# irfanfadhullah/unet_zoo

Hardware: AMD Instinct MI355X
Metric: images/sec (fwd+bwd) at B=16 3x256x256, 1/2/4/8 MI355X (higher is better)
Workload: dtype bf16; 1 GPU; unet train step (zero_grad+fwd+BCE+bwd+clip+AdamW), B=16/GPU 3x256x256, random-init weights; global_batch=16, parallelism=dp1

## Files before the change

### include/unetzoo_hip.h

```cpp
#ifndef UNETZOO_HIP_H
#define UNETZOO_HIP_H

#include <stddef.h>
#include <stdint.h>

#ifdef __cplusplus
extern "C" {
#endif

#define UZ_ABI_VERSION 1

enum { UZ_F32 = 0, UZ_BF16 = 1 };

enum {
  UZ_OK = 0,
  UZ_EINVAL = -1,
  UZ_ENOTIMPL = -2
};

enum {
  UZ_TAPS_CONV = 0,
  UZ_TAPS_GATHER2X2 = 1,
  UZ_TAPS_CONV_UP2 = 2,
  UZ_TAPS_CONV_S2 = 3
// ... 34 lines not shown
                         const void* res, int ldres, void* y, void* workspace, void* stream);
long long uz_conv_igemm_workspace_bytes(const uz_conv_desc* d);
int uz_conv_igemm_ws_grid_m(const uz_conv_desc* d);
int uz_conv_igemm_ws(const uz_conv_desc* d, const void* x, const void* w_packed, const float* bias,
                     void* y, float* stats_partial, void* workspace, void* stream);
int uz_conv_igemm_bnred_supported(const uz_conv_desc* d);
int uz_conv_igemm_bnred(const uz_conv_desc* d, const void* x, const void* w_packed, void* y, const void* bn_y,
                        int ld_bny, const float* scale, const float* shift, const float* mean, const float* invstd,
                        float* partial, void* stream);

int uz_conv_igemm_xf_supported(const uz_conv_desc* d);
int uz_conv_igemm_xf(const uz_conv_desc* d, const void* x, const float* in_scale, const float* in_shift,
                     const void* w_packed, const float* bias, void* y, float* stats_partial, void* stream);

int uz_conv_igemm_bnact_supported(const uz_conv_desc* d);
int uz_conv_igemm_bnact(const uz_conv_desc* d, const void* x, const void* w_packed, const float* bias,
                        const float* out_scale, const float* out_shift, int relu, void* y, void* stream);

typedef struct uz_wgrad_desc {
  int dtype;
  int N, H, W;
  int Hr, Wr;
  int Ci, ldl;
  int Cj, ldr;
  int ntaps, taps_mode, dil;
} uz_wgrad_desc;

int uz_wgrad_split(const uz_wgrad_desc* d);
long long uz_wgrad_workspace_bytes(const uz_wgrad_desc* d);
int uz_wgrad(const uz_wgrad_desc* d, const void* L, const void* R, float* out, void* workspace,
             void* stream);
int uz_wgrad_kernel_name(const uz_wgrad_desc* d, char* buf, int cap);
int uz_wgrad_xf_supported(const uz_wgrad_desc* d);
int uz_wgrad_xf(const uz_wgrad_desc* d, const void* L, const void* R, const float* r_scale, const float* r_shift,
                float* out, void* workspace, void* stream, int phase);
int uz_wgrad_phase(const uz_wgrad_desc* d, const void* L, const void* R, float* out, void* workspace, void* stream,
                   int phase);
typedef struct {
  uz_wgrad_desc desc;
  const void* L;
  const void* R;
  float* out;
} uz_wgrad_item;
long long uz_wgrad_multi_workspace_bytes(const uz_wgrad_item* items, int n);
int uz_wgrad_multi(const uz_wgrad_item* items, int n, void* workspace, void* stream);
long long uz_wgrad_batched_workspace_bytes(const uz_wgrad_desc* d, int batch);
int uz_wgrad_batched(const uz_wgrad_desc* d, int batch, const void* L, long long lb, const void* R, long long rb,
                     float* out, long long ob, void* workspace, void* stream);
int uz_wgrad_batched2(const uz_wgrad_desc* d, int batch, int batch2, const void* L, long long lb, long long lb2, const void* R,
                      long long rb, long long rb2, float* out, long long ob, void* workspace, void* stream);

int uz_conv3x3_first_supported(int dtype, int C, int Cout);
int uz_conv3x3_first_rows(int N, int H, int W);
int uz_conv3x3_first_fwd(int dtype, const float* x, int N, int C, int H, int W, const float* w, const float* bias, int Cout,
                         void* y, int ldy, float* stats, void* stream);
int uz_conv3x3_first_fwd_bnact(int dtype, const float* x, int N, int C, int H, int W, const float* w, const float* bias,
                               int Cout, const float* out_scale, const float* out_shift, int relu, void* y, int ldy,
                               void* stream);
long long uz_conv3x3_first_wgrad_workspace_bytes(int N, int H, int W, int Cout);
int uz_conv3x3_first_wgrad(int dtype, const float* x, int N, int C, int H, int W, const void* dy, int lddy, int Cout, float* dw,
                           void* workspace, void* stream);
int uz_conv3x3_first_wgrad_bn(int dtype, const float* x, int N, int C, int H, int W, const void* g, int ldg, const void* y,
                              int ldy, const float* scale, const float* shift, const float* mean, const float* invstd,
                              const double* sums, double count, int Cout, float* dw, void* workspace, void* stream);

enum { UZ_PACK_CONV_FWD = 0, UZ_PACK_CONV_DGRAD = 1, UZ_PACK_CONVT_FWD = 2, UZ_PACK_CONVT_DGRAD = 3,
       UZ_PACK_IM2COL = 4, UZ_PACK_VEC_REPEAT = 5 };
int uz_pack_weights(int dtype, int mode, const float* w, int Co, int Ci, int T, int Kpad, void* dst,
                    void* stream);
typedef struct uz_pack_item {
  const float* src;
  void* dst;
  long long begin;
  int mode, Co, Ci, T, Kpad;
  int pad_;
} uz_pack_item;
int uz_pack_weights_batched(int dtype, const uz_pack_item* items_device, int n_items,
                            long long total_elements, void* stream);
typedef struct uz_pack3x3_item {
  const float* src;
  void* dst_fwd;
  void* dst_dgrad;
  int Co, Ci;
  int tile_begin;
  int pad_;
} uz_pack3x3_item;
int uz_pack_conv3x3_batched(int dtype, const uz_pack3x3_item* items_device, int n_items, int total_tiles,
                            void* stream);

int uz_im2col3x3_nchw(int dtype, const float* x_nchw, int N, int C, int H, int W, int Kpad, void* dst,
                      void* stream);

int uz_bn_finalize(const float* stats_partial, int grid_m, int C, double count, const float* gamma,
                   const float* beta, float eps, float momentum, float* running_mean,
                   float* running_var, float* scale, float* shift, float* mean, float* invstd,
                   void* stream);
int uz_bn_eval_scale(int C, const float* gamma, const float* beta, const float* running_mean,
                     const float* running_var, float eps, float* scale, float* shift, void* stream);

int uz_bn_relu_apply(int dtype, const void* y, int ldy, const float* scale, const float* shift,
                     int N, int H, int W, int C, void* act, int lda, void* pooled, int ldp,
                     void* stream);
int uz_bn_relu_add_apply(int dtype, const void* y, int ldy, const float* scale, const float* shift,
                         int N, int H, int W, int C, const void* res, int ldr, void* act, int lda,
                         void* pooled, int ldp, int pool_ceil, void* stream);
int uz_bn_relu_add_apply_fin(int dtype, const void* y, int ldy, const float* stats_partial, int rows, double count,
                             const float* gamma, const float* beta, float eps, float momentum, float* running_mean,
                             float* running_var, float* vec, int* flag, int N, int H, int W, int C, const void* res, int ldr,
                             void* act, int lda, void* pooled, int ldp, int pool_ceil, void* stream);

typedef struct uz_bnbwd_desc {
  int dtype;
  int N, H, W, C;
  int ldy, ldg0, ldg1, ldgp, lddy;
  int pool_ceil;
} uz_bnbwd_desc;
int uz_colstats_rows(int dtype, int P, int C);
int uz_colstats(int dtype, const void* x, int ld, int P, int C, float* partial, void* stream);
long long uz_bn_relu_bwd_workspace_bytes(const uz_bnbwd_desc* d, int has_pool_grad);
int uz_bn_relu_bwd_reduce(const uz_bnbwd_desc* d, const void* y, const float* scale,
                          const float* shift, const float* mean, const float* invstd, const void* g0,
                          const void* g1, const void* gpool, void* workspace, double* sums,
                          float* dgamma, float* dbeta, void* stream);
int uz_bn_relu_bwd_apply(const uz_bnbwd_desc* d, const void* y, const float* scale,
                         const float* shift, const float* mean, const float* invstd, const void* g0,
                         const void* g1, const void* gpool, const double* sums, double count,
                         void* dy, void* stream);
int uz_bn_relu_bwd_reduce_rows(const uz_bnbwd_desc* d, const void* y, const float* scale, const float* shift,
                               const float* mean, const float* invstd, const void* g0, const void* g1, const void* gpool,
                               void* workspace, void* stream);
int uz_bn_relu_bwd_apply_fin(const uz_bnbwd_desc* d, const void* y, const float* scale, const float* shift,
                             const float* mean, const float* invstd, const void* g0, const void* g1, const void* gpool,
                             const float* partial, int rows, double* sums, float* dgamma, float* dbeta, int* flag,
                             double count, void* dy, void* stream);
int uz_bn_bwd_finalize(const float* partial, int rows, int C, double* sums, float* dgamma, float* dbeta, void* stream);
int uz_bn_relu_bwd_apply_head_supported(int dtype, int C, int Kout);
int uz_bn_relu_bwd_apply_head(const uz_bnbwd_desc* d, const void* y, const float* scale, const float* shift, const float* mean,
                              const float* invstd, const float* g_nchw, const float* w, int Kout, const double* sums,
                              double count, void* dy, void* stream);

int uz_outconv_fwd(int dtype, const void* x, int ldx, int N, int HW, int C, const float* w,
                   const float* b, int Kout, float* out_nchw, void* stream);
int uz_outconv_fwd_xf(int dtype, const void* y, int ldy, int N, int HW, int C, const float* scale, const float* shift,
                      const float* w, const float* b, int Kout, float* out_nchw, void* stream);
long long uz_outconv_bwd_workspace_bytes(int dtype, int N, int HW, int C, int Kout);
int uz_outconv_bwd(int dtype, const void* x, int ldx, int N, int HW, int C, const float* w, int Kout,
                   const float* g_nchw, void* dx, int lddx, float* dw, float* db, void* workspace,
                   void* stream);
int uz_outconv_bwd_rows(int dtype, int N, int HW, int C);
int uz_outconv_bwd_bnred(int dtype, const void* x, int ldx, int N, int HW, int C, const float* w, int Kout,
                         const float* g_nchw, void* dx, int lddx, float* dw, float* db, void* workspace,
                         const void* bn_y, int ld_bny, const float* scale, const float* shift, const float* mean,
                         const float* invstd, float* bn_partial, void* stream);

int uz_attn_grid(int dtype, int P, int channels);
int uz_attn_psi_fwd(int dtype, const void* g1raw, int ldg, const void* x1raw, int ldx, const float* vec_g,
                    const float* vec_x, const float* wpsi, const float* bpsi ,
                    int P, int F, float* q, float* partial , void* stream);
int uz_attn_gate_fwd(int dtype, const void* x, int ldx, const float* q, const float* vec_q, int P, int C,
                     void* out, int ldo, void* stream);
int uz_attn_bwd_psi(int dtype, const void* dout, int ldd, const void* x, int ldx, const float* q,
                    const float* vec_q, int P, int C, void* dx_direct, int lddx, float* dz,
                    float* partial , void* stream);
int uz_attn_bwd_reduce(int dtype, const void* g1raw, int ldg, const void* x1raw, int ldx, const float* q,
                       const float* dz, const float* wpsi, const float* vec_g, const float* vec_x,
                       const float* vec_q, const double* a01, int P, int F,
                       float* partial , void* stream);
int uz_attn_bwd_apply(int dtype, const void* g1raw, int ldg, const void* x1raw, int ldx, const float* q,
                      const float* dz, const float* wpsi, const float* vec_g, const float* vec_x,
                      const float* vec_q, const double* a01, const double* totals, int P, int F,
                      void* dg1raw, int lddg, void* dx1raw, int lddx, void* stream);
int uz_sum_rows(const float* partial, int rows, int n, double* out, void* stream);
int uz_sum_rows_f32(const float* partial, int rows, int n, float* out0, int n0, float* out1, void* stream);
int uz_sum_rows_f32_ld(const float* partial, int ld, int rows, int n, float* out0, int n0, float* out1,
                       void* stream);
int uz_sum2x2(int dtype, const void* du, int ldu, int N, int H, int W, int C, void* dx, int lddx,
              void* stream);

int uz_bilinear_fwd(int dtype, const void* x, int ldx, long long x_img_stride, int N, int Hi, int Wi,
                    int C, void* y, int ldy, long long y_img_stride, int Ho, int Wo, void* stream);
int uz_bilinear_bwd(int dtype, const void* g, int ldg, long long g_img_stride, int N, int Hi, int Wi,
                    int C, void* dx, int lddx, long long dx_img_stride, int Ho, int Wo, void* stream);
int uz_resize_bilinear_fwd(int dtype, const void* x, int ldx, long long x_img_stride, int N, int Hi, int Wi,
                           int C, void* y, int ldy, long long y_img_stride, int Ho, int Wo, int align_corners,
                           void* stream);
int uz_resize_bilinear_bwd(int dtype, const void* g, int ldg, long long g_img_stride, int N, int Hi, int Wi,
                           int C, void* dx, int lddx, long long dx_img_stride, int Ho, int Wo, int align_corners,
                           void* stream);
int uz_resample2(int dtype, const void* src, int lds, int N, int Hs, int Ws, int C, void* dst, int ldd, int Hd,
                 int Wd, int mode, void* stream);
int uz_pool_grad_combine(int dtype, int N, int H, int W, int C, const void* act, int lda, const void* g0,
                         int ldg0, const void* g1, int ldg1, const void* gp, int ldgp, void* out, int ldo,
                         int pool_ceil, void* stream);
int uz_sideconv3x3_fwd(int dtype, const void* x, int ldx, int N, int H, int W, int C, const float* w,
                       const float* bias, float* taps_ws, float* out, long long out_img_stride,
                       void* stream);
long long uz_sideconv3x3_bwd_workspace_bytes(int dtype, int N, int H, int W, int C);
int uz_sideconv3x3_bwd(int dtype, const void* x, int ldx, int N, int H, int W, int C, const float* w,
                       const float* g, long long g_img_stride, void* dx, int lddx, float* dw, float* db,
                       void* workspace, void* stream);
int uz_fuse1x1_fwd(const float* d, int N, int HW, int Cc, int K, const float* w, const float* b,
                   float* out, void* stream);
long long uz_fuse1x1_bwd_workspace_bytes(int N, int HW, int Cc, int K);
int uz_fuse1x1_bwd(const float* d, int N, int HW, int Cc, int K, const float* w, const float* g,
                   const float* const* g_extra, int n_extra, float* dcat, float* dw, float* db,
                   void* workspace, void* stream);

int uz_patchify(int dtype, const float* x_nchw, int N, int C, int H, int W, int patch, int Kpad,
                void* out, void* stream);

enum { UZ_LN_PLAIN = 0, UZ_LN_MERGE = 1, UZ_LN_EXPAND = 2 };
typedef struct uz_ln_desc {
  int dtype, N, Ho, Wo, C;
  int ldx, ldy, ldr, ldg, lddx;
  int mode, r;
  float eps;
  int act;
} uz_ln_desc;
int uz_layernorm_fwd(const uz_ln_desc* d, const void* x, const float* gamma, const float* beta,
                     const void* res, const float* image_scale, void* y, float* stats, void* stream);
int uz_layernorm_bwd_rows(const uz_ln_desc* d);
int uz_layernorm_bwd(const uz_ln_desc* d, const void* x, const float* gamma, const float* stats,
                     const void* g, const float* image_scale, void* dx, float* partial, void* stream);
int uz_layernorm_act_bwd(const uz_ln_desc* d, const void* x, const float* gamma, const float* beta,
                         const float* stats, const void* g, void* dx, float* partial, void* stream);
int uz_ln_head_fwd(const uz_ln_desc* d, const void* x, const float* gamma, const float* beta, const float* w,
                   const float* b , int K, float* logits, float* stats, void* stream);
long long uz_ln_head_bwd_workspace_bytes(const uz_ln_desc* d, int K);
int uz_ln_head_bwd(const uz_ln_desc* d, const void* x, const float* gamma, const float* beta, const float* w,
                   int K, const float* stats, const float* dlogits, void* dx, float* dgamma, float* dbeta,
                   float* dw, float* db , float* workspace, void* stream);

typedef struct uz_winattn_desc {
  int dtype, B, H, W, C, heads, ws, shift, Nt;
  int ldq, ldo;
  float scale;
} uz_winattn_desc;
int uz_winattn_fwd(const uz_winattn_desc* d, const void* qkv, const float* tau, const float* bias,
                   void* out, float* lse, void* stream);
int uz_cpb_fwd(const float* idx, const float* w1, const float* b1, const float* w2, const float* b2, int R,
               int hidden, int heads, float* bias, void* stream);
int uz_cpb_bwd(const float* idx, const float* w1, const float* b1, const float* w2, const float* G, int R,
               int hidden, int heads, float* dw1, float* db1, float* dw2, float* db2, void* stream);
typedef struct {
  const float* idx;
  const float* w1;
  const float* b1;
  const float* w2;
  const float* b2;
  int R, hidden, heads, reserved;
  float* bias;
  const float* G;
  float* dw1;
  float* db1;
  float* dw2;
  float* db2;
} uz_cpb_item;
int uz_cpb_fwd_batched(const uz_cpb_item* items, int n, void* stream);
long long uz_cpb_bwd_batched_workspace_bytes(const uz_cpb_item* items, int n);
int uz_cpb_bwd_batched(const uz_cpb_item* items, int n, float* workspace, void* stream);
int uz_winattn_bwd_rows(const uz_winattn_desc* d);
int uz_winattn_bwd(const uz_winattn_desc* d, const void* qkv, const float* tau, const float* bias,
                   const void* out, const float* lse, const void* dout, int lddo, void* dqkv, int lddq,
                   float* partial, void* stream);

int uz_colsum(int dtype, const void* x, int ld, int P, int C, float* out, void* stream);
long long uz_colsum_workspace_bytes(int dtype, int P, int C);
int uz_colsum_ws(int dtype, const void* x, int ld, int P, int C, float* out, void* workspace, void* stream);

long long uz_clip_adamw_workspace_bytes(void);
int uz_clip_adamw(float* p, const float* g, float* m, float* v, long long n, float lr, float beta1,
                  float beta2, float eps, float weight_decay, float max_norm, float* step, void* workspace,
                  void* stream);

int uz_gelu_fwd(int dtype, const void* x, int ldx, void* y, int ldy, long long P, int C, void* stream);
int uz_gelu_bwd(int dtype, const void* x, int ldx, const void* g, int ldg, void* dx, int lddx, long long P,
                int C, void* stream);
int uz_dwconv3x3(int dtype, const void* x, int ldx, const float* w_taps, const float* bias, void* y, int ldy,
                 int N, int H, int W, int C, int flags, void* stream);
int uz_dwconv3x3_wgrad_rows(int dtype, int N, int H, int W, int C);
int uz_dwconv3x3_wgrad(int dtype, const void* x, int ldx, const void* g, int ldg, float* part, int N, int H,
                       int W, int C, void* stream);
int uz_space_to_depth(int dtype, const void* src, int lds, void* dst, int ldd, int N, int Ho, int Wo, int C, int r,
                      int inverse, void* stream);
int uz_space_to_depth_crop(int dtype, const void* src, int lds, void* dst, int ldd, int N, int H, int W, int C, int r,
                           int inverse, void* stream);
int uz_im2col_nchw(int dtype, const float* x_nchw, int N, int C, int H, int W, int k, int stride, int pad, int Kpad,
                   void* out, void* stream);
typedef struct uz_sra_desc {
  int dtype, B, N, NK, heads, head_dim, kps;
  int ldq, ldk, ldv, ldo;
  float scale;
} uz_sra_desc;
int uz_sra_fwd(const uz_sra_desc* d, const void* q, const void* k, const void* v, void* out, float* lse,
               void* stream);
long long uz_sra_bwd_workspace_bytes(const uz_sra_desc* d);
int uz_sra_bwd(const uz_sra_desc* d, const void* q, const void* k, const void* v, const void* o, const float* lse,
               const void* go, int ldgo, void* dq, int lddq, void* dkv, int lddkv, void* workspace, void* stream);

long long uz_bce_dice_workspace_bytes(long long n);
int uz_bce_dice(const float* logits, const float* target, long long n, float* dlogits, float* out2, void* workspace,
                void* stream);

#define UZ_REGION_MAX_ITEMS 64
typedef struct uz_region_item {
  const float* logits;
// ... 144 lines not shown
```

### unet_zoo_amd/_lib.py

```python
from __future__ import annotations

import ctypes
import os
from ctypes import POINTER, Structure, c_char_p, c_double, c_float, c_int, c_void_p

import torch

UZ_F32, UZ_BF16 = 0, 1
TAPS_CONV, TAPS_GATHER2X2, TAPS_CONV_UP2, TAPS_CONV_S2 = 0, 1, 2, 3
STORE_PLAIN, STORE_SHUFFLE2X2 = 0, 1
PACK_CONV_FWD, PACK_CONV_DGRAD, PACK_CONVT_FWD, PACK_CONVT_DGRAD, PACK_IM2COL, PACK_VEC_REPEAT = range(6)

LIB_NAME = "libunetzoo_hip.so"
LIB_PATH = os.environ.get("UNET_ZOO_AMD_LIB") or os.path.join(os.path.dirname(os.path.abspath(__file__)), LIB_NAME)

EXPORTS = (
    "uz_abi_version", "uz_last_error_string", "uz_build_ablate", "uz_source_hash", "uz_set_cu_reserve", "uz_get_cu_reserve", "uz_clock_probe", "uz_conv_igemm_grid_m", "uz_conv_igemm",
    "uz_wgrad_split", "uz_wgrad_workspace_bytes", "uz_wgrad", "uz_wgrad_kernel_name", "uz_wgrad_phase", "uz_wgrad_xf_supported", "uz_wgrad_xf", "uz_conv3x3_first_supported", "uz_conv3x3_first_rows", "uz_conv3x3_first_fwd",
    "uz_conv3x3_first_wgrad_workspace_bytes", "uz_conv3x3_first_wgrad", "uz_conv3x3_first_wgrad_bn", "uz_pack_weights", "uz_pack_weights_batched", "uz_pack_conv3x3_batched", "uz_im2col3x3_nchw", "uz_bn_finalize",
    "uz_bn_eval_scale", "uz_bn_relu_apply", "uz_bn_relu_bwd_workspace_bytes", "uz_bn_relu_bwd_reduce", "uz_bn_relu_bwd_apply",
    "uz_outconv_fwd", "uz_outconv_fwd_xf", "uz_outconv_bwd_workspace_bytes", "uz_outconv_bwd", "uz_outconv_bwd_rows", "uz_outconv_bwd_bnred", "uz_bn_relu_bwd_apply_head_supported", "uz_bn_relu_bwd_apply_head",
    "uz_colsum",
    "uz_attn_grid", "uz_attn_psi_fwd", "uz_attn_gate_fwd", "uz_attn_bwd_psi", "uz_attn_bwd_reduce",
    "uz_attn_bwd_apply", "uz_sum_rows", "uz_sum_rows_f32", "uz_sum2x2",
    "uz_bn_relu_add_apply", "uz_bn_relu_add_apply_fin", "uz_bn_relu_bwd_reduce_rows", "uz_bn_relu_bwd_apply_fin", "uz_bilinear_fwd", "uz_bilinear_bwd", "uz_resize_bilinear_fwd", "uz_resize_bilinear_bwd", "uz_resample2",
    "uz_pool_grad_combine",
    "uz_sideconv3x3_fwd", "uz_sideconv3x3_bwd_workspace_bytes", "uz_sideconv3x3_bwd",
    "uz_fuse1x1_fwd", "uz_fuse1x1_bwd_workspace_bytes", "uz_fuse1x1_bwd",
    "uz_conv_igemm_workspace_bytes", "uz_conv_igemm_ws_grid_m", "uz_conv_igemm_ws",
    "uz_conv_igemm_bnred_supported", "uz_conv_igemm_bnred", "uz_conv_igemm_xf_supported", "uz_conv_igemm_xf", "uz_conv_igemm_kernel_name", "uz_bn_bwd_finalize", "uz_profile_arm", "uz_profile_disarm",
    "uz_patchify", "uz_layernorm_fwd", "uz_layernorm_bwd_rows", "uz_layernorm_bwd", "uz_layernorm_act_bwd",
    "uz_ln_head_fwd", "uz_ln_head_bwd_workspace_bytes", "uz_ln_head_bwd", "uz_sum_rows_f32_ld",
    "uz_winattn_fwd", "uz_winattn_bwd_rows", "uz_winattn_bwd",
    "uz_colsum_workspace_bytes", "uz_colsum_ws", "uz_colstats_rows", "uz_colstats", "uz_cpb_fwd", "uz_cpb_bwd",
    "uz_cpb_fwd_batched", "uz_cpb_bwd_batched_workspace_bytes", "uz_cpb_bwd_batched",
    "uz_clip_adamw_workspace_bytes", "uz_clip_adamw",
    "uz_gelu_fwd", "uz_gelu_bwd", "uz_dwconv3x3", "uz_dwconv3x3_wgrad_rows", "uz_dwconv3x3_wgrad",
    "uz_space_to_depth", "uz_space_to_depth_crop", "uz_im2col_nchw", "uz_sra_fwd", "uz_sra_bwd_workspace_bytes", "uz_sra_bwd",
    "uz_bce_dice_workspace_bytes", "uz_bce_dice", "uz_colsum_batched_workspace_bytes", "uz_colsum_batched", "uz_sum_rows_f32_batched", "uz_conv_igemm_res", "uz_wgrad_multi_workspace_bytes", "uz_wgrad_multi", "uz_conv_igemm_res_ws",
    "uz_add_relu", "uz_relu_bwd", "uz_pil_resample_h_u8", "uz_pil_resample_v_f32",
    "uz_gemm_nt", "uz_softmax_fwd", "uz_softmax_bwd", "uz_adaptive_avgpool_fwd", "uz_adaptive_avgpool_bwd",
    "uz_rowdot_f32", "uz_cast_rows", "uz_wgrad_batched_workspace_bytes", "uz_wgrad_batched", "uz_wgrad_batched2",
    "uz_softmax_workspace_bytes", "uz_add_map", "uz_dropout", "uz_chanscale_relu", "uz_chanattn_probs_fwd", "uz_chanattn_probs_bwd",
    "uz_conv5x5_grid_m", "uz_conv5x5", "uz_wgrad5x5_workspace_bytes", "uz_wgrad5x5",
    "uz_bn_elu_apply", "uz_bn_elu_bwd_rows", "uz_bn_elu_bwd_reduce", "uz_bn_elu_bwd_apply",
    "uz_conv_igemm_bnact_supported", "uz_conv_igemm_bnact", "uz_conv3x3_first_fwd_bnact",
    "uz_region_loss_workspace_bytes", "uz_region_loss",
    "uz_class_loss_workspace_bytes", "uz_class_loss",
)


class ConvDesc(Structure):
    _fields_ = [(n, c_int) for n in (
        "dtype", "N", "H", "W", "Hin", "Win", "Cin", "ldx", "Nout", "ldy", "ntaps", "taps_mode",
        "dil", "store_mode", "Co", "Hout", "Wout")]


class WgradDesc(Structure):
    _fields_ = [(n, c_int) for n in (
        "dtype", "N", "H", "W", "Hr", "Wr", "Ci", "ldl", "Cj", "ldr", "ntaps", "taps_mode", "dil")]


class Conv5Desc(Structure):
    _fields_ = [(n, c_int) for n in ("dtype", "N", "H", "W", "Cin", "ldx", "Nout", "ldy", "ksize")]


class Wgrad5Desc(Structure):
    _fields_ = [(n, c_int) for n in ("dtype", "N", "H", "W", "Ci", "ldl", "Cj", "ldr", "ksize", "CiOut", "CjOut")]


class BnEluBwdDesc(Structure):
    _fields_ = [(n, c_int) for n in ("dtype", "N", "HW", "C", "ldx", "ldo", "ldg0", "ldg1", "ldg2", "lddx", "ldgres", "flags")]


class BnBwdDesc(Structure):
    _fields_ = [(n, c_int) for n in (
        "dtype", "N", "H", "W", "C", "ldy", "ldg0", "ldg1", "ldgp", "lddy", "pool_ceil")]


class LnDesc(Structure):
    _fields_ = [(n, c_int) for n in ("dtype", "N", "Ho", "Wo", "C", "ldx", "ldy", "ldr", "ldg", "lddx", "mode", "r")] \
        + [("eps", c_float), ("act", c_int)]


class WinAttnDesc(Structure):
    _fields_ = [(n, c_int) for n in ("dtype", "B", "H", "W", "C", "heads", "ws", "shift", "Nt", "ldq", "ldo")] \
        + [("scale", c_float)]


class SraDesc(Structure):
    _fields_ = [(n, c_int) for n in ("dtype", "B", "N", "NK", "heads", "head_dim", "kps", "ldq", "ldk", "ldv", "ldo")] \
        + [("scale", c_float)]


class GemmDesc(Structure):
    _fields_ = [(n, c_int) for n in ("dtype", "batch", "M", "N", "K", "ldx", "ldw", "ldy", "ldres")] \
        + [(n, ctypes.c_longlong) for n in ("xb", "wb", "yb", "resb")] + [("batch2", c_int)] \
        + [(n, ctypes.c_longlong) for n in ("xb2", "wb2", "yb2", "resb2")]


class WgradItem(Structure):
    _fields_ = [("desc", WgradDesc), ("L", c_void_p), ("R", c_void_p), ("out", c_void_p)]


class SumRowsItem(Structure):
    _fields_ = [("partial", c_void_p), ("out0", c_void_p), ("out1", c_void_p), ("rows", c_int), ("n", c_int), ("n0", c_int),
                ("reserved", c_int)]


class ColsumItem(Structure):
    _fields_ = [("x", c_void_p), ("out", c_void_p), ("P", c_int), ("C", c_int), ("ld", c_int), ("reserved", c_int)]


LN_PLAIN, LN_MERGE, LN_EXPAND = 0, 1, 2


class CpbItem(Structure):
    _fields_ = [(n, c_void_p) for n in ("idx", "w1", "b1", "w2", "b2")] \
        + [(n, c_int) for n in ("R", "hidden", "heads", "reserved")] \
        + [(n, c_void_p) for n in ("bias", "G", "dw1", "db1", "dw2", "db2")]


class PackItem(Structure):
    _fields_ = [("src", c_void_p), ("dst", c_void_p), ("begin", ctypes.c_longlong), ("mode", c_int),
                ("Co", c_int), ("Ci", c_int), ("T", c_int), ("Kpad", c_int), ("pad_", c_int)]


class Pack3x3Item(Structure):
    _fields_ = [("src", c_void_p), ("dst_fwd", c_void_p), ("dst_dgrad", c_void_p), ("Co", c_int), ("Ci", c_int),
                ("tile_begin", c_int), ("pad_", c_int)]


REGION_MAX_ITEMS = 64


class RegionItem(Structure):
    _fields_ = [("logits", c_void_p), ("target", c_void_p), ("dlogits", c_void_p), ("weight", c_float)]


class RegionDesc(Structure):
    _fields_ = [("n_items", c_int), ("n", ctypes.c_longlong), ("groups", c_int)] \
        + [(n, c_float) for n in ("w_bce", "w_region", "alpha", "beta", "smooth", "gamma", "pos_weight")] \
        + [("metric_item", c_int)]


CLASS_MAX_ITEMS = 16
CLASS_MAX_K = 32
CLASS_REDUCE_BATCH, CLASS_REDUCE_IMAGE = 0, 1


class ClassItem(Structure):
    _fields_ = [("logits", c_void_p), ("dlogits", c_void_p), ("weight", c_float)]


class ClassDesc(Structure):
    _fields_ = [("n_items", c_int), ("N", c_int), ("K", c_int), ("HW", ctypes.c_longlong)] \
        + [(n, c_float) for n in ("w_ce", "w_dice", "smooth", "label_smoothing")] \
        + [(n, c_int) for n in ("ignore_index", "reduce", "include_background", "square", "metric_item")]


class HipLibraryError(RuntimeError):
    pass


_lib = None


def load():
    global _lib
    if _lib is not None:
        return _lib
    if not os.path.exists(LIB_PATH):
        raise HipLibraryError(
            f"{LIB_PATH} not found: the HIP kernel library is not built. Run "
            "`python -c 'import __graft_entry__ as g; g.build()'` from the repo root. "
            "unet_zoo_amd has no CPU fallback.")
    lib = ctypes.CDLL(LIB_PATH)
    lib.uz_abi_version.restype = c_int
    lib.uz_last_error_string.restype = c_char_p
    lib.uz_source_hash.restype = c_char_p
    lib.uz_source_hash.argtypes = []
    vp, ip, fp = c_void_p, c_int, c_float
    lib.uz_set_cu_reserve.argtypes = [c_int]
    lib.uz_clock_probe.argtypes = [c_int, vp, c_int, vp]
    lib.uz_get_cu_reserve.argtypes = []
    lib.uz_conv_igemm_grid_m.argtypes = [POINTER(ConvDesc)]
    lib.uz_conv_igemm.argtypes = [POINTER(ConvDesc), vp, vp, vp, vp, vp, vp]
    lib.uz_conv_igemm_res.argtypes = [POINTER(ConvDesc), vp, vp, vp, vp, ip, vp, vp]
    lib.uz_conv_igemm_res_ws.argtypes = [POINTER(ConvDesc), vp, vp, vp, vp, ip, vp, vp, vp]
    lib.uz_conv_igemm_workspace_bytes.argtypes = [POINTER(ConvDesc)]
    lib.uz_conv_igemm_ws_grid_m.argtypes = [POINTER(ConvDesc)]
    lib.uz_conv_igemm_ws.argtypes = [POINTER(ConvDesc), vp, vp, vp, vp, vp, vp, vp]
    lib.uz_conv_igemm_bnred_supported.argtypes = [POINTER(ConvDesc)]
    lib.uz_conv_igemm_xf_supported.argtypes = [POINTER(ConvDesc)]
    lib.uz_conv_igemm_xf.argtypes = [POINTER(ConvDesc), vp, vp, vp, vp, vp, vp, vp, vp]
    lib.uz_conv_igemm_bnact_supported.argtypes = [POINTER(ConvDesc)]
    lib.uz_conv_igemm_bnact.argtypes = [POINTER(ConvDesc), vp, vp, vp, vp, vp, c_int, vp, vp]
    lib.uz_conv_igemm_kernel_name.argtypes = [POINTER(ConvDesc), c_int, c_char_p, c_int]
    lib.uz_profile_arm.argtypes = [vp, vp]
    lib.uz_profile_disarm.argtypes = []
    lib.uz_conv_igemm_bnred.argtypes = [POINTER(ConvDesc), vp, vp, vp, vp, c_int, vp, vp, vp, vp, vp, vp]
    lib.uz_bn_bwd_finalize.argtypes = [vp, c_int, c_int, vp, vp, vp, vp]
    lib.uz_patchify.argtypes = [ip, vp, ip, ip, ip, ip, ip, ip, vp, vp]
    lib.uz_layernorm_fwd.argtypes = [POINTER(LnDesc), vp, vp, vp, vp, vp, vp, vp, vp]
    lib.uz_layernorm_act_bwd.argtypes = [POINTER(LnDesc), vp, vp, vp, vp, vp, vp, vp, vp]
    lib.uz_layernorm_bwd_rows.argtypes = [POINTER(LnDesc)]
    lib.uz_layernorm_bwd.argtypes = [POINTER(LnDesc), vp, vp, vp, vp, vp, vp, vp, vp]
    lib.uz_ln_head_fwd.argtypes = [POINTER(LnDesc), vp, vp, vp, vp, vp, ip, vp, vp, vp]
    lib.uz_ln_head_bwd_workspace_bytes.argtypes = [POINTER(LnDesc), ip]
    lib.uz_ln_head_bwd.argtypes = [POINTER(LnDesc), vp, vp, vp, vp, ip, vp, vp, vp, vp, vp, vp, vp, vp, vp]
    lib.uz_sum_rows_f32_ld.argtypes = [vp, ip, ip, ip, vp, ip, vp, vp]
    lib.uz_winattn_fwd.argtypes = [POINTER(WinAttnDesc), vp, vp, vp, vp, vp, vp]
    lib.uz_winattn_bwd_rows.argtypes = [POINTER(WinAttnDesc)]
    lib.uz_winattn_bwd.argtypes = [POINTER(WinAttnDesc), vp, vp, vp, vp, vp, vp, ip, vp, ip, vp, vp]
    lib.uz_colstats_rows.argtypes = [ip, ip, ip]
    lib.uz_colstats.argtypes = [ip, vp, ip, ip, ip, vp, vp]
    lib.uz_cpb_fwd.argtypes = [vp, vp, vp, vp, vp, ip, ip, ip, vp, vp]
    lib.uz_cpb_bwd.argtypes = [vp, vp, vp, vp, vp, ip, ip, ip, vp, vp, vp, vp, vp]
    lib.uz_cpb_fwd_batched.argtypes = [vp, ip, vp]
    lib.uz_cpb_bwd_batched_workspace_bytes.argtypes = [vp, ip]
    lib.uz_cpb_bwd_batched.argtypes = [vp, ip, vp, vp]
    lib.uz_clip_adamw_workspace_bytes.argtypes = []
    lib.uz_clip_adamw.argtypes = [vp, vp, vp, vp, ctypes.c_longlong, fp, fp, fp, fp, fp, fp, vp, vp, vp]
    lib.uz_wgrad_split.argtypes = [POINTER(WgradDesc)]
    lib.uz_wgrad_workspace_bytes.argtypes = [POINTER(WgradDesc)]
    lib.uz_wgrad.argtypes = [POINTER(WgradDesc), vp, vp, vp, vp, vp]
    lib.uz_wgrad_kernel_name.argtypes = [POINTER(WgradDesc), c_char_p, c_int]
    lib.uz_wgrad_phase.argtypes = [POINTER(WgradDesc), vp, vp, vp, vp, vp, c_int]
    lib.uz_wgrad_xf_supported.argtypes = [POINTER(WgradDesc)]
    lib.uz_wgrad_xf.argtypes = [POINTER(WgradDesc), vp, vp, vp, vp, vp, vp, vp, c_int]
    lib.uz_conv3x3_first_supported.argtypes = [ip, ip, ip]
    lib.uz_conv3x3_first_rows.argtypes = [ip, ip, ip]
    lib.uz_conv3x3_first_fwd.argtypes = [ip, vp, ip, ip, ip, ip, vp, vp, ip, vp, ip, vp, vp]
    lib.uz_conv3x3_first_fwd_bnact.argtypes = [ip, vp, ip, ip, ip, ip, vp, vp, ip, vp, vp, ip, vp, ip, vp]
    lib.uz_conv3x3_first_wgrad_workspace_bytes.argtypes = [ip, ip, ip, ip]
    lib.uz_conv3x3_first_wgrad_workspace_bytes.restype = ctypes.c_longlong
    lib.uz_conv3x3_first_wgrad.argtypes = [ip, vp, ip, ip, ip, ip, vp, ip, ip, vp, vp, vp]
    lib.uz_conv3x3_first_wgrad_bn.argtypes = [ip, vp, ip, ip, ip, ip, vp, ip, vp, ip, vp, vp, vp, vp, vp, ctypes.c_double, ip, vp, vp, vp]
    lib.uz_pack_weights.argtypes = [ip, ip, vp, ip, ip, ip, ip, vp, vp]
    lib.uz_pack_weights_batched.argtypes = [ip, vp, ip, ctypes.c_longlong, vp]
    lib.uz_pack_conv3x3_batched.argtypes = [ip, vp, ip, ip, vp]
    lib.uz_im2col3x3_nchw.argtypes = [ip, vp, ip, ip, ip, ip, ip, vp, vp]
    lib.uz_bn_finalize.argtypes = [vp, ip, ip, c_double, vp, vp, fp, fp, vp, vp, vp, vp, vp, vp, vp]
    lib.uz_bn_eval_scale.argtypes = [ip, vp, vp, vp, vp, fp, vp, vp, vp]
    lib.uz_bn_relu_apply.argtypes = [ip, vp, ip, vp, vp, ip, ip, ip, ip, vp, ip, vp, ip, vp]
    lib.uz_bn_relu_bwd_workspace_bytes.argtypes = [POINTER(BnBwdDesc), ip]
    lib.uz_bn_relu_bwd_reduce.argtypes = [POINTER(BnBwdDesc), vp, vp, vp, vp, vp, vp, vp, vp, vp, vp,
                                          vp, vp, vp]
    lib.uz_bn_relu_bwd_apply.argtypes = [POINTER(BnBwdDesc), vp, vp, vp, vp, vp, vp, vp, vp, vp,
                                         c_double, vp, vp]
    lib.uz_outconv_fwd.argtypes = [ip, vp, ip, ip, ip, ip, vp, vp, ip, vp, vp]
    lib.uz_outconv_fwd_xf.argtypes = [ip, vp, ip, ip, ip, ip, vp, vp, vp, vp, ip, vp, vp]
    lib.uz_outconv_bwd_workspace_bytes.argtypes = [ip, ip, ip, ip, ip]
    lib.uz_outconv_bwd.argtypes = [ip, vp, ip, ip, ip, ip, vp, ip, vp, vp, ip, vp, vp, vp, vp]
    lib.uz_outconv_bwd_rows.argtypes = [ip, ip, ip, ip]
    lib.uz_bn_relu_bwd_apply_head_supported.argtypes = [ip, ip, ip]
    lib.uz_bn_relu_bwd_apply_head.argtypes = [POINTER(BnBwdDesc), vp, vp, vp, vp, vp, vp, vp, ip, vp, ctypes.c_double, vp, vp]
    lib.uz_outconv_bwd_bnred.argtypes = [ip, vp, ip, ip, ip, ip, vp, ip, vp, vp, ip, vp, vp, vp, vp, ip, vp, vp, vp, vp, vp, vp]
    lib.uz_colsum.argtypes = [ip, vp, ip, ip, ip, vp, vp]
    lib.uz_colsum_workspace_bytes.argtypes = [ip, ip, ip]
    lib.uz_colsum_ws.argtypes = [ip, vp, ip, ip, ip, vp, vp, vp]
    lib.uz_attn_grid.argtypes = [ip, ip, ip]
    lib.uz_attn_psi_fwd.argtypes = [ip, vp, ip, vp, ip, vp, vp, vp, vp, ip, ip, vp, vp, vp]
    lib.uz_attn_gate_fwd.argtypes = [ip, vp, ip, vp, vp, ip, ip, vp, ip, vp]
    lib.uz_attn_bwd_psi.argtypes = [ip, vp, ip, vp, ip, vp, vp, ip, ip, vp, ip, vp, vp, vp]
    lib.uz_attn_bwd_reduce.argtypes = [ip, vp, ip, vp, ip, vp, vp, vp, vp, vp, vp, vp, ip, ip, vp, vp]
    lib.uz_attn_bwd_apply.argtypes = [ip, vp, ip, vp, ip, vp, vp, vp, vp, vp, vp, vp, vp, ip, ip, vp, ip,
                                      vp, ip, vp]
    lib.uz_sum_rows.argtypes = [vp, ip, ip, vp, vp]
    lib.uz_sum_rows_f32.argtypes = [vp, ip, ip, vp, ip, vp, vp]
    lib.uz_sum2x2.argtypes = [ip, vp, ip, ip, ip, ip, ip, vp, ip, vp]
    ll = ctypes.c_longlong
    lib.uz_bn_relu_add_apply.argtypes = [ip, vp, ip, vp, vp, ip, ip, ip, ip, vp, ip, vp, ip, vp, ip, ip, vp]
    lib.uz_bn_relu_add_apply_fin.argtypes = [ip, vp, ip, vp, ip, ctypes.c_double, vp, vp, c_float, c_float, vp, vp, vp, vp,
                                             ip, ip, ip, ip, vp, ip, vp, ip, vp, ip, ip, vp]
    lib.uz_bn_relu_bwd_reduce_rows.argtypes = [POINTER(BnBwdDesc), vp, vp, vp, vp, vp, vp, vp, vp, vp, vp]
    lib.uz_bn_relu_bwd_apply_fin.argtypes = [POINTER(BnBwdDesc), vp, vp, vp, vp, vp, vp, vp, vp, vp, ip, vp, vp, vp, vp,
                                             ctypes.c_double, vp, vp]
    lib.uz_bilinear_fwd.argtypes = [ip, vp, ip, ll, ip, ip, ip, ip, vp, ip, ll, ip, ip, vp]
    lib.uz_bilinear_bwd.argtypes = [ip, vp, ip, ll, ip, ip, ip, ip, vp, ip, ll, ip, ip, vp]
    lib.uz_resize_bilinear_fwd.argtypes = [ip, vp, ip, ll, ip, ip, ip, ip, vp, ip, ll, ip, ip, ip, vp]
    lib.uz_resize_bilinear_bwd.argtypes = [ip, vp, ip, ll, ip, ip, ip, ip, vp, ip, ll, ip, ip, ip, vp]
    lib.uz_resample2.argtypes = [ip, vp, ip, ip, ip, ip, ip, vp, ip, ip, ip, ip, vp]
    lib.uz_pool_grad_combine.argtypes = [ip, ip, ip, ip, ip, vp, ip, vp, ip, vp, ip, vp, ip, vp, ip, ip, vp]
    lib.uz_sideconv3x3_fwd.argtypes = [ip, vp, ip, ip, ip, ip, ip, vp, vp, vp, vp, ll, vp]
    lib.uz_sideconv3x3_bwd_workspace_bytes.argtypes = [ip, ip, ip, ip, ip]
    lib.uz_sideconv3x3_bwd.argtypes = [ip, vp, ip, ip, ip, ip, ip, vp, vp, ll, vp, ip, vp, vp, vp, vp]
    lib.uz_fuse1x1_fwd.argtypes = [vp, ip, ip, ip, ip, vp, vp, vp, vp]
    lib.uz_fuse1x1_bwd_workspace_bytes.argtypes = [ip, ip, ip, ip]
    lib.uz_fuse1x1_bwd.argtypes = [vp, ip, ip, ip, ip, vp, vp, POINTER(c_void_p), ip, vp, vp, vp, vp, vp]
    lib.uz_sum_rows_f32_batched.argtypes = [POINTER(SumRowsItem), ip, vp]
    lib.uz_wgrad_multi_workspace_bytes.argtypes = [POINTER(WgradItem), ip]
    lib.uz_wgrad_multi_workspace_bytes.restype = ctypes.c_longlong
    lib.uz_wgrad_multi.argtypes = [POINTER(WgradItem), ip, vp, vp]
    lib.uz_colsum_batched_workspace_bytes.argtypes = [ip, POINTER(ColsumItem), ip]
    lib.uz_colsum_batched.argtypes = [ip, POINTER(ColsumItem), ip, vp, vp]
    lib.uz_bce_dice_workspace_bytes.argtypes = [ll]
    lib.uz_bce_dice.argtypes = [vp, vp, ll, vp, vp, vp, vp]
    lib.uz_gelu_fwd.argtypes = [ip, vp, ip, vp, ip, ll, ip, vp]
    lib.uz_gelu_bwd.argtypes = [ip, vp, ip, vp, ip, vp, ip, ll, ip, vp]
    lib.uz_dwconv3x3.argtypes = [ip, vp, ip, vp, vp, vp, ip, ip, ip, ip, ip, ip, vp]
    lib.uz_dwconv3x3_wgrad_rows.argtypes = [ip, ip, ip, ip, ip]
    lib.uz_dwconv3x3_wgrad.argtypes = [ip, vp, ip, vp, ip, vp, ip, ip, ip, ip, vp]
    lib.uz_space_to_depth.argtypes = [ip, vp, ip, vp, ip, ip, ip, ip, ip, ip, ip, vp]
    lib.uz_space_to_depth_crop.argtypes = [ip, vp, ip, vp, ip, ip, ip, ip, ip, ip, ip, vp]
    lib.uz_im2col_nchw.argtypes = [ip, vp, ip, ip, ip, ip, ip, ip, ip, ip, vp, vp]
    lib.uz_sra_fwd.argtypes = [POINTER(SraDesc), vp, vp, vp, vp, vp, vp]
    lib.uz_sra_bwd_workspace_bytes.argtypes = [POINTER(SraDesc)]
    lib.uz_sra_bwd.argtypes = [POINTER(SraDesc), vp, vp, vp, vp, vp, vp, ip, vp, ip, vp, ip, vp, vp]
    lib.uz_add_relu.argtypes = [ip, vp, ip, vp, ip, vp, ip, ll, ip, vp]
    lib.uz_relu_bwd.argtypes = [ip, vp, ip, vp, ip, vp, ip, ll, ip, vp]
    lib.uz_pil_resample_h_u8.argtypes = [vp, ip, ip, ip, vp, vp, ip, ip, vp, vp]
    lib.uz_pil_resample_v_f32.argtypes = [vp, ip, ip, ip, vp, vp, ip, ip, POINTER(c_float), POINTER(c_float), ip, vp, vp]
    lib.uz_wgrad_batched_workspace_bytes.argtypes = [POINTER(WgradDesc), ip]
    lib.uz_wgrad_batched.argtypes = [POINTER(WgradDesc), ip, vp, ll, vp, ll, vp, ll, vp, vp]
    lib.uz_wgrad_batched2.argtypes = [POINTER(WgradDesc), ip, ip, vp, ll, ll, vp, ll, ll, vp, ll, vp, vp]
    lib.uz_gemm_nt.argtypes = [POINTER(GemmDesc), vp, vp, vp, vp, vp, vp]
    lib.uz_softmax_workspace_bytes.argtypes = [ip, ip, ip, ip]
    lib.uz_softmax_fwd.argtypes = [ip, vp, ip, ll, ip, ip, ip, ip, c_float, vp, vp]
    lib.uz_chanattn_probs_fwd.argtypes = [ip, vp, ip, ip, ip, ip, c_float, c_float, vp, vp, vp]
    lib.uz_chanattn_probs_bwd.argtypes = [ip, vp, vp, ip, ip, ip, ip, c_float, c_float, vp, vp, vp]
    lib.uz_dropout.argtypes = [ip, vp, ip, vp, c_float, vp, ip, ll, ip, vp]
    lib.uz_chanscale_relu.argtypes = [ip, ip, vp, ip, vp, ip, vp, vp, ip, ip, ip, vp, ip, vp]
    lib.uz_add_map.argtypes = [ip, vp, ip, vp, vp, ip, ll, ip, ip, vp]
    lib.uz_softmax_bwd.argtypes = [ip, vp, vp, ip, ll, ip, ip, ip, ip, c_float, vp, ip, vp]
    lib.uz_adaptive_avgpool_fwd.argtypes = [ip, vp, ip, ip, ip, ip, ip, vp, ip, ip, ip, vp]
    lib.uz_adaptive_avgpool_bwd.argtypes = [ip, vp, ip, ip, ip, ip, ip, vp, ip, ip, ip, ip, vp]
    lib.uz_rowdot_f32.argtypes = [ip, vp, ip, vp, ip, ll, ip, vp, vp]
    lib.uz_cast_rows.argtypes = [ip, vp, ip, vp, ip, ll, ip, ip, vp]
    lib.uz_conv5x5_grid_m.argtypes = [POINTER(Conv5Desc)]
    lib.uz_conv5x5.argtypes = [POINTER(Conv5Desc), vp, vp, vp, vp, vp, vp]
    lib.uz_wgrad5x5_workspace_bytes.argtypes = [POINTER(Wgrad5Desc)]
    lib.uz_wgrad5x5.argtypes = [POINTER(Wgrad5Desc), vp, vp, vp, vp, vp]
    lib.uz_bn_elu_apply.argtypes = [ip, vp, ip, vp, vp, ip, ip, ip, vp, ip, vp, ip, vp, ip, vp, ip, vp]
    lib.uz_bn_elu_bwd_rows.argtypes = [POINTER(BnEluBwdDesc)]
    lib.uz_bn_elu_bwd_reduce.argtypes = [POINTER(BnEluBwdDesc), vp, vp, vp, vp, vp, vp, vp, vp, vp, vp, vp, vp]
    lib.uz_bn_elu_bwd_apply.argtypes = [POINTER(BnEluBwdDesc), vp, vp, vp, vp, vp, vp, vp, vp, vp, vp, vp, vp, vp, vp]
    lib.uz_region_loss_workspace_bytes.argtypes = [POINTER(RegionDesc)]
    lib.uz_region_loss.argtypes = [POINTER(RegionDesc), POINTER(RegionItem), vp, vp, vp]
    lib.uz_class_loss_workspace_bytes.argtypes = [POINTER(ClassDesc)]
    lib.uz_class_loss.argtypes = [POINTER(ClassDesc), POINTER(ClassItem), vp, vp, vp, vp, vp, vp]
    for name in EXPORTS:
        fn = getattr(lib, name)
        if name not in ("uz_last_error_string", "uz_source_hash"):
            fn.restype = ctypes.c_longlong if name.endswith("_workspace_bytes") else c_int
    if lib.uz_abi_version() != 1:
        raise HipLibraryError("libunetzoo_hip.so ABI version mismatch; rebuild it")
    _lib = lib
    return lib


def _fail(rc: int, what: str):
    msg = load().uz_last_error_string().decode("utf-8", "replace")
    raise HipLibraryError(f"{what} failed (code {rc}): {msg}")


def check(rc: int, what: str) -> None:
    if rc != 0:
        _fail(rc, what)


def check_count(rc: int, what: str) -> int:
    if rc < 0:
        _fail(rc, what)
    return rc


def region_loss_workspace_bytes(desc: "RegionDesc") -> int:
    return check_count(load().uz_region_loss_workspace_bytes(ctypes.byref(desc)), "uz_region_loss_workspace_bytes")


def region_loss(desc: "RegionDesc", items, out2: torch.Tensor, workspace: torch.Tensor) -> None:
    check(load().uz_region_loss(ctypes.byref(desc), items, out2.data_ptr(), workspace.data_ptr(), stream_ptr()),
          "uz_region_loss")


def class_loss_workspace_bytes(desc: "ClassDesc") -> int:
    return check_count(load().uz_class_loss_workspace_bytes(ctypes.byref(desc)), "uz_class_loss_workspace_bytes")


def class_loss(desc: "ClassDesc", items, labels: torch.Tensor, class_weight, out2: torch.Tensor, counts: torch.Tensor,
               workspace: torch.Tensor) -> None:
    check(load().uz_class_loss(ctypes.byref(desc), items, labels.data_ptr(),
                               class_weight.data_ptr() if class_weight is not None else None, out2.data_ptr(),
                               counts.data_ptr() if counts is not None else None, workspace.data_ptr(), stream_ptr()),
          "uz_class_loss")


def set_cu_reserve(n: int) -> None:
    check(load().uz_set_cu_reserve(int(n)), "uz_set_cu_reserve")


def get_cu_reserve() -> int:
    return int(load().uz_get_cu_reserve())


def mfma_clock_ghz(settle_s: float = 0.6, iters: int = 40000) -> dict:
    import time
    lib = load()
    dev = torch.device("cuda", torch.cuda.current_device())
    out = torch.zeros(256, 2, dtype=torch.int64, device=dev)
    torch.cuda.synchronize()
    t_end = time.perf_counter() + settle_s
    while time.perf_counter() < t_end:
        for _ in range(4):
            check(lib.uz_clock_probe(iters, out.data_ptr(), 256, stream_ptr()), "uz_clock_probe")
        torch.cuda.synchronize()
    e0, e1 = torch.cuda.Event(enable_timing=True), torch.cuda.Event(enable_timing=True)
    e0.record()
    check(lib.uz_clock_probe(iters, out.data_ptr(), 256, stream_ptr()), "uz_clock_probe")
    e1.record()
# ... 28 lines not shown
```

### unet_zoo_amd/csrc/uz_common.h

```cpp
#pragma once
#include <hip/hip_runtime.h>
#include <stdarg.h>
#include <stdint.h>
#include <stdio.h>
#include "../../include/unetzoo_hip.h"

typedef __bf16 bf16_t;
typedef __attribute__((ext_vector_type(16))) float f32x16;
typedef __attribute__((ext_vector_type(4))) float f32x4;
typedef __attribute__((ext_vector_type(8))) __bf16 bf16x8;
typedef __attribute__((ext_vector_type(4))) __bf16 bf16x4;

#include <hip/hip_ext.h>
bool uz_prof_take(hipEvent_t* e0, hipEvent_t* e1);
#undef hipLaunchKernelGGL
#define hipLaunchKernelGGL(kern, grid, block, shm, stream, ...)                                              \
  do {                                                                                                       \
    hipEvent_t uz_e0_, uz_e1_;                                                                               \
    if (uz_prof_take(&uz_e0_, &uz_e1_))                                                                      \
      hipExtLaunchKernelGGL(kern, dim3(grid), dim3(block), (shm), (stream), uz_e0_, uz_e1_, 0, __VA_ARGS__);   \
    else                                                                                                     \
      kern<<<dim3(grid), dim3(block), (shm), (stream)>>>(__VA_ARGS__);                                       \
  } while (0)

#define UZ_WAVE 64
#define UZ_NUM_CU_HW 256
#define UZ_NUM_XCD 8
int uz_num_cu();
#define UZ_NUM_CU (uz_num_cu())

void uz_set_error(const char* fmt, ...);

#define UZ_REQUIRE(cond, ...)            \
  do {                                   \
    if (!(cond)) {                       \
      uz_set_error(__VA_ARGS__);         \
      return UZ_EINVAL;                  \
    }                                    \
  } while (0)

#define UZ_LAUNCH_CHECK(name)                                               \
  do {                                                                      \
    hipError_t e__ = hipGetLastError();                                     \
    if (e__ != hipSuccess) {                                                \
      uz_set_error("%s: launch failed: %s", name, hipGetErrorString(e__));  \
      return (int)e__;                                                      \
    }                                                                       \
  } while (0)

template <typename T> struct ElemTraits;
template <> struct ElemTraits<float> {
  static constexpr int VEC = 4;
};
template <> struct ElemTraits<bf16_t> {
  static constexpr int VEC = 8;
};

template <typename T> struct alignas(16) Vec16 {
  T v[ElemTraits<T>::VEC];
};

template <typename T> __device__ __forceinline__ Vec16<T> ld16(const T* p) {
  return *reinterpret_cast<const Vec16<T>*>(p);
}
template <typename T> __device__ __forceinline__ void st16(T* p, const Vec16<T>& v) {
  *reinterpret_cast<Vec16<T>*>(p) = v;
}
template <typename T> __device__ __forceinline__ Vec16<T> zero16() {
  Vec16<T> z;
#pragma unroll
  for (int i = 0; i < ElemTraits<T>::VEC; ++i) z.v[i] = (T)0.0f;
  return z;
}

static inline int uz_cdiv(long long a, long long b) { return (int)((a + b - 1) / b); }

template <int RG>
__device__ __forceinline__ void uz_sum_rows_wide_body(const float* __restrict__ partial, int ld, int rows, int n,
                                                      float* __restrict__ out0, int n0, float* __restrict__ out1, int block) {
  constexpr int CQ = 256 / RG;
  __shared__ double sh[RG][CQ][4 + 1];
  const int cq = threadIdx.x % CQ, g = threadIdx.x / CQ;
  const int e = (block * CQ + cq) * 4;
  double s[4] = {0.0, 0.0, 0.0, 0.0};
  if (e < n) {
    int r = g;
    for (; r + 3 * RG < rows; r += 4 * RG) {
      float4 v[4];
#pragma unroll
      for (int u = 0; u < 4; ++u) v[u] = *reinterpret_cast<const float4*>(partial + (size_t)(r + u * RG) * ld + e);
#pragma unroll
      for (int u = 0; u < 4; ++u) {
        s[0] += (double)v[u].x;
        s[1] += (double)v[u].y;
        s[2] += (double)v[u].z;
        s[3] += (double)v[u].w;
      }
    }
    for (; r < rows; r += RG) {
      const float4 v = *reinterpret_cast<const float4*>(partial + (size_t)r * ld + e);
      s[0] += (double)v.x;
      s[1] += (double)v.y;
      s[2] += (double)v.z;
      s[3] += (double)v.w;
    }
  }
#pragma unroll
  for (int i = 0; i < 4; ++i) sh[g][cq][i] = s[i];
  __syncthreads();
  if (g == 0 && e < n) {
#pragma unroll
    for (int i = 0; i < 4; ++i) {
      double t = 0.0;
      for (int r = 0; r < RG; ++r) t += sh[r][cq][i];
      const int idx = e + i;
      if (idx < n0) out0[idx] = (float)t;
      else out1[idx - n0] = (float)t;
    }
  }
}
static inline int uz_sum_rows_wide_rg(const float* partial, int ld, int rows, int n) {
  if (rows <= 256 && n >= 16384 && n % 4 == 0 && ld % 4 == 0 && ((uintptr_t)partial & 15) == 0) return rows >= 64 ? 16 : 4;
  return 0;
}

#include <stdlib.h>
#ifdef UZ_ABLATE
#define UZ_KFLAGS(a) ((a).flags)
#else
#define UZ_KFLAGS(a) 0
#endif
#ifdef UZ_ABLATE
static inline int uz_tune_flags() {
  const char* e = getenv("UZ_TUNE");
  return e ? atoi(e) : 0;
}
static inline const char* uz_ablate_env(const char* name) { return getenv(name); }
#else
static inline int uz_tune_flags() { return 0; }
static inline const char* uz_ablate_env(const char*) { return nullptr; }
#endif

struct UzDirectPlan {
  int tw, bn, bres, th_n, tw_n, ntiles, tiles_n, grid_m;
  int ppcfg;
  int ksplit, cps;
};
int uz_direct_plan(const uz_conv_desc* d, UzDirectPlan* p);
struct UzBnRed {
  const void* y;
  int ldy;
  const float *scale, *shift, *mean, *invstd;
};
struct UzXf {
  const float *scale, *shift;
};
struct UzBnAct {
  const float *scale, *shift;
  int relu;
};
int uz_direct_launch(const uz_conv_desc* d, const UzDirectPlan& p, const void* x, const void* w,
                     const float* bias, void* y, float* stats, hipStream_t s, const UzBnRed* br = nullptr,
                     float* part = nullptr,
                     const UzXf* xf = nullptr, const UzBnAct* ba = nullptr);

enum { UZ_PP_512 = 0,
       UZ_PP_512X64 = 1,
       UZ_PP_256 = 2,
       UZ_PP_256W16 = 3,
       UZ_PP_128W16 = 4 };
struct UzPpPlan {
  int cfg, bn, th_n, tw_n, ntiles, tiles_n, grid_m;
  int ksplit, cps;
};
int uz_pp_plan(const uz_conv_desc* d, UzPpPlan* p);
int uz_pp_launch(const uz_conv_desc* d, const UzPpPlan& p, const void* x, const void* w, const float* bias, void* y,
                 float* stats, hipStream_t s, const UzBnRed* br = nullptr, float* part = nullptr, const UzXf* xf = nullptr,
                 const UzBnAct* ba = nullptr);
int uz_pp_xf_channels(const UzPpPlan& p);

struct UzWgrad2Plan {
  int big, one_tap, gather, kw, kr, tiles_i, tiles_j, kg, units, upb, split, nslabs, H, W;
  int wide9;
  int v9, bi;
};
int uz_wgrad9_plan(const uz_wgrad_desc* d, UzWgrad2Plan* p);
int uz_wgrad9_launch(const uz_wgrad_desc* d, const UzWgrad2Plan& p, const void* L, const void* R, float* slab, hipStream_t s,
                     const UzXf* xf = nullptr);
const char* uz_wgrad9_name(const UzWgrad2Plan& p);
int uz_wgrad_g4_plan(const uz_wgrad_desc* d, UzWgrad2Plan* p);
int uz_wgrad_g4_launch(const uz_wgrad_desc* d, const UzWgrad2Plan& p, const void* L, const void* R, float* slab, hipStream_t s);
int uz_wgrad3x3_plan(const uz_wgrad_desc* d, UzWgrad2Plan* p, int batch = 1);
int uz_wgrad3x3_launch(const uz_wgrad_desc* d, const UzWgrad2Plan& p, const void* L, const void* R,
                       float* slab, hipStream_t s, int batch = 1, long long lb_bytes = 0, long long rb_bytes = 0,
                       long long slab_stride = 0,
                       int batch2 = 1, long long lb2_bytes = 0, long long rb2_bytes = 0,
                       const UzXf* xf = nullptr);

struct UzWgradMultiItem {
  const uz_wgrad_desc* d;
  UzWgrad2Plan p;
  const void *L, *R;
  float* slab;
};
int uz_wgrad3x3_multi_max();
int uz_wgrad3x3_multi_launch(const UzWgradMultiItem* items, int n, hipStream_t s);

struct UzGemmPlan {
  int bn, bm, nst, tiles_m, tiles_n, grid_m;
  int ksplit, cps;
};
int uz_gemm_dma_plan(const uz_conv_desc* d, UzGemmPlan* p);
long long uz_gemm_dma_workspace_bytes(const uz_conv_desc* d);
int uz_gemm_dma_launch(const uz_conv_desc* d, const UzGemmPlan& p, const void* x, const void* w,
                       const float* bias, void* y, float* stats, hipStream_t s, const void* res = nullptr,
                       int ldres = 0, const UzBnRed* br = nullptr, float* part = nullptr);
```

### unet_zoo_amd/csrc/uz_eltwise.hip

```cpp
#include "uz_common.h"

namespace {

template <typename T> __device__ __forceinline__ void load_f(const T* p, float* f) {
  const Vec16<T> v = ld16(p);
#pragma unroll
  for (int i = 0; i < ElemTraits<T>::VEC; ++i) f[i] = (float)v.v[i];
}
template <typename T> __device__ __forceinline__ void store_f(T* p, const float* f) {
  Vec16<T> v;
#pragma unroll
  for (int i = 0; i < ElemTraits<T>::VEC; ++i) v.v[i] = (T)f[i];
  st16(p, v);
}

template <int EW>
__global__ __launch_bounds__(1024) void bn_finalize_kernel(
    const float* __restrict__ part, int grid_m, int C, double count, const float* __restrict__ gamma,
    const float* __restrict__ beta, float eps, float momentum, float* running_mean,
    float* running_var, float* scale, float* shift, float* mean, float* invstd) {
  constexpr int NG = 1024 / EW;
  __shared__ double sh[2][NG][EW + 1];
  const int cl = threadIdx.x % EW, g = threadIdx.x / EW;
  const int c = blockIdx.x * EW + cl;
// ... 655 lines not shown
#pragma unroll
    for (int i = 0; i < VEC; ++i) wr[k][i] = live ? w[k * C + sub * VEC + i] : 0.f;
  float xsc[VEC], xsh[VEC];
  if constexpr (XF) {
#pragma unroll
    for (int i = 0; i < VEC; ++i) {
      xsc[i] = live ? xf_scale[sub * VEC + i] : 0.f;
      xsh[i] = live ? xf_shift[sub * VEC + i] : 0.f;
    }
  }
  for (int p0 = blockIdx.x * ppb; p0 < P; p0 += gridDim.x * ppb) {
    const int p = p0 + pl;
    float v[VEC];
    if (p < P && live) {
      load_f(x + (size_t)p * ldx + sub * VEC, v);
      if constexpr (XF) {
#pragma unroll
        for (int i = 0; i < VEC; ++i) v[i] = (float)(T)fmaxf(fmaf(v[i], xsc[i], xsh[i]), 0.f);
      }
    } else {
#pragma unroll
      for (int i = 0; i < VEC; ++i) v[i] = 0.f;
    }
    const int img = (KOUT == 1) ? 0 : p / HW;
    const int hw = p - img * HW;
#pragma unroll
    for (int k = 0; k < KOUT; ++k) {
      float s = 0.f;
#pragma unroll
      for (int i = 0; i < VEC; ++i) s = fmaf(v[i], wr[k][i], s);
      for (int o = LPP >> 1; o > 0; o >>= 1) s += __shfl_xor(s, o);
      if (sub == 0 && p < P) out[((size_t)img * KOUT + k) * HW + hw] = s + b[k];
    }
  }
}

template <typename T, int KOUT, bool BNRED = false, bool XNULL = false>
__global__ __launch_bounds__(256) void outconv_bwd_kernel(const T* __restrict__ x, int ldx, int N,
                                                          int HW, int C, const float* __restrict__ w,
                                                          const float* __restrict__ g,
                                                          T* __restrict__ dx, int lddx,
                                                          float* __restrict__ partial, const T* __restrict__ bn_y = nullptr, int ld_bny = 0,
                                                          const float* __restrict__ bn_scale = nullptr, const float* __restrict__ bn_shift = nullptr,
                                                          const float* __restrict__ bn_mean = nullptr, const float* __restrict__ bn_invstd = nullptr,
                                                          float* __restrict__ bnpart = nullptr) {
  constexpr int VEC = ElemTraits<T>::VEC;
  constexpr int UNR = 4;
  __shared__ float red[256 * 9];
  const int LPP = lanes_per_pixel(C / VEC);
  const int ppb = blockDim.x / LPP;
  const int sub = threadIdx.x % LPP, pl = threadIdx.x / LPP;
  const bool live = sub < C / VEC;
  const int P = N * HW;
  float wr[KOUT][VEC], aw[KOUT][VEC], ab[KOUT];
#pragma unroll
  for (int k = 0; k < KOUT; ++k) {
    ab[k] = 0.f;
#pragma unroll
    for (int i = 0; i < VEC; ++i) {
      wr[k][i] = live ? w[k * C + sub * VEC + i] : 0.f;
      aw[k][i] = 0.f;
    }
  }
  float bsc[VEC], bsh[VEC], bmu[VEC], bis[VEC], S0[VEC], S1[VEC];
  if constexpr (BNRED) {
#pragma unroll
    for (int i = 0; i < VEC; ++i) {
      const int ch = live ? sub * VEC + i : 0;
      bsc[i] = bn_scale[ch];
      bsh[i] = bn_shift[ch];
      bmu[i] = bn_mean[ch];
      bis[i] = bn_invstd[ch];
      S0[i] = S1[i] = 0.f;
    }
  }
  for (int p0 = blockIdx.x * ppb * UNR; p0 < P; p0 += gridDim.x * ppb * UNR) {
    float v[UNR][VEC], gk[UNR][KOUT], yv[UNR][VEC];
    int pp[UNR];
#pragma unroll
    for (int u = 0; u < UNR; ++u) {
      const int p = p0 + u * ppb + pl;
      const bool inp = p < P, ok = inp && live;
      pp[u] = inp ? p : -1;
      const size_t pc = ok ? (size_t)p : 0;
      const int cs = ok ? sub * VEC : 0;
      Vec16<T> xr, yr;
      if constexpr (BNRED) yr = ld16(bn_y + pc * ld_bny + cs);
      if constexpr (!XNULL) xr = ld16(x + pc * ldx + cs);
      const int pg = inp ? p : 0;
      const int img = (KOUT == 1) ? 0 : pg / HW;
      const int hw = pg - img * HW;
#pragma unroll
      for (int k = 0; k < KOUT; ++k) {
        const float gq = g[((size_t)img * KOUT + k) * HW + hw];
        gk[u][k] = inp ? gq : 0.f;
      }
#pragma unroll
      for (int i = 0; i < VEC; ++i) {
        if constexpr (BNRED) {
          yv[u][i] = (float)yr.v[i];
          float xv;
          if constexpr (XNULL) xv = (float)(T)fmaxf(fmaf(yv[u][i], bsc[i], bsh[i]), 0.f);
          else xv = (float)xr.v[i];
          v[u][i] = ok ? xv : 0.f;
        } else {
          v[u][i] = ok ? (float)xr.v[i] : 0.f;
        }
      }
    }
#pragma unroll
    for (int u = 0; u < UNR; ++u) {
      float d[VEC];
#pragma unroll
      for (int i = 0; i < VEC; ++i) d[i] = 0.f;
#pragma unroll
      for (int k = 0; k < KOUT; ++k) {
        ab[k] += gk[u][k];
#pragma unroll
        for (int i = 0; i < VEC; ++i) {
          d[i] = fmaf(gk[u][k], wr[k][i], d[i]);
          aw[k][i] = fmaf(gk[u][k], v[u][i], aw[k][i]);
        }
      }
      if (dx != nullptr && pp[u] >= 0 && live) store_f(dx + (size_t)pp[u] * lddx + sub * VEC, d);
      if constexpr (BNRED) {
        if (pp[u] >= 0 && live) {
#pragma unroll
          for (int i = 0; i < VEC; ++i) {
            const float dz = fmaf(yv[u][i], bsc[i], bsh[i]) > 0.f ? (float)(T)d[i] : 0.f;
            S0[i] += dz;
            S1[i] += dz * ((yv[u][i] - bmu[i]) * bis[i]);
          }
        }
      }
    }
  }
  if constexpr (BNRED) {
#pragma unroll
    for (int which = 0; which < 2; ++which) {
      __syncthreads();
#pragma unroll
      for (int i = 0; i < VEC; ++i) red[threadIdx.x * 9 + i] = which ? S1[i] : S0[i];
      __syncthreads();
      if (pl == 0 && live) {
        float t[VEC];
#pragma unroll
        for (int i = 0; i < VEC; ++i) t[i] = 0.f;
        for (int r = 0; r < ppb; ++r)
#pragma unroll
          for (int i = 0; i < VEC; ++i) t[i] += red[(r * LPP + sub) * 9 + i];
#pragma unroll
        for (int i = 0; i < VEC; ++i) bnpart[((size_t)blockIdx.x * 2 + which) * C + sub * VEC + i] = t[i];
      }
    }
  }
#pragma unroll
  for (int k = 0; k < KOUT; ++k) {
    __syncthreads();
#pragma unroll
    for (int i = 0; i < VEC; ++i) red[threadIdx.x * 9 + i] = aw[k][i];
    red[threadIdx.x * 9 + 8] = ab[k];
    __syncthreads();
    if (pl == 0) {
      float t[9];
#pragma unroll
      for (int i = 0; i < 9; ++i) t[i] = 0.f;
      for (int r = 0; r < ppb; ++r)
#pragma unroll
        for (int i = 0; i < 9; ++i)
          if (i < VEC || i == 8) t[i] += red[(r * LPP + sub) * 9 + i];
      float* row = partial + ((size_t)blockIdx.x * KOUT + k) * (C + 1);
      if (live) {
#pragma unroll
        for (int i = 0; i < VEC; ++i) row[sub * VEC + i] = t[i];
      }
      if (sub == 0) row[C] = t[8];
    }
  }
}

__global__ __launch_bounds__(1024) void outconv_bwd_finalize_kernel(const float* __restrict__ partial, int rows,
                                                                    int Kout, int C, float* __restrict__ dw,
                                                                    float* __restrict__ db) {
  __shared__ double sh[32][33];
  const int el = threadIdx.x & 31, g = threadIdx.x >> 5;
  const int ne = Kout * (C + 1);
  const int e = blockIdx.x * 32 + el;
  double s = 0.0;
  {
    const bool in = e < ne;
    const float* base = partial + (in ? e : 0);
    for (int r = g; r < rows; r += 8 * 32) {
      float v[8];
#pragma unroll
      for (int u = 0; u < 8; ++u) v[u] = base[(size_t)(r + u * 32 < rows ? r + u * 32 : 0) * ne];
#pragma unroll
      for (int u = 0; u < 8; ++u) asm volatile("" : "+v"(v[u]));
#pragma unroll
      for (int u = 0; u < 8; ++u)
        if (in && r + u * 32 < rows) s += (double)v[u];
    }
  }
  sh[g][el] = s;
  __syncthreads();
#pragma unroll
  for (int st = 16; st > 0; st >>= 1) {
    if (g < st) sh[g][el] += sh[g + st][el];
    __syncthreads();
  }
  if (g == 0 && e < ne) {
    const double t = sh[0][el];
    const int k = e / (C + 1), c = e - k * (C + 1);
    if (c < C) dw[k * C + c] = (float)t;
    else db[k] = (float)t;
  }
}

#define UZ_KOUT_SWITCH(K, ...)                   \
  switch (K) {                                   \
    case 1: { constexpr int KOUT = 1; __VA_ARGS__; break; } \
    case 2: { constexpr int KOUT = 2; __VA_ARGS__; break; } \
    case 3: { constexpr int KOUT = 3; __VA_ARGS__; break; } \
    case 4: { constexpr int KOUT = 4; __VA_ARGS__; break; } \
    case 5: { constexpr int KOUT = 5; __VA_ARGS__; break; } \
    case 6: { constexpr int KOUT = 6; __VA_ARGS__; break; } \
    case 7: { constexpr int KOUT = 7; __VA_ARGS__; break; } \
    default: { constexpr int KOUT = 8; __VA_ARGS__; break; } \
  }

template <typename T, bool PARTIAL>
__global__ __launch_bounds__(256) void colsum_kernel(const T* __restrict__ x, int ld, long long P, int C,
                                                     float* __restrict__ out) {
  constexpr int VEC = ElemTraits<T>::VEC;
  extern __shared__ __attribute__((aligned(16))) float red[];
  const int CC = C / VEC;
  const int cc = blockIdx.y * blockDim.x + threadIdx.x;
  const bool cok = cc < CC;
  const int c0 = (cok ? cc : 0) * VEC;
  float s[VEC];
#pragma unroll
  for (int i = 0; i < VEC; ++i) s[i] = 0.f;
  for (long long p = (long long)blockIdx.x * blockDim.y + threadIdx.y; p < P && cok;
       p += (long long)gridDim.x * blockDim.y) {
    float v[VEC];
    load_f(x + (size_t)p * ld + c0, v);
#pragma unroll
    for (int i = 0; i < VEC; ++i) s[i] += v[i];
  }
  float* mine = red + ((size_t)threadIdx.y * blockDim.x + threadIdx.x) * VEC;
#pragma unroll
  for (int i = 0; i < VEC; ++i) mine[i] = s[i];
  __syncthreads();
  for (int e = threadIdx.y; e < VEC; e += blockDim.y) {
    float t = 0.f;
    for (int r = 0; r < (int)blockDim.y; ++r) t += red[((size_t)r * blockDim.x + threadIdx.x) * VEC + e];
    if (cok) {
      if (PARTIAL) out[(size_t)blockIdx.x * C + c0 + e] = t;
      else atomicAdd(out + c0 + e, t);
    }
  }
}

template <typename T>
__global__ __launch_bounds__(256) void colstats_kernel(const T* __restrict__ x, int ld, long long P, int C,
                                                       float* __restrict__ out) {
  constexpr int VEC = ElemTraits<T>::VEC;
  extern __shared__ __attribute__((aligned(16))) float red[];
  const int CC = C / VEC;
  const int cc = blockIdx.y * blockDim.x + threadIdx.x;
  const bool cok = cc < CC;
  const int c0 = (cok ? cc : 0) * VEC;
  float s[VEC], q[VEC];
#pragma unroll
  for (int i = 0; i < VEC; ++i) s[i] = q[i] = 0.f;
  const long long stride = (long long)gridDim.x * blockDim.y;
  for (long long p = (long long)blockIdx.x * blockDim.y + threadIdx.y; p < P && cok; p += 4 * stride) {
    float v[4][VEC];
#pragma unroll
    for (int k = 0; k < 4; ++k) {
      if (p + k * stride < P) {
        load_f(x + (size_t)(p + k * stride) * ld + c0, v[k]);
      } else {
#pragma unroll
        for (int i = 0; i < VEC; ++i) v[k][i] = 0.f;
      }
    }
#pragma unroll
    for (int k = 0; k < 4; ++k)
#pragma unroll
      for (int i = 0; i < VEC; ++i) {
        s[i] += v[k][i];
        q[i] = fmaf(v[k][i], v[k][i], q[i]);
      }
  }
  float* mine = red + ((size_t)threadIdx.y * blockDim.x + threadIdx.x) * (2 * VEC);
#pragma unroll
  for (int i = 0; i < VEC; ++i) {
    mine[i] = s[i];
    mine[VEC + i] = q[i];
  }
  __syncthreads();
  for (int e = threadIdx.y; e < 2 * VEC; e += blockDim.y) {
    float t = 0.f;
    for (int r = 0; r < (int)blockDim.y; ++r) t += red[((size_t)r * blockDim.x + threadIdx.x) * (2 * VEC) + e];
    if (cok) out[((size_t)blockIdx.x * 2 + e / VEC) * C + c0 + (e % VEC)] = t;
  }
// ... 576 lines not shown
  UZ_REQUIRE(count > 0 && rows > 0, "uz_bn_relu_bwd_apply_fin: count / rows");
  UZ_REQUIRE((dgamma == nullptr) == (dbeta == nullptr), "uz_bn_relu_bwd_apply_fin: dgamma/dbeta");
  const int vec = d->dtype == UZ_BF16 ? 8 : 4;
  UZ_REQUIRE(d->lddy % vec == 0 && d->lddy >= d->C, "uz_bn_relu_bwd_apply_fin: bad lddy");
  BnBwdArgs a = bnbwd_args(d, y, scale, shift, mean, invstd, g0, g1, gpool);
  a.sums = sums;
  a.dy = dy;
  a.inv_count = 1.0 / count;
  a.fin.part = partial; a.fin.rows = rows; a.fin.ew = fin_ew(rows, d->C);
  a.fin.sums = sums; a.fin.dgamma = dgamma; a.fin.dbeta = dbeta; a.fin.flag = flag;
  hipStream_t s = (hipStream_t)stream;
  dim3 grid, block;
  bnbwd_shape(d, gpool != nullptr, &grid, &block, 2);
  if ((long long)grid.x * grid.y < (d->C + a.fin.ew - 1) / a.fin.ew) {
    bnbwd_finalize(partial, rows, d->C, sums, dgamma, dbeta, s);
    UZ_LAUNCH_CHECK("uz_bn_relu_bwd_apply_fin(finalize)");
    a.fin = BnFin{};
    return d->dtype == UZ_BF16 ? bnbwd_launch<bf16_t, 2>(d, a, gpool != nullptr, s) : bnbwd_launch<float, 2>(d, a, gpool != nullptr, s);
  }
  return d->dtype == UZ_BF16 ? bnbwd_launch<bf16_t, 2, true>(d, a, gpool != nullptr, s)
                             : bnbwd_launch<float, 2, true>(d, a, gpool != nullptr, s);
}

extern "C" int uz_bn_relu_bwd_apply_head_supported(int dtype, int C, int Kout) {
  return dtype == UZ_BF16 && C > 0 && C % 8 == 0 && Kout >= 1 && Kout <= OUTCONV_MAXK;
}

extern "C" int uz_bn_relu_bwd_apply_head(const uz_bnbwd_desc* d, const void* y, const float* scale, const float* shift,
                                         const float* mean, const float* invstd, const float* g_nchw, const float* w,
                                         int Kout, const double* sums, double count, void* dy, void* stream) {
  UZ_REQUIRE(d != nullptr, "uz_bn_relu_bwd_apply_head: null descriptor");
  UZ_REQUIRE(uz_bn_relu_bwd_apply_head_supported(d->dtype, d->C, Kout), "uz_bn_relu_bwd_apply_head: dtype=%d C=%d Kout=%d unsupported",
             d->dtype, d->C, Kout);
  UZ_REQUIRE(y && scale && shift && mean && invstd && g_nchw && w && sums && dy, "uz_bn_relu_bwd_apply_head: null pointer");
  UZ_REQUIRE(d->N > 0 && d->H > 0 && d->W > 0 && (long long)d->N * d->H * d->W < (1LL << 31), "uz_bn_relu_bwd_apply_head: bad shape");
  UZ_REQUIRE(d->ldy % 8 == 0 && d->ldy >= d->C && d->lddy % 8 == 0 && d->lddy >= d->C, "uz_bn_relu_bwd_apply_head: bad ldy / lddy");
  UZ_REQUIRE((d->pool_ceil & 3) == 0, "uz_bn_relu_bwd_apply_head: a ReLU block without a pool only");
  UZ_REQUIRE(count > 0, "uz_bn_relu_bwd_apply_head: count");
  BnBwdHeadArgs a;
  a.y = static_cast<const bf16_t*>(y);
  a.dy = static_cast<bf16_t*>(dy);
  a.scale = scale;
  a.shift = shift;
  a.mean = mean;
  a.invstd = invstd;
  a.sums = sums;
  a.g = g_nchw;
  a.w = w;
  a.inv_count = 1.0 / count;
  a.P = d->N * d->H * d->W;
  a.HW = d->H * d->W;
  a.C = d->C;
  a.ldy = d->ldy;
  a.lddy = d->lddy;
  a.rev = (d->pool_ceil & 4) != 0;
  dim3 grid, block;
  bnbwd_shape(d, false, &grid, &block, 2);
  hipStream_t s = (hipStream_t)stream;
  UZ_KOUT_SWITCH(Kout, hipLaunchKernelGGL((bn_relu_bwd_head_kernel<KOUT>), grid, block, 0, s, a))
  UZ_LAUNCH_CHECK("uz_bn_relu_bwd_apply_head");
  return UZ_OK;
}

extern "C" int uz_outconv_fwd(int dtype, const void* x, int ldx, int N, int HW, int C, const float* w,
                              const float* b, int Kout, float* out_nchw, void* stream) {
  UZ_REQUIRE(dtype == UZ_F32 || dtype == UZ_BF16, "uz_outconv_fwd: bad dtype");
  const int vec = dtype == UZ_BF16 ? 8 : 4;
  UZ_REQUIRE(x && w && b && out_nchw, "uz_outconv_fwd: null pointer");
  UZ_REQUIRE(Kout >= 1 && Kout <= OUTCONV_MAXK, "uz_outconv_fwd: Kout=%d (max %d)", Kout, OUTCONV_MAXK);
  UZ_REQUIRE(C % vec == 0 && C / vec <= 64, "uz_outconv_fwd: C=%d unsupported", C);
  UZ_REQUIRE(ldx % vec == 0 && ldx >= C && N > 0 && HW > 0 && (long long)N * HW < (1LL << 31),
             "uz_outconv_fwd: bad shape");
  const int ppb = 256 / lanes_per_pixel(C / vec);
  const int grid = grid_for(((long long)N * HW + ppb - 1) / ppb, 1);
  hipStream_t s = (hipStream_t)stream;
  if (dtype == UZ_BF16) {
    UZ_KOUT_SWITCH(Kout, hipLaunchKernelGGL((outconv_fwd_kernel<bf16_t, KOUT>), dim3(grid), dim3(256), 0, s, (const bf16_t*)x, ldx, N, HW, C, w, b, out_nchw, (const float*)nullptr, (const float*)nullptr))
  } else {
    UZ_KOUT_SWITCH(Kout, hipLaunchKernelGGL((outconv_fwd_kernel<float, KOUT>), dim3(grid), dim3(256), 0, s, (const float*)x, ldx, N, HW, C, w, b, out_nchw, (const float*)nullptr, (const float*)nullptr))
  }
  UZ_LAUNCH_CHECK("uz_outconv_fwd");
  return UZ_OK;
}

extern "C" int uz_outconv_fwd_xf(int dtype, const void* y, int ldy, int N, int HW, int C, const float* scale,
                                 const float* shift, const float* w, const float* b, int Kout, float* out_nchw,
                                 void* stream) {
  UZ_REQUIRE(dtype == UZ_BF16, "uz_outconv_fwd_xf: bf16 only");
  UZ_REQUIRE(y && scale && shift && w && b && out_nchw, "uz_outconv_fwd_xf: null pointer");
  UZ_REQUIRE(Kout >= 1 && Kout <= OUTCONV_MAXK, "uz_outconv_fwd_xf: Kout=%d (max %d)", Kout, OUTCONV_MAXK);
  UZ_REQUIRE(C % 8 == 0 && C / 8 <= 64, "uz_outconv_fwd_xf: C=%d unsupported", C);
  UZ_REQUIRE(ldy % 8 == 0 && ldy >= C && N > 0 && HW > 0 && (long long)N * HW < (1LL << 31), "uz_outconv_fwd_xf: bad shape");
  const int ppb = 256 / lanes_per_pixel(C / 8);
  const int grid = grid_for(((long long)N * HW + ppb - 1) / ppb, 1);
  hipStream_t s = (hipStream_t)stream;
  UZ_KOUT_SWITCH(Kout, hipLaunchKernelGGL((outconv_fwd_kernel<bf16_t, KOUT, true>), dim3(grid), dim3(256), 0, s, (const bf16_t*)y, ldy, N, HW, C, w, b, out_nchw, scale, shift))
  UZ_LAUNCH_CHECK("uz_outconv_fwd_xf");
  return UZ_OK;
}

static int outconv_bwd_grid(int dtype, int N, int HW, int C) {
  const int vec = dtype == UZ_BF16 ? 8 : 4;
  const int ppb = 256 / lanes_per_pixel(C / vec);
  long long g = ((long long)N * HW + (long long)ppb * 4 - 1) / ((long long)ppb * 4);
  if (g > UZ_NUM_CU * 4) g = UZ_NUM_CU * 4;
  if (g < 1) g = 1;
  return (int)g;
}

extern "C" long long uz_outconv_bwd_workspace_bytes(int dtype, int N, int HW, int C, int Kout) {
  UZ_REQUIRE(dtype == UZ_F32 || dtype == UZ_BF16, "uz_outconv_bwd_workspace_bytes: bad dtype");
  const int vec = dtype == UZ_BF16 ? 8 : 4;
  UZ_REQUIRE(N > 0 && HW > 0 && Kout >= 1 && Kout <= OUTCONV_MAXK && C % vec == 0 && C / vec <= 64,
             "uz_outconv_bwd_workspace_bytes: bad shape");
  return (long long)outconv_bwd_grid(dtype, N, HW, C) * Kout * (C + 1) * (long long)sizeof(float);
}

extern "C" int uz_outconv_bwd_rows(int dtype, int N, int HW, int C) {
  UZ_REQUIRE(dtype == UZ_F32 || dtype == UZ_BF16, "uz_outconv_bwd_rows: bad dtype");
  return outconv_bwd_grid(dtype, N, HW, C);
}

extern "C" int uz_outconv_bwd_bnred(int dtype, const void* x, int ldx, int N, int HW, int C, const float* w,
                                    int Kout, const float* g_nchw, void* dx, int lddx, float* dw, float* db,
                                    void* workspace, const void* bn_y, int ld_bny, const float* scale,
                                    const float* shift, const float* mean, const float* invstd, float* bn_partial,
                                    void* stream) {
  UZ_REQUIRE(dtype == UZ_BF16, "uz_outconv_bwd_bnred: bf16 only");
  UZ_REQUIRE(w && g_nchw && dw && db && workspace && bn_y && scale && shift && mean && invstd && bn_partial,
             "uz_outconv_bwd_bnred: null pointer");
  UZ_REQUIRE(Kout >= 1 && Kout <= OUTCONV_MAXK, "uz_outconv_bwd_bnred: Kout=%d", Kout);
  UZ_REQUIRE(C % 8 == 0 && C / 8 <= 64, "uz_outconv_bwd_bnred: C=%d unsupported", C);
  UZ_REQUIRE((x == nullptr || (ldx % 8 == 0 && ldx >= C)) && (dx == nullptr || (lddx % 8 == 0 && lddx >= C)) && ld_bny % 8 == 0 && ld_bny >= C && N > 0 &&
                 HW > 0 && (long long)N * HW < (1LL << 31), "uz_outconv_bwd_bnred: bad shape");
  const int g = outconv_bwd_grid(dtype, N, HW, C);
  float* part = static_cast<float*>(workspace);
  hipStream_t s = (hipStream_t)stream;
  if (x != nullptr) {
    UZ_KOUT_SWITCH(Kout, hipLaunchKernelGGL((outconv_bwd_kernel<bf16_t, KOUT, true>), dim3((unsigned)g), dim3(256), 0, s,
                                            (const bf16_t*)x, ldx, N, HW, C, w, g_nchw, (bf16_t*)dx, lddx, part,
                                            (const bf16_t*)bn_y, ld_bny, scale, shift, mean, invstd, bn_partial))
  } else {
    UZ_KOUT_SWITCH(Kout, hipLaunchKernelGGL((outconv_bwd_kernel<bf16_t, KOUT, true, true>), dim3((unsigned)g), dim3(256), 0, s,
                                            (const bf16_t*)nullptr, 0, N, HW, C, w, g_nchw, (bf16_t*)dx, lddx, part,
                                            (const bf16_t*)bn_y, ld_bny, scale, shift, mean, invstd, bn_partial))
  }
  UZ_LAUNCH_CHECK("uz_outconv_bwd_bnred");
  const int ne = Kout * (C + 1);
  hipLaunchKernelGGL(outconv_bwd_finalize_kernel, dim3(uz_cdiv(ne, 32)), dim3(1024), 0, s, part, g, Kout, C, dw, db);
  UZ_LAUNCH_CHECK("uz_outconv_bwd_bnred(finalize)");
  return UZ_OK;
}

extern "C" int uz_outconv_bwd(int dtype, const void* x, int ldx, int N, int HW, int C, const float* w,
                              int Kout, const float* g_nchw, void* dx, int lddx, float* dw, float* db,
                              void* workspace, void* stream) {
  UZ_REQUIRE(dtype == UZ_F32 || dtype == UZ_BF16, "uz_outconv_bwd: bad dtype");
  const int vec = dtype == UZ_BF16 ? 8 : 4;
  UZ_REQUIRE(x && w && g_nchw && dw && db && workspace, "uz_outconv_bwd: null pointer");
  UZ_REQUIRE(Kout >= 1 && Kout <= OUTCONV_MAXK, "uz_outconv_bwd: Kout=%d", Kout);
  UZ_REQUIRE(C % vec == 0 && C / vec <= 64, "uz_outconv_bwd: C=%d unsupported", C);
  UZ_REQUIRE(ldx % vec == 0 && ldx >= C && N > 0 && HW > 0 && (long long)N * HW < (1LL << 31),
             "uz_outconv_bwd: bad shape");
  if (dx) UZ_REQUIRE(lddx % vec == 0 && lddx >= C, "uz_outconv_bwd: bad lddx");
  const int g = outconv_bwd_grid(dtype, N, HW, C);
  float* part = static_cast<float*>(workspace);
  hipStream_t s = (hipStream_t)stream;
  if (dtype == UZ_BF16) {
    UZ_KOUT_SWITCH(Kout, hipLaunchKernelGGL((outconv_bwd_kernel<bf16_t, KOUT>), dim3((unsigned)g), dim3(256), 0, s, (const bf16_t*)x, ldx, N, HW, C, w, g_nchw, (bf16_t*)dx, lddx, part, (const bf16_t*)nullptr, 0, (const float*)nullptr, (const float*)nullptr, (const float*)nullptr, (const float*)nullptr, (float*)nullptr))
  } else {
    UZ_KOUT_SWITCH(Kout, hipLaunchKernelGGL((outconv_bwd_kernel<float, KOUT>), dim3((unsigned)g), dim3(256), 0, s, (const float*)x, ldx, N, HW, C, w, g_nchw, (float*)dx, lddx, part, (const float*)nullptr, 0, (const float*)nullptr, (const float*)nullptr, (const float*)nullptr, (const float*)nullptr, (float*)nullptr))
  }
  UZ_LAUNCH_CHECK("uz_outconv_bwd");
  const int ne = Kout * (C + 1);
  hipLaunchKernelGGL(outconv_bwd_finalize_kernel, dim3(uz_cdiv(ne, 32)), dim3(1024), 0, s, part, g, Kout, C, dw, db);
  UZ_LAUNCH_CHECK("uz_outconv_bwd(finalize)");
  return UZ_OK;
}

extern "C" int uz_colsum(int dtype, const void* x, int ld, int P, int C, float* out, void* stream) {
  UZ_REQUIRE(dtype == UZ_F32 || dtype == UZ_BF16, "uz_colsum: bad dtype");
  const int vec = dtype == UZ_BF16 ? 8 : 4;
  UZ_REQUIRE(x && out && P > 0 && C > 0 && C % vec == 0 && ld % vec == 0 && ld >= C, "uz_colsum: bad args");
  dim3 grid, block;
  reduce_shape(C / vec, P, &grid, &block);
  const size_t shm = (size_t)256 * vec * sizeof(float);
  hipStream_t s = (hipStream_t)stream;
  if (dtype == UZ_BF16)
    hipLaunchKernelGGL((colsum_kernel<bf16_t, false>), grid, block, shm, s, (const bf16_t*)x, ld, (long long)P, C, out);
  else
    hipLaunchKernelGGL((colsum_kernel<float, false>), grid, block, shm, s, (const float*)x, ld, (long long)P, C, out);
  UZ_LAUNCH_CHECK("uz_colsum");
  return UZ_OK;
}

extern "C" long long uz_colsum_workspace_bytes(int dtype, int P, int C) {
  UZ_REQUIRE(dtype == UZ_F32 || dtype == UZ_BF16, "uz_colsum_workspace_bytes: bad dtype");
  const int vec = dtype == UZ_BF16 ? 8 : 4;
  UZ_REQUIRE(P > 0 && C > 0 && C % vec == 0, "uz_colsum_workspace_bytes: bad shape");
  dim3 grid, block;
  reduce_shape(C / vec, P, &grid, &block);
  return (long long)grid.x * C * (long long)sizeof(float);
}

extern "C" int uz_colsum_ws(int dtype, const void* x, int ld, int P, int C, float* out, void* workspace,
                            void* stream) {
  UZ_REQUIRE(dtype == UZ_F32 || dtype == UZ_BF16, "uz_colsum_ws: bad dtype");
  const int vec = dtype == UZ_BF16 ? 8 : 4;
  UZ_REQUIRE(x && out && workspace && P > 0 && C > 0 && C % vec == 0 && ld % vec == 0 && ld >= C, "uz_colsum_ws: bad args");
  dim3 grid, block;
  reduce_shape(C / vec, P, &grid, &block);
  const size_t shm = (size_t)256 * vec * sizeof(float);
  hipStream_t s = (hipStream_t)stream;
  float* part = static_cast<float*>(workspace);
  if (dtype == UZ_BF16)
    hipLaunchKernelGGL((colsum_kernel<bf16_t, true>), grid, block, shm, s, (const bf16_t*)x, ld, (long long)P, C, part);
  else
    hipLaunchKernelGGL((colsum_kernel<float, true>), grid, block, shm, s, (const float*)x, ld, (long long)P, C, part);
  UZ_LAUNCH_CHECK("uz_colsum_ws");
  hipLaunchKernelGGL(colsum_finalize_kernel, dim3(uz_cdiv(C, 32)), dim3(1024), 0, s, part, (int)grid.x, C, out);
  UZ_LAUNCH_CHECK("uz_colsum_ws(finalize)");
  return UZ_OK;
}

extern "C" int uz_colstats_rows(int dtype, int P, int C) {
  UZ_REQUIRE(dtype == UZ_F32 || dtype == UZ_BF16, "uz_colstats_rows: bad dtype");
  const int vec = dtype == UZ_BF16 ? 8 : 4;
  UZ_REQUIRE(P > 0 && C > 0 && C % vec == 0, "uz_colstats_rows: bad shape");
  dim3 grid, block;
  reduce_shape(C / vec, P, &grid, &block, 4);
  return (int)grid.x;
}

extern "C" int uz_colstats(int dtype, const void* x, int ld, int P, int C, float* partial, void* stream) {
  UZ_REQUIRE(dtype == UZ_F32 || dtype == UZ_BF16, "uz_colstats: bad dtype");
  const int vec = dtype == UZ_BF16 ? 8 : 4;
  UZ_REQUIRE(x && partial && P > 0 && C > 0 && C % vec == 0 && ld % vec == 0 && ld >= C, "uz_colstats: bad args");
  dim3 grid, block;
  reduce_shape(C / vec, P, &grid, &block, 4);
  const size_t shm = (size_t)256 * 2 * vec * sizeof(float);
  hipStream_t s = (hipStream_t)stream;
  if (dtype == UZ_BF16)
    hipLaunchKernelGGL((colstats_kernel<bf16_t>), grid, block, shm, s, (const bf16_t*)x, ld, (long long)P, C, partial);
  else
    hipLaunchKernelGGL((colstats_kernel<float>), grid, block, shm, s, (const float*)x, ld, (long long)P, C, partial);
  UZ_LAUNCH_CHECK("uz_colstats");
  return UZ_OK;
}

extern "C" int uz_pack_weights(int dtype, int mode, const float* w, int Co, int Ci, int T, int Kpad,
                               void* dst, void* stream) {
  UZ_REQUIRE(dtype == UZ_F32 || dtype == UZ_BF16, "uz_pack_weights: bad dtype");
  UZ_REQUIRE(w && dst && Co > 0 && Ci > 0 && T > 0, "uz_pack_weights: bad args");
  UZ_REQUIRE(mode >= UZ_PACK_CONV_FWD && mode <= UZ_PACK_IM2COL, "uz_pack_weights: bad mode %d", mode);
  long long total = (long long)Co * Ci * T;
  if (mode == UZ_PACK_IM2COL) {
    UZ_REQUIRE(Kpad >= T * Ci, "uz_pack_weights: Kpad too small");
    total = (long long)Co * Kpad;
  }
  hipStream_t s = (hipStream_t)stream;
  const int grid = grid_for(total, 256);
  if (dtype == UZ_BF16)
    hipLaunchKernelGGL((pack_weights_kernel<bf16_t>), dim3(grid), dim3(256), 0, s, mode, w, Co, Ci, T, Kpad, (bf16_t*)dst, total);
  else
    hipLaunchKernelGGL((pack_weights_kernel<float>), dim3(grid), dim3(256), 0, s, mode, w, Co, Ci, T, Kpad, (float*)dst, total);
  UZ_LAUNCH_CHECK("uz_pack_weights");
  return UZ_OK;
}

template <typename T>
__global__ __launch_bounds__(256) void pack_conv3x3_tiled_kernel(const uz_pack3x3_item* __restrict__ items,
                                                                 int n, int total_tiles) {
  constexpr int TP = 32 * 33 + 4;
  __shared__ float tile[9 * TP];
  for (int gt = blockIdx.x; gt < total_tiles; gt += gridDim.x) {
    int lo = 0, hi = n - 1;
    while (lo < hi) {
      const int mid = (lo + hi + 1) >> 1;
      if (items[mid].tile_begin <= gt) lo = mid; else hi = mid - 1;
    }
    const uz_pack3x3_item it = items[lo];
    const int tl = gt - it.tile_begin;
    const int tiles_ci = it.Ci / 32;
    T* __restrict__ df = static_cast<T*>(it.dst_fwd);
    T* __restrict__ dd = static_cast<T*>(it.dst_dgrad);
    const int co0 = (tl / tiles_ci) * 32, ci0 = (tl % tiles_ci) * 32;
    __syncthreads();
    float stage[36];
#pragma unroll
    for (int i = 0; i < 36; ++i) {
      const int e = threadIdx.x + 256 * i;
      const int co_l = e / 288, r = e - co_l * 288;
      stage[i] = it.src[((size_t)(co0 + co_l) * it.Ci + ci0) * 9 + r];
    }
#pragma unroll
    for (int i = 0; i < 36; ++i) {
      const int e = threadIdx.x + 256 * i;
      const int co_l = e / 288, r = e - co_l * 288;
      const int ci_l = r / 9, tap = r - ci_l * 9;
      tile[tap * TP + co_l * 33 + ci_l] = stage[i];
    }
    __syncthreads();
    constexpr int VEC = ElemTraits<T>::VEC, PPR = 32 / VEC;
    for (int e = threadIdx.x; e < 9 * 32 * PPR; e += 256) {
      const int part = e % PPR, row = e / PPR;
      const int y = row & 31, tap = row >> 5;
// ... 237 lines not shown
```

### unet_zoo_amd/csrc/uz_loss.hip

```cpp
#include "uz_common.h"

namespace {

constexpr int BD_THREADS = 256;
constexpr int BD_MAX_ROWS = 1024;

__global__ __launch_bounds__(BD_THREADS) void bce_dice_kernel(const float* __restrict__ x, const float* __restrict__ t,
                                                              long long n, float inv_n, float* __restrict__ dlogits,
                                                              double* __restrict__ part) {
  double s[4] = {0.0, 0.0, 0.0, 0.0};
  for (long long i = (long long)blockIdx.x * BD_THREADS + threadIdx.x; i < n; i += (long long)gridDim.x * BD_THREADS) {
    const float xv = x[i], tv = t[i];
    const float m = fmaxf(-xv, 0.f);
    s[0] += (double)((1.f - tv) * xv + m + logf(expf(-m) + expf(-xv - m)));
    const float pred = xv > 0.f ? 1.f : 0.f;
    s[1] += (double)(pred * tv);
    s[2] += (double)pred;
    s[3] += (double)tv;
    if (dlogits != nullptr) dlogits[i] = (1.f / (1.f + expf(-xv)) - tv) * inv_n;
  }
  __shared__ double red[BD_THREADS / 64][4];
#pragma unroll
  for (int k = 0; k < 4; ++k) {
    double v = s[k];
    for (int o = 32; o > 0; o >>= 1) v += __shfl_down(v, o);
    if ((threadIdx.x & 63) == 0) red[threadIdx.x >> 6][k] = v;
  }
  __syncthreads();
  if (threadIdx.x < 4) {
    double v = 0.0;
    for (int w = 0; w < BD_THREADS / 64; ++w) v += red[w][threadIdx.x];
    part[(size_t)blockIdx.x * 4 + threadIdx.x] = v;
  }
}

__global__ __launch_bounds__(BD_THREADS) void bce_dice_finalize_kernel(const double* __restrict__ part, int rows,
                                                                       long long n, float* __restrict__ out) {
  __shared__ double red[BD_THREADS][4];
  double s[4] = {0.0, 0.0, 0.0, 0.0};
  for (int r = threadIdx.x; r < rows; r += BD_THREADS)
#pragma unroll
    for (int k = 0; k < 4; ++k) s[k] += part[(size_t)r * 4 + k];
#pragma unroll
  for (int k = 0; k < 4; ++k) red[threadIdx.x][k] = s[k];
  __syncthreads();
  for (int o = BD_THREADS / 2; o > 0; o >>= 1) {
    if ((int)threadIdx.x < o)
#pragma unroll
      for (int k = 0; k < 4; ++k) red[threadIdx.x][k] += red[threadIdx.x + o][k];
    __syncthreads();
  }
  if (threadIdx.x == 0) {
    out[0] = (float)(red[0][0] / (double)n);
    const double uni = red[0][2] + red[0][3];
    out[1] = uni == 0.0 ? 1.f : (float)((2.0 * red[0][1] + 1e-7) / (uni + 1e-7));
  }
}

int bd_rows(long long n) {
  long long r = (n + (long long)BD_THREADS * 8 - 1) / ((long long)BD_THREADS * 8);
  if (r > BD_MAX_ROWS) r = BD_MAX_ROWS;
  if (r < 1) r = 1;
  return (int)r;
}

}

extern "C" long long uz_bce_dice_workspace_bytes(long long n) { return n > 0 ? (long long)bd_rows(n) * 4 * sizeof(double) : -1; }

extern "C" int uz_bce_dice(const float* logits, const float* target, long long n, float* dlogits, float* out2,
                           void* workspace, void* stream) {
  UZ_REQUIRE(logits && target && out2 && workspace && n > 0, "uz_bce_dice: bad arguments");
  const int rows = bd_rows(n);
  hipStream_t s = (hipStream_t)stream;
  hipLaunchKernelGGL(bce_dice_kernel, dim3(rows), dim3(BD_THREADS), 0, s, logits, target, n, 1.f / (float)n, dlogits,
                     (double*)workspace);
  UZ_LAUNCH_CHECK("uz_bce_dice");
  hipLaunchKernelGGL(bce_dice_finalize_kernel, dim3(1), dim3(BD_THREADS), 0, s, (const double*)workspace, rows, n, out2);
  UZ_LAUNCH_CHECK("uz_bce_dice(finalize)");
  return UZ_OK;
}
```

### unet_zoo_amd/engine.py

```python
from __future__ import annotations

import math
from types import SimpleNamespace
from typing import Callable, Dict, List, Optional, Sequence, Tuple

import torch
import torch.nn as nn

from . import _lib as L
from . import ops
from .ops import Act


def _round_up(a: int, b: int) -> int:
    return (a + b - 1) // b * b


def _bias_of(m: nn.Module) -> Optional[torch.Tensor]:
    return m.bias.detach() if m.bias is not None else None


class PackCache:

    def __init__(self):
        self.entries: Dict[tuple, tuple] = {}
        self._table: Optional[torch.Tensor] = None
        self._total = 0
        self._n = 0
        self._table_dtype = None
        self._table3: Optional[torch.Tensor] = None
        self._n3 = 0
        self._tiles3 = 0

    def invalidate(self) -> None:
        self.entries.clear()
        self._table = None

    def repoint(self) -> None:
        self._table = None

    def get(self, p: nn.Parameter, mode: int, kpad: int, dtype: torch.dtype) -> torch.Tensor:
        key = (id(p), mode, kpad, dtype)
        e = self.entries.get(key)
        if e is None:
            if mode == L.PACK_VEC_REPEAT:
                assert p.dtype == torch.float32 and p.is_contiguous(), "PACK_VEC_REPEAT takes a contiguous fp32 vector"
                dst = p.detach().repeat(kpad).contiguous()
            else:
                dst = ops.pack_weights(p.detach(), mode, dtype, kpad)
            self.entries[key] = (p, mode, kpad, dtype, dst)
            self._table = None
            return dst
        return e[4]

    def refresh(self, dtype: torch.dtype) -> None:
        ents = [e for e in self.entries.values() if e[3] == dtype]
        if not ents:
            return
        if self._table is None or self._table_dtype != dtype:
            self._build_tables(ents, dtype)
        lib = L.load()
        if self._n3 > 0:
            L.check(lib.uz_pack_conv3x3_batched(L.dtype_code(dtype), self._table3.data_ptr(), self._n3,
                                                self._tiles3, L.stream_ptr()), "uz_pack_conv3x3_batched")
        if self._n > 0:
            L.check(lib.uz_pack_weights_batched(L.dtype_code(dtype), self._table.data_ptr(), self._n,
                                                self._total, L.stream_ptr()), "uz_pack_weights_batched")

    def _build_tables(self, ents, dtype) -> None:
        dev = ents[0][4].device
        tiled = {}
        generic = []
        for (p, mode, kpad, _, dst) in ents:
            ok = (mode in (L.PACK_CONV_FWD, L.PACK_CONV_DGRAD) and p.dim() == 4 and tuple(p.shape[2:]) == (3, 3)
                  and p.shape[0] % 32 == 0 and p.shape[1] % 32 == 0)
            if ok:
                it = tiled.setdefault(id(p), [p, None, None])
                it[1 if mode == L.PACK_CONV_FWD else 2] = dst
            else:
                generic.append((p, mode, kpad, dst))
        arr3 = (L.Pack3x3Item * max(len(tiled), 1))()
        tb = 0
        for i, (p, df, dd) in enumerate(tiled.values()):
            arr3[i] = L.Pack3x3Item(p.data_ptr(), df.data_ptr() if df is not None else None,
                                    dd.data_ptr() if dd is not None else None, p.shape[0], p.shape[1], tb, 0)
            tb += (p.shape[0] // 32) * (p.shape[1] // 32)
        self._n3, self._tiles3 = len(tiled), tb
        self._table3 = torch.frombuffer(bytearray(bytes(arr3)), dtype=torch.uint8).to(dev)
        arr = (L.PackItem * max(len(generic), 1))()
        begin = 0
        for i, (p, mode, kpad, dst) in enumerate(generic):
            if mode == L.PACK_VEC_REPEAT:
                assert dst.dtype == torch.float32
                arr[i] = L.PackItem(p.data_ptr(), dst.data_ptr(), begin, mode, p.numel(), 1, kpad, 0, 0)
                begin += dst.numel()
                continue
            d0, d1 = p.shape[0], p.shape[1]
            T = p.numel() // (d0 * d1)
            co, ci = (d0, d1) if mode in (L.PACK_CONV_FWD, L.PACK_CONV_DGRAD, L.PACK_IM2COL) else (d1, d0)
            arr[i] = L.PackItem(p.data_ptr(), dst.data_ptr(), begin, mode, co, ci, T, kpad, 0)
            begin += dst.numel()
        self._table = torch.frombuffer(bytearray(bytes(arr)), dtype=torch.uint8).to(dev)
        self._total, self._n, self._table_dtype = begin, len(generic), dtype

class ImageInput:

    __slots__ = ("nchw", "kpad", "dtype", "_patches", "N", "H", "W")

    def __init__(self, nchw: torch.Tensor, kpad: int, dtype: torch.dtype):
        self.nchw, self.kpad, self.dtype, self._patches = nchw, kpad, dtype, None
        self.N, _, self.H, self.W = nchw.shape

    def patches(self) -> Act:
        if self._patches is None:
            self._patches = ops.im2col3x3_nchw(self.nchw, self.kpad, self.dtype)
        return self._patches


class Engine:
    direct_first_conv = True
    defer_linear_wgrads = True
    fuse_bn_reduce = True
    fuse_bn_reduce_convt = True
    fold_bn_apply = True
    fold_bn_apply_head = True
    fold_head_grad = True
    fold_first_bn_bwd = True
    fuse_bn_finalize = False
    FIN_FLAGS = 4096
    reverse_element_passes = True
    fold_bn_eval = False

    def __init__(self, dtype: torch.dtype, device: torch.device, training: bool, record: bool,
                 grad_sink: Optional[Callable[[nn.Parameter, torch.Tensor], None]] = None,
                 pack_cache: Optional[PackCache] = None, grads_in_place: bool = False,
                 fold_bn_eval: Optional[bool] = None):
        if fold_bn_eval is not None:
            self.fold_bn_eval = bool(fold_bn_eval)
        self.folded_layers = 0
        self.unfolded_layers = 0
        self.dtype = dtype
        self.device = device
        self.training = training
        self.record = record
        self.tape: List[Callable[[], None]] = []
        self.param_grads: Dict[nn.Parameter, torch.Tensor] = {}
        self.grad_sink = grad_sink
        self.bk = 64 if dtype == torch.bfloat16 else 32
        self._bn_channels = 0
        self._sums: Optional[torch.Tensor] = None
        self._sums_used = 0
        self._cache = pack_cache if pack_cache is not None else PackCache()
        self.grads_in_place = grads_in_place
        self._heads: List[Tuple[Callable[..., None], int]] = []
        self.grad_log: List[Tuple[int, nn.Parameter]] = []
        self._pending_colsums: List[Tuple[int, nn.Parameter, Act]] = []
        self._pending_rowsums: List[Tuple[int, Callable[[], None]]] = []
        self._pending_wgrads: List[Tuple[int, nn.Parameter, Act, Act]] = []
        self._rowsum_items: list = []
        self._cpb: Dict[nn.Module, dict] = {}
        self._bn_counters: List[torch.Tensor] = []
        self._cur_entry = -1
        self._fin_flags: Optional[torch.Tensor] = None
        self._fin_used = 0

    def _fin_flag(self) -> Optional[torch.Tensor]:
        if not self.fuse_bn_finalize:
            return None
        if self._fin_flags is None:
            self._fin_flags = torch.zeros(self.FIN_FLAGS, dtype=torch.int32, device=self.device)
        if self._fin_used >= self.FIN_FLAGS:
            return None
        self._fin_used += 1
        return self._fin_flags[self._fin_used - 1:self._fin_used]

    def new_act(self, N, H, W, C, needs_grad=True) -> Act:
        return ops.new_act(N, H, W, C, self.dtype, self.device, needs_grad)

    def new_cat(self, N, H, W, channels: Sequence[int]) -> Tuple[Act, List[Act]]:
        full = self.new_act(N, H, W, sum(channels))
        parts, o = [], 0
        for c in channels:
            parts.append(full.window(o, c))
            o += c
        full.parts = parts
        return full, parts

    def _dst(self, p: nn.Parameter) -> Optional[torch.Tensor]:
        if self.grads_in_place and p.grad is not None and p.grad.is_contiguous() and p.grad.dtype == torch.float32:
            return p.grad
        return None

    def _give_grad(self, p: nn.Parameter, g: Optional[torch.Tensor]) -> None:
        if not isinstance(p, nn.Parameter):
            return
        self.grad_log.append((self._cur_entry, p))
        if self.grads_in_place and p.grad is not None:
            if g is None:
                return
            if p in self.param_grads:
                if g.data_ptr() == p.grad.data_ptr():
                    raise RuntimeError("a parameter shared by two layers received its second gradient in place: "
                                       "shared parameters are not supported by the in-place (graphed) backward")
                p.grad.add_(g.reshape(p.grad.shape))
            elif g.data_ptr() != p.grad.data_ptr():
                p.grad.copy_(g.reshape(p.grad.shape))
            self.param_grads[p] = None
            if self.grad_sink is not None:
                self.grad_sink(p, p.grad)
            return
        if g is None:
            g = torch.zeros(p.shape, dtype=torch.float32, device=self.device)
        if p in self.param_grads:
            self.param_grads[p] = self.param_grads[p] + g
        else:
            self.param_grads[p] = g
        if self.grad_sink is not None:
            self.grad_sink(p, self.param_grads[p])

    def _bias_grad(self, p: nn.Parameter, g: Act) -> None:
        self._pending_colsums.append((self._cur_entry, p, g))

    def _linear_wgrad(self, p: nn.Parameter, g: Act, x: Act) -> None:
        if self.defer_linear_wgrads and self.dtype == torch.bfloat16:
            self._pending_wgrads.append((self._cur_entry, p, g, x))
        else:
            self._give_grad(p, ops.wgrad(g, x, tuple(p.shape), ntaps=1, out=self._dst(p)))

    def _after_rowsums(self, fn: Callable[[], None]) -> None:
        self._pending_rowsums.append((self._cur_entry, fn))

    def _flush_rowsums(self) -> None:
        if self._pending_rowsums:
            items, self._rowsum_items = self._rowsum_items, []
            after, self._pending_rowsums = self._pending_rowsums, []
            ops.sum_rows_f32_batched(items)
            cur = self._cur_entry
            for entry, fn in after:
                self._cur_entry = entry
                fn()
            self._cur_entry = cur

    def _flush_colsums(self) -> None:
        self._flush_rowsums()
        wpend, self._pending_wgrads = self._pending_wgrads, []
        if wpend:
            wouts = []
            for _, p, _, _ in wpend:
                dst = self._dst(p)
                wouts.append(dst if dst is not None else torch.empty(tuple(p.shape), dtype=torch.float32, device=self.device))
            ops.wgrad_multi([(g, x, o, 1, L.TAPS_CONV, 1) for (_, _, g, x), o in zip(wpend, wouts)])
            for (entry, p, _, _), o in zip(wpend, wouts):
                self._cur_entry = entry
                self._give_grad(p, o)
        pend, self._pending_colsums = self._pending_colsums, []
        if not pend:
            return
        outs = []
        for _, p, g in pend:
            dst = self._dst(p)
            outs.append(dst if dst is not None else torch.empty(g.C, dtype=torch.float32, device=self.device))
        ops.colsum_batched([(g, o) for (_, _, g), o in zip(pend, outs)])
        for (entry, p, _), o in zip(pend, outs):
            self._cur_entry = entry
            self._give_grad(p, o)

    def _pack(self, p: nn.Parameter, mode: int, kpad: int = 0) -> torch.Tensor:
        return self._cache.get(p, mode, kpad, self.dtype)

    def _bn_sums(self, C: int) -> torch.Tensor:
        if self._sums is None:
            self._sums = torch.empty(2 * self._bn_channels, dtype=torch.float64, device=self.device)
            self._sums_used = 0
        s = self._sums[self._sums_used:self._sums_used + 2 * C].view(2, C)
        self._sums_used += 2 * C
        return s

    def _sum_grads(self, a: Act, limit: int) -> List[Act]:
        gs = list(a.grads)
        while len(gs) > limit:
            x, y = gs.pop(), gs.pop()
            t = self.new_act(x.N, x.H, x.W, x.C)
            ops.add_acts(x, y, t)
            gs.append(t)
        return gs

    def input_im2col(self, x: torch.Tensor) -> "ImageInput":
        L.require_cuda(x)
        if x.dim() != 4:
            raise ValueError(f"expected a (N, C, H, W) input, got shape {tuple(x.shape)}")
        return ImageInput(x.contiguous().float(), _round_up(9 * x.shape[1], self.bk), self.dtype)

    def conv_bn_relu(self, x: Act, conv: nn.Conv2d, bn: nn.BatchNorm2d, *, out: Optional[Act] = None,
                     pool: bool = False, im2col: bool = False, upsample: bool = False,
                     residual: Optional[Act] = None, pool_ceil: bool = False, relu: bool = True,
                     stat_repeat: int = 1, sole_reader: bool = False,
                     defer_apply: Optional[nn.Conv2d] = None) -> Tuple[Act, Optional[Act]]:
        assert not (isinstance(x, Act) and x.lazy is not None) \
            or (sole_reader and not im2col and conv.kernel_size == (3, 3) and conv.dilation == (1, 1)), \
            "a lazy activation goes to the 3x3 convolution it was deferred for"
        xf = x.take_lazy() if isinstance(x, Act) else None
        N, H, W = (x.N, 2 * x.H, 2 * x.W) if upsample else (x.N, x.H, x.W)
        x, image, image_version, wp, ntaps, tmode, dil = self._lower_conv(x, conv, im2col, upsample)
        bare = not pool and residual is None and stat_repeat == 1
        if self.fold_bn_eval and not self.training and not self.record:
            act = self._conv_bn_relu_folded(x, conv, bn, out, image, wp, ntaps, dil, tmode, relu, N, H, W) \
                if (bare and xf is None) else None
            if act is not None:
                self.folded_layers += 1
                return act, None
            self.unfolded_layers += 1
        y = self.new_act(N, H, W, conv.out_channels)
        if image is not None:
            stats = ops.conv_first_fwd(image, conv.weight.detach(), _bias_of(conv), y, self.training)
        else:
            stats = ops.conv_igemm(x, wp, _bias_of(conv), y, ntaps=ntaps, dil=dil, taps_mode=tmode,
                                   want_stats=self.training, xform=xf)
# ... 1260 lines not shown
        cpb = attn.cpb
        pre = self._cpb.get(attn)
        if pre is not None and pre["N"] == N:
            idx, bias = pre["idx"], pre["bias"].view(heads, N, N)
        else:
            pre = None
            w1, b1, w2, b2 = (t.detach() for t in (cpb.fc1.weight, cpb.fc1.bias, cpb.fc2.weight, cpb.fc2.bias))
            idx = attn.log_relative_position_index[:N, :N].reshape(N * N, 2).contiguous()
            bias = ops.cpb_fwd(idx, w1, b1, w2, b2).view(heads, N, N)
        tau = attn.tau.detach()
        o = self.new_act(x.N, x.H, x.W, x.C)
        lse = ops.winattn_fwd(qkv, tau, bias, o, heads, ws, shift, scale=attn.scale)
        if self.record:
            def bwd():
                g = self._total_grad(o)
                if g is None:
                    return
                dqkv = self.new_act(qkv.N, qkv.H, qkv.W, qkv.C)
                whole = tuple(attn.tau.shape) == (heads, N, N)
                late = pre is not None and whole
                dbias, dtau = ops.winattn_bwd(qkv, tau, bias, o, lse, g, dqkv, heads, ws, shift,
                                              dtau=self._dst(attn.tau) if whole else None, scale=attn.scale,
                                              defer=self._rowsum_items if late else None)
                qkv.add_grad(dqkv)
                if late:
                    def give():
                        self._give_grad(attn.tau, dtau)
                        pre["G"] = dbias.view(heads, N * N)
                    self._after_rowsums(give)
                    return
                if not whole:
                    full = torch.zeros_like(attn.tau)
                    full[:, :N, :N] = dtau
                    dtau = full
                self._give_grad(attn.tau, dtau)
                if pre is not None:
                    pre["G"] = dbias.view(heads, N * N)
                    return
                gs = []
                for p_ in (cpb.fc1.weight, cpb.fc1.bias, cpb.fc2.weight, cpb.fc2.bias):
                    d_ = self._dst(p_)
                    gs.append(d_ if d_ is not None else torch.empty(p_.shape, dtype=torch.float32, device=self.device))
                ops.cpb_bwd(idx, w1, b1, w2, dbias.view(heads, N * N), *gs)
                for p_, g_ in zip((cpb.fc1.weight, cpb.fc1.bias, cpb.fc2.weight, cpb.fc2.bias), gs):
                    self._give_grad(p_, g_)

            self.tape.append(bwd)
        return self.dropout(self.linear(o, attn.proj), attn.proj_drop.p)

    def resize_bilinear(self, x: Act, out: Act, align_corners: bool = False) -> Act:
        assert x.N == out.N and x.C == out.C
        ops.bilinear_fwd(x, out, align_corners)
        if self.record and x.needs_grad:
            def bwd():
                gs = self._sum_grads(out, 1)
                if not gs:
                    return
                dx = self.new_act(x.N, x.H, x.W, x.C)
                ops.bilinear_bwd(gs[0], dx, align_corners)
                x.add_grad(dx)

            self.tape.append(bwd)
        return out

    def copy_into(self, src: Act, dst: Act) -> Act:
        assert (src.N, src.H, src.W, src.C) == (dst.N, dst.H, dst.W, dst.C) and src.dtype == dst.dtype
        ops.resample2(src, dst, ops.RESAMPLE_COPY)
        if self.record and src.needs_grad:
            def bwd():
                g = self._total_grad(dst)
                if g is not None:
                    src.add_grad(g)

            self.tape.append(bwd)
        return dst

    def u2net_heads(self, feats: Sequence[Act], sides: Sequence[nn.Conv2d], fuse: nn.Conv2d) -> List[torch.Tensor]:
        N, H, W = feats[0].N, feats[0].H, feats[0].W
        S, K, HW = len(feats), sides[0].out_channels, H * W
        assert fuse.kernel_size == (1, 1) and fuse.in_channels == S * K and fuse.out_channels == K
        dev = self.device
        dcat = torch.empty((N, S * K, H, W), dtype=torch.float32, device=dev)
        taps = torch.empty(N * 9 * HW, dtype=torch.float32, device=dev)
        for s_, (f, conv) in enumerate(zip(feats, sides)):
            assert conv.kernel_size == (3, 3) and conv.padding == (1, 1) and conv.in_channels == f.C
            wt = conv.weight.detach()
            hw = f.H * f.W
            low = None if (f.H, f.W) == (H, W) else torch.empty((N, K, f.H, f.W), dtype=torch.float32, device=dev)
            for o in range(K):
                wp = wt.data_ptr() + o * f.C * 9 * 4
                bp = conv.bias.detach().data_ptr() + 4 * o if conv.bias is not None else None
                plane = dcat.data_ptr() + (s_ * K + o) * HW * 4
                if low is None:
                    ops.sideconv_fwd(f, wp, bp, taps, plane, S * K * HW)
                else:
                    lp = low.data_ptr() + o * hw * 4
                    ops.sideconv_fwd(f, wp, bp, taps, lp, K * hw)
                    ops.bilinear_planes(lp, K * hw, f.H, f.W, plane, S * K * HW, H, W, N)
        wf = fuse.weight.detach().reshape(K, S * K)
        d0 = ops.fuse1x1_fwd(dcat, wf, _bias_of(fuse))
        outs = [d0] + [dcat[:, s_ * K:(s_ + 1) * K] for s_ in range(S)]

        if self.record:
            def bwd(*gs: Optional[torch.Tensor]):
                if all(g is None for g in gs):
                    return
                g0 = gs[0].contiguous().float() if gs[0] is not None else None
                extras = [g.contiguous().float() if g is not None else None for g in gs[1:]]
                dwf, dbf = self._dst(fuse.weight), (self._dst(fuse.bias) if fuse.bias is not None else None)
                if dwf is None:
                    dwf = torch.empty(fuse.weight.shape, dtype=torch.float32, device=dev)
                if dbf is None and fuse.bias is not None:
                    dbf = torch.empty(K, dtype=torch.float32, device=dev)
                dcat_g = ops.fuse1x1_bwd(dcat, wf, g0, extras, dwf, dbf)
                self._give_grad(fuse.weight, dwf)
                if fuse.bias is not None:
                    self._give_grad(fuse.bias, dbf)
                for s_, (f, conv) in enumerate(zip(feats, sides)):
                    hw = f.H * f.W
                    dw, db = self._dst(conv.weight), (self._dst(conv.bias) if conv.bias is not None else None)
                    if dw is None:
                        dw = torch.empty(conv.weight.shape, dtype=torch.float32, device=dev)
                    if db is None and conv.bias is not None:
                        db = torch.empty(K, dtype=torch.float32, device=dev)
                    low = None if (f.H, f.W) == (H, W) else torch.empty((N, K, f.H, f.W), dtype=torch.float32, device=dev)
                    wt = conv.weight.detach()
                    for o in range(K):
                        plane = dcat_g.data_ptr() + (s_ * K + o) * HW * 4
                        if low is None:
                            gp_, gi = plane, S * K * HW
                        else:
                            gp_, gi = low.data_ptr() + o * hw * 4, K * hw
                            ops.bilinear_planes(plane, S * K * HW, f.H, f.W, gp_, gi, H, W, N, backward=True)
                        dx = self.new_act(f.N, f.H, f.W, f.C) if f.needs_grad else None
                        ops.sideconv_bwd(f, wt.data_ptr() + o * f.C * 9 * 4, gp_, gi, dx,
                                         dw.data_ptr() + o * f.C * 9 * 4,
                                         db.data_ptr() + 4 * o if db is not None else None)
                        if dx is not None:
                            f.add_grad(dx)
                    self._give_grad(conv.weight, dw)
                    if conv.bias is not None:
                        self._give_grad(conv.bias, db)

            self._heads.append((bwd, len(outs)))
        return outs

    def out_conv(self, x: Act, conv: nn.Conv2d, sole_reader: bool = False) -> torch.Tensor:
        assert conv.kernel_size == (1, 1) and conv.in_channels == x.C
        K = conv.out_channels
        w = conv.weight.detach().reshape(K, x.C)
        b = conv.bias.detach() if conv.bias is not None else torch.zeros(K, device=self.device)
        assert x.lazy is None or sole_reader, "a lazy activation goes to the head it was deferred for"
        xf = x.take_lazy()
        logits = ops.outconv_fwd(x, w, b, xform=xf)
        if self.record:
            def bwd(g_logits: torch.Tensor):
                dwt = self._dst(conv.weight)
                dbt = self._dst(conv.bias) if conv.bias is not None else None
                src = x.bn_src if (sole_reader and (self.fuse_bn_reduce_convt or xf is not None)) else None
                gl = g_logits.contiguous().float()
                virt = (xf is not None and self.fold_head_grad and src is not None and self.training
                        and not self.fuse_bn_finalize and ops.bn_bwd_head_supported(src[0], K))
                dx = self.new_act(x.N, x.H, x.W, x.C) if ((x.needs_grad or xf is not None) and not virt) else None
                if virt:
                    dw, db, part = ops.outconv_bwd(x, w, gl, None, dwt.view(K, x.C) if dwt is not None else None, dbt,
                                                   bnred=src, lazy=True, store_dx=False)
                else:
                    dw, db = ops.outconv_bwd(x, w, gl, dx, dwt.view(K, x.C) if dwt is not None else None, dbt, bnred=src,
                                             lazy=xf is not None)
                self._give_grad(conv.weight, dwt if dwt is not None else dw.reshape(conv.weight.shape))
                if conv.bias is not None:
                    self._give_grad(conv.bias, db)
                if virt:
                    x.add_grad(ops.HeadGrad(gl, w, part))
                elif dx is not None:
                    x.add_grad(dx)

            self._heads.append((bwd, 1))
        return logits

    def out_conv_resized(self, x: Act, conv: nn.Conv2d, H: int, W: int, align_corners: bool = True) -> torch.Tensor:
        low = self.out_conv(x, conv)
        N, K, h, w = low.shape
        logits = torch.empty((N, K, H, W), dtype=torch.float32, device=low.device)
        ops.bilinear_planes_ac(low.data_ptr(), h, w, logits.data_ptr(), H, W, N * K, align_corners)
        if self.record:
            inner, n = self._heads.pop()

            def bwd(g_logits: torch.Tensor):
                g_low = torch.empty((N, K, h, w), dtype=torch.float32, device=low.device)
                ops.bilinear_planes_ac(g_logits.contiguous().float().data_ptr(), h, w, g_low.data_ptr(), H, W, N * K,
                                       align_corners, backward=True)
                inner(g_low)

            self._heads.append((bwd, n))
        return logits

    def layer_norm_head(self, x: Act, ln: nn.LayerNorm, conv: nn.Conv2d, *, mode: int = L.LN_PLAIN, r: int = 1) -> torch.Tensor:
        C, K = ln.normalized_shape[0], conv.out_channels
        assert conv.kernel_size == (1, 1) and conv.in_channels == C
        if not ops.ln_head_supported(C, K, self.dtype):
            return self.out_conv(self.layer_norm(x, ln, mode=mode, r=r), conv)
        if mode == L.LN_EXPAND:
            assert x.C == r * r * C
            N, Ho, Wo = x.N, x.H * r, x.W * r
        else:
            assert mode == L.LN_PLAIN and x.C == C
            N, Ho, Wo = x.N, x.H, x.W
        gamma, beta = ln.weight.detach(), ln.bias.detach()
        w = conv.weight.detach().reshape(K, C)
        b = _bias_of(conv)
        logits, stats = ops.ln_head_fwd(x, gamma, beta, w, b, N, Ho, Wo, C, mode=mode, r=r, eps=ln.eps)
        if self.record:
            def bwd(g_logits: torch.Tensor):
                dx = self.new_act(x.N, x.H, x.W, x.C)
                dwt = self._dst(conv.weight)
                outs = ops.ln_head_bwd(x, gamma, beta, w, stats, g_logits.contiguous().float(), dx, mode=mode, r=r,
                                       eps=ln.eps, dgamma=self._dst(ln.weight), dbeta=self._dst(ln.bias),
                                       dw=dwt.view(K, C) if dwt is not None else None,
                                       db=self._dst(conv.bias) if conv.bias is not None else None)
                self._give_grad(conv.weight, dwt if dwt is not None else outs[2].reshape(conv.weight.shape))
                if conv.bias is not None:
                    self._give_grad(conv.bias, outs[3])
                self._give_grad(ln.weight, outs[0])
                self._give_grad(ln.bias, outs[1])
                if x.needs_grad:
                    x.add_grad(dx)

            self._heads.append((bwd, 1))
        return logits

    def conv5x5(self, x: Act, conv: nn.Conv2d) -> Tuple[Act, torch.Tensor]:
        assert conv.kernel_size == (5, 5) and conv.padding == (2, 2) and conv.stride == (1, 1) and conv.dilation == (1, 1) \
            and conv.groups == 1 and conv.in_channels == x.C
        N, H, W, Cout = x.N, x.H, x.W, conv.out_channels
        thin = Cout % 8 != 0
        if thin:
            y = Act(torch.zeros((x.P, _round_up(Cout, 8)), dtype=self.dtype, device=self.device), 0, Cout, N, H, W)
        else:
            y = self.new_act(N, H, W, Cout)
        stats = ops.conv5x5(x, self._pack(conv.weight, L.PACK_CONV_FWD), _bias_of(conv), y, want_stats=True)
        if self.record:
            def bwd():
                g = self._total_grad(y)
                if g is None:
                    return
                if conv.bias is not None:
                    self._give_grad(conv.bias, None)
                if thin:
                    assert g.off == 0 and g.ld == _round_up(Cout, 8)
                    g = Act(g.buf, 0, g.ld, N, H, W)
                self._give_grad(conv.weight, ops.wgrad5x5(g, x, tuple(conv.weight.shape), out=self._dst(conv.weight)))
                if x.needs_grad:
                    if thin:
                        wd = torch.zeros((x.C, 25, g.C), dtype=torch.float32, device=self.device)
                        wd[:, :, :Cout] = conv.weight.detach().flip(2, 3).reshape(Cout, x.C, 25).permute(1, 2, 0)
                        wd = wd.reshape(x.C, 25 * g.C).to(self.dtype)
                    else:
                        wd = self._pack(conv.weight, L.PACK_CONV_DGRAD)
                    dx = self.new_act(N, H, W, x.C)
                    ops.conv5x5(g, wd, None, dx)
                    x.add_grad(dx)

            self.tape.append(bwd)
        return y, stats

    def bn_elu(self, raw: Act, bn: nn.Module, stats: Optional[torch.Tensor] = None, *, act1: bool = True, act2: bool = False,
               res: Optional[Act] = None, out: Optional[Act] = None, out2: Optional[Act] = None,
               mask2: Optional[torch.Tensor] = None, pad_grad: bool = False) -> Act:
        N, H, W, C = raw.N, raw.H, raw.W, raw.C
        if raw.P <= 1:
            raise ValueError(f"Expected more than 1 value per channel when training, got input size {(N, C, H, W)}")
        if stats is None:
            stats = ops.colstats(raw)
        vec = ops.bn_finalize(stats, raw.P, bn.weight.detach(), bn.bias.detach(), bn.eps, self._momentum(bn, count=False),
                              bn.running_mean, bn.running_var)
        if out is None:
            out = Act(torch.zeros_like(raw.buf), 0, C, N, H, W) if pad_grad else self.new_act(N, H, W, C)
        ops.bn_elu_apply(raw, vec[0], vec[1], out, act1=act1, act2=act2, res=res, out2=out2, mask2=mask2)
        if self.record:
            self._bn_channels += C

            def bwd():
                gs = self._sum_grads(out, 2)
                g2 = self._sum_grads(out2, 1)[0] if (out2 is not None and out2.grads) else None
                if not gs and g2 is None:
                    return
                if not gs:
                    z = self.new_act(N, H, W, C)
                    z.buf.zero_()
                    gs = [z]
                if pad_grad:
                    dx = Act(torch.zeros_like(raw.buf), 0, C, N, H, W)
                else:
                    dx = self.new_act(N, H, W, C)
                gres = self.new_act(N, H, W, C) if (res is not None and res.needs_grad) else None
                dgamma, dbeta = self._bn_grad_dst(bn, C)
                ops.bn_elu_bwd(raw, vec, out, gs[0], gs[1] if len(gs) > 1 else None, g2, mask2, self._bn_sums(C), dx, gres,
                               dgamma, dbeta, act1=act1, act2=act2)
                self._give_grad(bn.weight, dgamma)
                self._give_grad(bn.bias, dbeta)
                if gres is not None:
                    res.add_grad(gres)
                if raw.needs_grad:
                    raw.add_grad(dx)

            self.tape.append(bwd)
        return out

    def logits_from(self, x: Act) -> torch.Tensor:
        logits = x.buf[:, x.off:x.off + x.C].float().reshape(x.N, x.H, x.W, x.C).permute(0, 3, 1, 2).contiguous()
        if self.record:
            def bwd(g_logits: torch.Tensor):
                gb = torch.zeros((x.P, x.ld), dtype=self.dtype, device=self.device)
                gb[:, :x.C] = g_logits.permute(0, 2, 3, 1).reshape(x.P, x.C)
                x.add_grad(Act(gb, 0, x.C, x.N, x.H, x.W))

            self._heads.append((bwd, 1))
        return logits

    def backward(self, grad_outputs: Sequence[Optional[torch.Tensor]]) -> Dict[nn.Parameter, torch.Tensor]:
        self.backward_range(grad_outputs, len(self.tape), 0)
        self.tape.clear()
        return self.param_grads

    def backward_range(self, grad_outputs: Optional[Sequence[Optional[torch.Tensor]]], hi: int, lo: int) -> None:
        if grad_outputs is not None:
            self._cur_entry = len(self.tape)
            gl, pos, calls = list(grad_outputs), 0, []
            for fn, n in self._heads:
                calls.append((fn, gl[pos:pos + n]))
                pos += n
            assert pos == len(gl)
# ... 9 lines not shown
```

### unet_zoo_amd/graph.py

```python
from __future__ import annotations

import os
from typing import Callable, List, Optional, Sequence, Tuple

import torch
import torch.nn as nn

from . import _lib as L
from .engine import Engine, PackCache

_DTYPES = {"bf16": torch.bfloat16, "bfloat16": torch.bfloat16, "fp32": torch.float32,
           "float32": torch.float32}
_default_dtype = _DTYPES[os.environ.get("UNET_ZOO_AMD_DTYPE", "bf16").lower()]


def set_default_dtype(dtype) -> None:
    global _default_dtype
    _default_dtype = _DTYPES[dtype.lower()] if isinstance(dtype, str) else dtype
    L.dtype_code(_default_dtype)


def get_default_dtype() -> torch.dtype:
    return _default_dtype


class _GraphFn(torch.autograd.Function):
    @staticmethod
    def forward(ctx, model: "HipModule", plist: List[nn.Parameter], record: bool, x: torch.Tensor,
                *params: torch.Tensor):
        model._pack_cache.refresh(model.run_dtype)
        eng = Engine(model.run_dtype, x.device, model.training, record, model._grad_sink,
                     model._pack_cache, model.grads_in_place)
        outs = model.emit(eng, x)
        eng.finish_forward()
        ctx.eng = eng if record else None
        ctx.plist = plist
        ctx.sink_done = model._grad_sink_done
        return tuple(outs)

    @staticmethod
    def backward(ctx, *grad_outputs):
        eng = ctx.eng
        if eng is None:
            raise RuntimeError("backward through a HipModule forward that ran without gradient recording")
        grads = eng.backward(grad_outputs)
        ctx.eng = None
        if ctx.sink_done is not None:
            ctx.sink_done(grads)
        out = []
        for i, p in enumerate(ctx.plist):
            out.append(grads.get(p) if ctx.needs_input_grad[4 + i] else None)
        grads.clear()
        return (None, None, None, None, *out)


class HipModule(nn.Module):

    def __init__(self):
        super().__init__()
        self.run_dtype: torch.dtype = get_default_dtype()
        self._grad_sink: Optional[Callable] = None
        self._grad_sink_done: Optional[Callable] = None
        self._pack_cache = PackCache()
        self.grads_in_place = False

    def _apply(self, fn, *args, **kwargs):
        self._pack_cache.invalidate()
        return super()._apply(fn, *args, **kwargs)

    def emit(self, eng: Engine, x: torch.Tensor) -> Sequence[torch.Tensor]:
        raise NotImplementedError

    def wrap_outputs(self, outs: Tuple[torch.Tensor, ...]):
        return outs[0]

    def forward(self, x: torch.Tensor):
        L.load()
        L.require_cuda(x)
        if x.requires_grad:
            raise NotImplementedError("gradients with respect to the input image are not produced")
        plist = list(self.parameters())
        record = torch.is_grad_enabled() and any(p.requires_grad for p in plist)
        outs = _GraphFn.apply(self, plist, record, x, *plist)
        return self.wrap_outputs(outs)


class PhasedStep:

    def __init__(self, model: HipModule, loss_fn: Callable):
        self.model = model
        self.loss_fn = loss_fn
        self.eng: Optional[Engine] = None
        self._gouts: Optional[Tuple[Optional[torch.Tensor], ...]] = None

    def forward(self, x: torch.Tensor, target: torch.Tensor) -> torch.Tensor:
        self.emit(x)
        return self.loss(target)

    def emit(self, x: torch.Tensor):
        m = self.model
        L.load()
        L.require_cuda(x)
        m._pack_cache.refresh(m.run_dtype)
        self.eng = Engine(m.run_dtype, x.device, m.training, True, None, m._pack_cache, True)
        with torch.no_grad():
            self._outs = tuple(m.emit(self.eng, x))
            self.eng.finish_forward()
        self.outputs = m.wrap_outputs(tuple(o.detach() for o in self._outs))
        return self.outputs

    def loss(self, target: torch.Tensor) -> torch.Tensor:
        direct = getattr(self.loss_fn, "direct", None)
        if direct is not None:
            res = direct(self.model.wrap_outputs(tuple(o.detach() for o in self._outs)), target)
            loss, gouts = res[0], res[-1]
            assert len(gouts) == len(self._outs)
            self._gouts = tuple(gouts)
            return loss.detach()
        leaves = tuple(o.detach().requires_grad_(True) for o in self._outs)
        with torch.enable_grad():
            loss = self.loss_fn(self.model.wrap_outputs(leaves), target)
            self._gouts = torch.autograd.grad(loss, leaves, allow_unused=True)
        return loss.detach()

    def set_output_grads(self, gouts: Sequence[Optional[torch.Tensor]]) -> None:
        self._gouts = tuple(gouts)

    @property
    def n_entries(self) -> int:
        return len(self.eng.tape)

    def backward(self, hi: int, lo: int, heads: bool) -> None:
        self.eng.backward_range(self._gouts if heads else None, hi, lo)

    def finish(self) -> None:
        self.eng.tape.clear()
        self.eng = None
        self._gouts = None
        self._outs = None

    def plan(self, fractions: Sequence[float] = (0.45, 0.85)):
        log = self.eng.grad_log
        n = self.n_entries
        last: dict = {}
        for pos, p in log:
            last[p] = pos if p not in last else min(last[p], pos)
        order = sorted(last.items(), key=lambda kv: -kv[1])
        total = sum(p.numel() for p, _ in order)
        cuts, groups, cur, acc, fi = [n], [], [], 0, 0
        fr = list(fractions)
        for idx, (p, pos) in enumerate(order):
            cur.append(p)
            acc += p.numel()
            nxt = order[idx + 1][1] if idx + 1 < len(order) else None
            if fi < len(fr) and acc >= fr[fi] * total and nxt is not None and nxt < pos:
                cuts.append(pos)
                groups.append(cur)
                cur = []
                while fi < len(fr) and acc >= fr[fi] * total:
                    fi += 1
        cuts.append(0)
        cur += [p for p in self.model.parameters() if p not in last and p.grad is not None]
        groups.append(cur)
        return cuts, groups
```

### unet_zoo_amd/loss.py

```python
from __future__ import annotations

from typing import Optional, Tuple

import torch

from . import _lib as L


class _BceDice(torch.autograd.Function):
    @staticmethod
    def forward(ctx, logits: torch.Tensor, target: torch.Tensor):
        L.require_cuda(logits, target)
        assert logits.shape == target.shape, (logits.shape, target.shape)
        x = logits.detach().contiguous().float()
        t = target.detach().contiguous().float()
        n = x.numel()
        lib = L.load()
        need_grad = ctx.needs_input_grad[0]
        dlogits = torch.empty_like(x) if need_grad else None
        out = torch.empty(2, dtype=torch.float32, device=x.device)
        ws = torch.empty(L.check_count(lib.uz_bce_dice_workspace_bytes(n), "uz_bce_dice_workspace_bytes") // 8,
                         dtype=torch.float64, device=x.device)
        L.check(lib.uz_bce_dice(x.data_ptr(), t.data_ptr(), n, dlogits.data_ptr() if need_grad else None, out.data_ptr(),
                                ws.data_ptr(), L.stream_ptr()), "uz_bce_dice")
        ctx.dlogits = dlogits
        ctx.in_dtype = logits.dtype
        dice = out[1]
        ctx.mark_non_differentiable(dice)
        return out[0], dice

    @staticmethod
    def backward(ctx, g_loss, _g_dice):
        return (ctx.dlogits * g_loss).to(ctx.in_dtype), None


def bce_dice_direct(logits: torch.Tensor, target: torch.Tensor):
    L.require_cuda(logits, target)
    assert logits.shape == target.shape, (logits.shape, target.shape)
    x = logits.detach().contiguous().float()
    t = target.detach().contiguous().float()
    n = x.numel()
    lib = L.load()
    dlogits = torch.empty_like(x)
    out = torch.empty(2, dtype=torch.float32, device=x.device)
    ws = torch.empty(L.check_count(lib.uz_bce_dice_workspace_bytes(n), "uz_bce_dice_workspace_bytes") // 8,
                     dtype=torch.float64, device=x.device)
    L.check(lib.uz_bce_dice(x.data_ptr(), t.data_ptr(), n, dlogits.data_ptr(), out.data_ptr(), ws.data_ptr(),
                            L.stream_ptr()), "uz_bce_dice")
    return out[0], out[1], dlogits


def loss_and_dice_direct(outputs, target: torch.Tensor):
    if isinstance(outputs, dict):
        trip = [bce_dice_direct(v, target) for v in outputs.values()]
        return sum(p[0] for p in trip), trip[0][1], tuple(p[2] for p in trip)
    if isinstance(outputs, (list, tuple)):
        trip = [bce_dice_direct(v, target) for v in outputs]
        return sum(p[0] for p in trip), trip[-1][1], tuple(p[2] for p in trip)
    l, d, g = bce_dice_direct(outputs, target)
    return l, d, (g,)


def bce_dice_with_logits(logits: torch.Tensor, target: torch.Tensor) -> Tuple[torch.Tensor, torch.Tensor]:
    return _BceDice.apply(logits, target)


def loss_and_dice(outputs, target: torch.Tensor) -> Tuple[torch.Tensor, torch.Tensor]:
    if isinstance(outputs, dict):
        pairs = [bce_dice_with_logits(v, target) for v in outputs.values()]
        return sum(p[0] for p in pairs), pairs[0][1]
    if isinstance(outputs, (list, tuple)):
        pairs = [bce_dice_with_logits(v, target) for v in outputs]
        return sum(p[0] for p in pairs), pairs[-1][1]
    return bce_dice_with_logits(outputs, target)


_REDUCES = ("batch", "image", "channel")


def _maps_of(outputs):
    if isinstance(outputs, dict):
        return tuple(outputs.keys()), tuple(outputs.values()), 0
    if isinstance(outputs, (list, tuple)):
        return None, tuple(outputs), len(outputs) - 1
    return None, (outputs,), 0


class _RegionFn(torch.autograd.Function):

    @staticmethod
    def forward(ctx, crit: "RegionLoss", target: torch.Tensor, weights: tuple, main: int, *logits: torch.Tensor):
        loss, dice, dl = crit._launch(logits, target, weights, main, ctx.needs_input_grad[4:])
        ctx.dl = dl
        ctx.in_dtypes = tuple(v.dtype for v in logits)
        ctx.mark_non_differentiable(dice)
        return loss, dice

    @staticmethod
    def backward(ctx, g_loss, _g_dice):
        return (None, None, None, None) + tuple(None if d is None else (d * g_loss).to(dt)
                                                for d, dt in zip(ctx.dl, ctx.in_dtypes))


class RegionLoss:

    def __init__(self, w_bce: float = 1.0, w_region: float = 1.0, alpha: float = 0.5, beta: float = 0.5,
                 smooth: float = 1.0, gamma: float = 1.0, reduce: str = "image", pos_weight=None, output_weights=None):
        def num(name, v):
            try:
                f = float(v)
            except (TypeError, ValueError):
                raise ValueError(f"RegionLoss: {name} must be a number, got {v!r}") from None
            if f != f or f in (float("inf"), float("-inf")):
                raise ValueError(f"RegionLoss: {name} must be finite, got {v!r}")
            return f
        self.w_bce, self.w_region = num("w_bce", w_bce), num("w_region", w_region)
        self.alpha, self.beta = num("alpha", alpha), num("beta", beta)
        self.smooth, self.gamma = num("smooth", smooth), num("gamma", gamma)
        self.pos_weight = 1.0 if pos_weight is None else num("pos_weight", pos_weight)
        if self.smooth <= 0:
            raise ValueError(f"RegionLoss: smooth must be > 0, got {smooth!r}")
        if self.gamma < 1:
            raise ValueError(f"RegionLoss: gamma must be >= 1, got {gamma!r}")
        if self.alpha < 0 or self.beta < 0:
            raise ValueError(f"RegionLoss: alpha and beta must be >= 0, got {alpha!r}, {beta!r}")
        if self.w_bce < 0 or self.w_region < 0:
            raise ValueError(f"RegionLoss: w_bce and w_region must be >= 0, got {w_bce!r}, {w_region!r}")
        if self.w_bce == 0 and self.w_region == 0:
            raise ValueError("RegionLoss: w_bce and w_region are both zero")
        if self.pos_weight <= 0:
            raise ValueError(f"RegionLoss: pos_weight must be > 0, got {pos_weight!r}")
        if reduce not in _REDUCES:
            raise ValueError(f"RegionLoss: reduce must be one of {_REDUCES}, got {reduce!r}")
        self.reduce = reduce
        if output_weights is None:
            self.output_weights = None
        elif isinstance(output_weights, dict):
            self.output_weights = {k: num(f"output_weights[{k!r}]", v) for k, v in output_weights.items()}
        else:
            self.output_weights = tuple(num(f"output_weights[{i}]", v) for i, v in enumerate(output_weights))
        if self.output_weights is not None:
            vals = self.output_weights.values() if isinstance(self.output_weights, dict) else self.output_weights
            if any(v < 0 for v in vals):
                raise ValueError(f"RegionLoss: output_weights must be >= 0, got {output_weights!r}")
        self._plans = {}

    @classmethod
    def dice(cls, smooth: float = 1.0, **kw) -> "RegionLoss":
        return cls(alpha=0.5, beta=0.5, smooth=float(smooth) / 2.0, **kw)

    @classmethod
    def tversky(cls, alpha: float, beta: float, **kw) -> "RegionLoss":
        return cls(alpha=alpha, beta=beta, **kw)

    def weights_for(self, outputs) -> tuple:
        keys, maps, _ = _maps_of(outputs)
        ow = self.output_weights
        if ow is None:
            return (1.0,) * len(maps)
        if isinstance(ow, dict):
            if keys is None:
                raise ValueError("RegionLoss: output_weights is a dict but the outputs are not")
            missing = [k for k in keys if k not in ow]
            if missing:
                raise ValueError(f"RegionLoss: output_weights has no entry for the outputs {missing}")
            return tuple(ow[k] for k in keys)
        if len(ow) != len(maps):
            raise ValueError(f"RegionLoss: {len(ow)} output_weights for {len(maps)} output maps")
        return ow

    def _groups(self, shape) -> int:
        if self.reduce == "batch":
            return 1
        if len(shape) < 2:
            raise ValueError(f"RegionLoss: reduce={self.reduce!r} needs (N, K, ...) maps, got shape {tuple(shape)}")
        return int(shape[0]) if self.reduce == "image" else int(shape[0]) * int(shape[1])

    def _plan(self, n_items: int, shape, device: torch.device, main: int):
        key = (n_items, tuple(shape), device.index, main)
        plan = self._plans.get(key)
        if plan is None:
            if n_items > L.REGION_MAX_ITEMS:
                raise ValueError(f"RegionLoss: {n_items} output maps, at most {L.REGION_MAX_ITEMS} per call")
            n = 1
            for s in shape:
                n *= int(s)
            desc = L.RegionDesc(n_items, n, self._groups(shape), self.w_bce, self.w_region, self.alpha, self.beta,
                                self.smooth, self.gamma, self.pos_weight, main)
            ws = torch.empty((L.region_loss_workspace_bytes(desc) + 7) // 8, dtype=torch.float64, device=device)
            plan = self._plans[key] = (desc, (L.RegionItem * n_items)(), ws)
        return plan

    def _launch(self, logits, target: torch.Tensor, weights, main: int, need):
        L.require_cuda(target, *logits)
        for v in logits:
            if v.shape != target.shape:
                raise ValueError(f"RegionLoss: an output map of shape {tuple(v.shape)} against a target of shape "
                                 f"{tuple(target.shape)}")
            if v.dtype not in (torch.float32, torch.bfloat16):
                raise ValueError(f"RegionLoss: logits must be float32 or bfloat16, got {v.dtype}")
            if v.device != target.device:
                raise ValueError(f"RegionLoss: an output map on {v.device} against a target on {target.device}")
        if target.numel() == 0:
            raise ValueError("RegionLoss: empty maps")
        xs = [v.detach().contiguous().float() for v in logits]
        t = target.detach().contiguous().float()
        desc, items, ws = self._plan(len(xs), t.shape, t.device, main)
        dl = [torch.empty_like(x) if g else None for x, g in zip(xs, need)]
        out = torch.empty(2, dtype=torch.float32, device=t.device)
        for it, x, d, w in zip(items, xs, dl, weights):
            it.logits, it.target, it.dlogits, it.weight = x.data_ptr(), t.data_ptr(), (d.data_ptr() if d is not None else None), w
        L.region_loss(desc, items, out, ws)
        return out[0], out[1], dl
# ... 203 lines not shown
```

### unet_zoo_amd/ops.py

```python
from __future__ import annotations

import ctypes
import math
from ctypes import byref
from typing import List, Optional, Sequence

import torch

from . import _lib as L


class Act:

    __slots__ = ("buf", "off", "C", "N", "H", "W", "grads", "parts", "rparts", "needs_grad", "colsums", "bn_src",
                 "bn_partials", "lazy", "_taken")

    def __init__(self, buf: torch.Tensor, off: int, C: int, N: int, H: int, W: int, needs_grad: bool = True):
        assert buf.dim() == 2 and buf.is_contiguous() and buf.shape[0] == N * H * W
        assert 0 <= off and off + C <= buf.shape[1]
        self.buf, self.off, self.C, self.N, self.H, self.W = buf, off, C, N, H, W
        self.grads: List["Act"] = []
        self.parts: Optional[Sequence["Act"]] = None
        self.rparts: Optional[Sequence[tuple]] = None
        self.needs_grad = needs_grad
# ... 483 lines not shown
    with _Timed("relu_bwd", 0.0, out.buf.element_size() * out.P * out.C * 3):
        L.check(L.load().uz_relu_bwd(L.dtype_code(out.dtype), out.ptr(), out.ld, g.ptr(), g.ld, dx.ptr(), dx.ld, out.P,
                                     out.C, L.stream_ptr()), "uz_relu_bwd")


def bn_eval_scale(gamma, beta, running_mean, running_var, eps: float):
    lib = L.load()
    C = gamma.numel()
    vec = torch.empty((2, C), dtype=torch.float32, device=gamma.device)
    L.check(lib.uz_bn_eval_scale(C, gamma.data_ptr(), beta.data_ptr(), running_mean.data_ptr(),
                                 running_var.data_ptr(), eps, vec[0].data_ptr(), vec[1].data_ptr(),
                                 L.stream_ptr()), "uz_bn_eval_scale")
    return vec


def bn_relu_apply(y: Act, scale: torch.Tensor, shift: torch.Tensor, act: Act,
                  pooled: Optional[Act] = None, res: Optional[Act] = None, pool_ceil: bool = False,
                  relu: bool = True, reverse: bool = False) -> None:
    if pooled is not None:
        want = ((y.H + 1) // 2, (y.W + 1) // 2) if pool_ceil else (y.H // 2, y.W // 2)
        assert (pooled.H, pooled.W) == want, (pooled.H, pooled.W, want)
    lib = L.load()
    es = y.buf.element_size()
    with _Timed("bn_relu_apply", 0.0, es * y.P * y.C * ((2.25 if pooled is not None else 2.0) + (res is not None))):
        L.check(lib.uz_bn_relu_add_apply(L.dtype_code(y.dtype), y.ptr(), y.ld, scale.data_ptr(),
                                         shift.data_ptr(), y.N, y.H, y.W, y.C,
                                         res.ptr() if res is not None else None,
                                         res.ld if res is not None else 0, act.ptr(), act.ld,
                                         pooled.ptr() if pooled is not None else None,
                                         pooled.ld if pooled is not None else 0,
                                         int(pool_ceil) | (0 if relu else 2) | (4 if reverse else 0), L.stream_ptr()),
                "uz_bn_relu_add_apply")


def bn_relu_apply_fin(y: Act, stats: torch.Tensor, count: int, gamma, beta, eps: float, momentum: float, running_mean,
                      running_var, flag: torch.Tensor, act: Act, pooled: Optional[Act] = None, res: Optional[Act] = None,
                      pool_ceil: bool = False, relu: bool = True) -> torch.Tensor:
    if pooled is not None:
        want = ((y.H + 1) // 2, (y.W + 1) // 2) if pool_ceil else (y.H // 2, y.W // 2)
        assert (pooled.H, pooled.W) == want, (pooled.H, pooled.W, want)
    C = stats.shape[2]
    assert C == y.C and flag.dtype == torch.int32 and flag.numel() == 1
    vec = torch.empty((4, C), dtype=torch.float32, device=stats.device)
    es = y.buf.element_size()
    with _Timed("bn_relu_apply", 0.0, es * y.P * y.C * ((2.25 if pooled is not None else 2.0) + (res is not None)) + 4.0 * stats.numel()):
        L.check(L.load().uz_bn_relu_add_apply_fin(
            L.dtype_code(y.dtype), y.ptr(), y.ld, stats.data_ptr(), stats.shape[0], float(count), gamma.data_ptr(), beta.data_ptr(),
            eps, momentum, _p(running_mean), _p(running_var), vec.data_ptr(), flag.data_ptr(), y.N, y.H, y.W, y.C,
            res.ptr() if res is not None else None, res.ld if res is not None else 0, act.ptr(), act.ld,
            pooled.ptr() if pooled is not None else None, pooled.ld if pooled is not None else 0,
            int(pool_ceil) | (0 if relu else 2), L.stream_ptr()), "uz_bn_relu_add_apply_fin")
    return vec


BN_BWD_ALTERNATE = True


def bn_relu_bwd(y: Act, vec: torch.Tensor, g0: Optional[Act], g1: Optional[Act],
                gpool: Optional[Act], sums: torch.Tensor, dy: Optional[Act], dgamma: torch.Tensor,
                dbeta: torch.Tensor, pool_ceil: bool = False, relu: bool = True,
                partials: Optional[torch.Tensor] = None, frozen: bool = False,
                fin_flag: Optional[torch.Tensor] = None, reverse: bool = False) -> None:
    lib = L.load()
    assert dy is not None or (fin_flag is None and not frozen)
    def desc(rev):
        return L.BnBwdDesc(L.dtype_code(y.dtype), y.N, y.H, y.W, y.C, y.ld,
                           g0.ld if g0 is not None else 0, g1.ld if g1 is not None else 0,
                           gpool.ld if gpool is not None else 0, dy.ld if dy is not None else 0,
                           int(pool_ceil) | (0 if relu else 2) | (4 if rev else 0))
    d = desc(reverse)
    d_apply = desc(reverse != (partials is None and BN_BWD_ALTERNATE))
    args = (y.ptr(), vec[0].data_ptr(), vec[1].data_ptr(), vec[2].data_ptr(), vec[3].data_ptr(),
            g0.ptr() if g0 is not None else None, g1.ptr() if g1 is not None else None,
            gpool.ptr() if gpool is not None else None)
    s = L.stream_ptr()
    nsrc = (g0 is not None) + (g1 is not None) + 0.25 * (gpool is not None)
    es = y.buf.element_size()
    if fin_flag is not None and not frozen:
        if partials is not None:
            assert relu and g1 is None and gpool is None and partials.shape[1:] == (2, y.C) and partials.is_contiguous()
            rows, pptr = partials.shape[0], partials.data_ptr()
        else:
            wsb = L.check_count(lib.uz_bn_relu_bwd_workspace_bytes(byref(d), int(gpool is not None)),
                                "uz_bn_relu_bwd_workspace_bytes")
            ws = torch.empty(wsb // 4, dtype=torch.float32, device=y.buf.device)
            rows, pptr = wsb // (8 * y.C), ws.data_ptr()
            with _Timed("bn_relu_bwd_reduce", 0.0, es * y.P * y.C * (1 + nsrc)):
                L.check(lib.uz_bn_relu_bwd_reduce_rows(byref(d), *args, pptr, s), "uz_bn_relu_bwd_reduce_rows")
        with _Timed("bn_relu_bwd_apply", 0.0, es * y.P * y.C * (2 + nsrc)):
            L.check(lib.uz_bn_relu_bwd_apply_fin(byref(d_apply), *args, pptr, rows, sums.data_ptr(), dgamma.data_ptr(),
                                                 dbeta.data_ptr(), fin_flag.data_ptr(), float(y.P), dy.ptr(), s),
                    "uz_bn_relu_bwd_apply_fin")
        return
    if partials is not None:
        assert relu and g1 is None and gpool is None and partials.shape[1:] == (2, y.C) and partials.is_contiguous()
        L.check(lib.uz_bn_bwd_finalize(partials.data_ptr(), partials.shape[0], y.C, sums.data_ptr(),
                                       dgamma.data_ptr(), dbeta.data_ptr(), s), "uz_bn_bwd_finalize")
    else:
        wsb = L.check_count(lib.uz_bn_relu_bwd_workspace_bytes(byref(d), int(gpool is not None)),
                            "uz_bn_relu_bwd_workspace_bytes")
        ws = torch.empty(wsb // 4, dtype=torch.float32, device=y.buf.device)
        with _Timed("bn_relu_bwd_reduce", 0.0, es * y.P * y.C * (1 + nsrc)):
            L.check(lib.uz_bn_relu_bwd_reduce(byref(d), *args, ws.data_ptr(), sums.data_ptr(),
                                              dgamma.data_ptr(), dbeta.data_ptr(), s), "uz_bn_relu_bwd_reduce")
    if dy is None:
        return
    if frozen:
        sums.zero_()
    with _Timed("bn_relu_bwd_apply", 0.0, es * y.P * y.C * (2 + nsrc)):
        L.check(lib.uz_bn_relu_bwd_apply(byref(d_apply), *args, sums.data_ptr(), float(y.P), dy.ptr(), s),
                "uz_bn_relu_bwd_apply")


class HeadGrad:
    __slots__ = ("g", "w", "bn_partials")

    def __init__(self, g: torch.Tensor, w: torch.Tensor, bn_partials: torch.Tensor):
        self.g, self.w, self.bn_partials = g, w, bn_partials


def bn_bwd_head_supported(y: Act, K: int) -> bool:
    return bool(L.load().uz_bn_relu_bwd_apply_head_supported(L.dtype_code(y.dtype), y.C, K)) and y.ld % 8 == 0


def bn_relu_bwd_head(y: Act, vec: torch.Tensor, hg: HeadGrad, sums: torch.Tensor, dy: Act, dgamma: torch.Tensor,
                     dbeta: torch.Tensor, reverse: bool = False) -> None:
    lib = L.load()
    K = hg.w.shape[0]
    parts = hg.bn_partials
    assert hg.g.dtype == torch.float32 and hg.g.is_contiguous() and hg.g.shape == (y.N, K, y.H, y.W)
    assert hg.w.dtype == torch.float32 and hg.w.is_contiguous() and hg.w.shape == (K, y.C)
    assert parts.shape[1:] == (2, y.C) and parts.is_contiguous() and bn_bwd_head_supported(y, K)
    s = L.stream_ptr()
    L.check(lib.uz_bn_bwd_finalize(parts.data_ptr(), parts.shape[0], y.C, sums.data_ptr(), dgamma.data_ptr(),
                                   dbeta.data_ptr(), s), "uz_bn_bwd_finalize")
    d = L.BnBwdDesc(L.dtype_code(y.dtype), y.N, y.H, y.W, y.C, y.ld, 0, 0, 0, dy.ld, 4 if reverse else 0)
    es = y.buf.element_size()
    with _Timed("bn_relu_bwd_apply_head", 2.0 * K * y.P * y.C, es * y.P * y.C * 2 + 4.0 * K * y.P):
        L.check(lib.uz_bn_relu_bwd_apply_head(byref(d), y.ptr(), vec[0].data_ptr(), vec[1].data_ptr(), vec[2].data_ptr(),
                                              vec[3].data_ptr(), hg.g.data_ptr(), hg.w.data_ptr(), K, sums.data_ptr(),
                                              float(y.P), dy.ptr(), s), "uz_bn_relu_bwd_apply_head")


def outconv_xform_supported(x: Act, K: int) -> bool:
    return x.dtype == torch.bfloat16 and x.C % 8 == 0 and x.C // 8 <= 64 and 1 <= K <= 8 and x.ld % 8 == 0


def outconv_fwd(x: Act, w: torch.Tensor, b: torch.Tensor, xform: Optional[tuple] = None) -> torch.Tensor:
    lib = L.load()
    K = w.shape[0]
    out = torch.empty((x.N, K, x.H, x.W), dtype=torch.float32, device=x.buf.device)
    if xform is not None:
        assert outconv_xform_supported(x, K)
        L.check(lib.uz_outconv_fwd_xf(L.dtype_code(x.dtype), x.raw_ptr(), x.ld, x.N, x.H * x.W, x.C, xform[0].data_ptr(),
                                      xform[1].data_ptr(), w.data_ptr(), b.data_ptr(), K, out.data_ptr(), L.stream_ptr()),
                "uz_outconv_fwd_xf")
        return out
    L.check(lib.uz_outconv_fwd(L.dtype_code(x.dtype), x.ptr(), x.ld, x.N, x.H * x.W, x.C,
                               w.data_ptr(), b.data_ptr(), K, out.data_ptr(), L.stream_ptr()),
            "uz_outconv_fwd")
    return out


def outconv_bwd(x: Act, w: torch.Tensor, g: torch.Tensor, dx: Optional[Act],
                dw: Optional[torch.Tensor] = None, db: Optional[torch.Tensor] = None,
                bnred: Optional[tuple] = None, lazy: bool = False, store_dx: bool = True):
    lib = L.load()
    K = w.shape[0]
    assert g.dtype == torch.float32 and g.is_contiguous() and g.shape == (x.N, K, x.H, x.W)
    dev = x.buf.device
    if dw is None:
        dw = torch.empty((K, x.C), dtype=torch.float32, device=dev)
    if db is None:
        db = torch.empty(K, dtype=torch.float32, device=dev)
    code = L.dtype_code(x.dtype)
    wsb = L.check_count(lib.uz_outconv_bwd_workspace_bytes(code, x.N, x.H * x.W, x.C, K),
                        "uz_outconv_bwd_workspace_bytes")
    ws = torch.empty(wsb // 4, dtype=torch.float32, device=dev)
    if lazy:
        assert bnred is not None and (dx is not None) == store_dx and x.dtype == torch.bfloat16 and (bnred[0].P, bnred[0].C) == (x.P, x.C), \
            "a head on a lazy activation takes its backward through uz_outconv_bwd_bnred"
    assert store_dx or lazy
    if bnred is not None and (dx is not None or not store_dx) and x.dtype == torch.bfloat16 and (bnred[0].P, bnred[0].C) == (x.P, x.C):
        bn_y, vec4 = bnred
        rows = L.check_count(lib.uz_outconv_bwd_rows(code, x.N, x.H * x.W, x.C), "uz_outconv_bwd_rows")
        part = torch.empty((rows, 2, x.C), dtype=torch.float32, device=dev)
        L.check(lib.uz_outconv_bwd_bnred(code, None if lazy else x.ptr(), x.ld, x.N, x.H * x.W, x.C, w.data_ptr(), K, g.data_ptr(),
                                         dx.ptr() if store_dx else None, dx.ld if store_dx else 0, dw.data_ptr(), db.data_ptr(),
                                         ws.data_ptr(), bn_y.ptr(), bn_y.ld,
                                         vec4[0].data_ptr(), vec4[1].data_ptr(), vec4[2].data_ptr(), vec4[3].data_ptr(),
                                         part.data_ptr(), L.stream_ptr()), "uz_outconv_bwd_bnred")
        if not store_dx:
            return dw.view(K, x.C), db, part
        dx.bn_partials = part
        return dw.view(K, x.C), db
    L.check(lib.uz_outconv_bwd(code, x.ptr(), x.ld, x.N, x.H * x.W, x.C, w.data_ptr(), K, g.data_ptr(),
                               dx.ptr() if dx is not None else None,
                               dx.ld if dx is not None else 0, dw.data_ptr(), db.data_ptr(),
                               ws.data_ptr(), L.stream_ptr()), "uz_outconv_bwd")
    return dw.view(K, x.C), db


def colsum(x: Act, out: Optional[torch.Tensor] = None) -> torch.Tensor:
    lib = L.load()
    code = L.dtype_code(x.dtype)
    if out is None:
        out = torch.empty(x.C, dtype=torch.float32, device=x.buf.device)
    assert out.numel() == x.C and out.dtype == torch.float32 and out.is_contiguous()
    wsb = L.check_count(lib.uz_colsum_workspace_bytes(code, x.P, x.C), "uz_colsum_workspace_bytes")
    ws = torch.empty(wsb // 4, dtype=torch.float32, device=x.buf.device)
    with _Timed("colsum", 0.0, x.buf.element_size() * x.P * x.C):
        L.check(lib.uz_colsum_ws(code, x.ptr(), x.ld, x.P, x.C, out.data_ptr(), ws.data_ptr(), L.stream_ptr()),
                "uz_colsum_ws")
    return out


def colsum_batched(pairs: Sequence) -> None:
    by_dtype = {}
    for x, out in pairs:
        assert out.numel() == x.C and out.dtype == torch.float32 and out.is_contiguous()
        by_dtype.setdefault(x.dtype, []).append((x, out))
    lib = L.load()
    for dt, group in by_dtype.items():
        arr = (L.ColsumItem * len(group))()
        nbytes = 0.0
        for i, (x, out) in enumerate(group):
            arr[i] = L.ColsumItem(x.ptr(), out.data_ptr(), x.P, x.C, x.ld, 0)
            nbytes += x.buf.element_size() * x.P * x.C
        code = L.dtype_code(dt)
        wsb = L.check_count(lib.uz_colsum_batched_workspace_bytes(code, arr, len(group)), "uz_colsum_batched_workspace_bytes")
        ws = torch.empty(max(wsb // 4, 1), dtype=torch.float32, device=group[0][0].buf.device)
        with _Timed("colsum_batched", 0.0, nbytes):
            L.check(lib.uz_colsum_batched(code, arr, len(group), ws.data_ptr(), L.stream_ptr()), "uz_colsum_batched")


def sum_rows(partial: torch.Tensor, rows: int, n: int) -> torch.Tensor:
    out = torch.empty(n, dtype=torch.float64, device=partial.device)
    L.check(L.load().uz_sum_rows(partial.data_ptr(), rows, n, out.data_ptr(), L.stream_ptr()), "uz_sum_rows")
    return out


def sum_rows_f32_batched(entries: Sequence) -> None:
    if not entries:
        return
    arr = (L.SumRowsItem * len(entries))()
    for i, (partial, rows, out0, out1) in enumerate(entries):
        n0 = out0.numel()
        n = n0 + (out1.numel() if out1 is not None else 0)
        assert partial.numel() == rows * n and partial.dtype == torch.float32
        arr[i] = L.SumRowsItem(partial.data_ptr(), out0.data_ptr(), out1.data_ptr() if out1 is not None else None, rows, n, n0, 0)
    with _Timed("sum_rows_batched", 0.0, 4.0 * sum(e[0].numel() for e in entries)):
        L.check(L.load().uz_sum_rows_f32_batched(arr, len(entries), L.stream_ptr()), "uz_sum_rows_f32_batched")


def sum_rows_f32(partial: torch.Tensor, rows: int, out0: torch.Tensor, out1: Optional[torch.Tensor] = None,
                 defer: Optional[list] = None) -> None:
    if defer is not None:
        defer.append((partial, rows, out0, out1))
        return
    n0 = out0.numel()
    n = n0 + (out1.numel() if out1 is not None else 0)
    assert partial.numel() == rows * n and partial.dtype == torch.float32
    for o in (out0, out1):
        assert o is None or (o.dtype == torch.float32 and o.is_contiguous())
    L.check(L.load().uz_sum_rows_f32(partial.data_ptr(), rows, n, out0.data_ptr(), n0,
                                     out1.data_ptr() if out1 is not None else None, L.stream_ptr()), "uz_sum_rows_f32")


def attn_grid(dtype: torch.dtype, P: int, channels: int) -> int:
    return L.check_count(L.load().uz_attn_grid(L.dtype_code(dtype), P, channels), "uz_attn_grid")


def attn_psi_fwd(g1: Act, x1: Act, vec_g, vec_x, wpsi: torch.Tensor, bpsi: Optional[torch.Tensor]):
    dev = g1.buf.device
    G = attn_grid(g1.dtype, g1.P, g1.C)
    q = torch.empty(g1.P, dtype=torch.float32, device=dev)
    part = torch.empty((G, 2, 1), dtype=torch.float32, device=dev)
    with _Timed("attn_psi_fwd", 0.0, g1.buf.element_size() * 2.0 * g1.P * g1.C):
        L.check(L.load().uz_attn_psi_fwd(L.dtype_code(g1.dtype), g1.ptr(), g1.ld, x1.ptr(), x1.ld,
                                         vec_g.data_ptr(), vec_x.data_ptr(), wpsi.data_ptr(), _p(bpsi),
                                         g1.P, g1.C, q.data_ptr(), part.data_ptr(), L.stream_ptr()),
                "uz_attn_psi_fwd")
    return q, part


def attn_gate_fwd(x: Act, q: torch.Tensor, vec_q: torch.Tensor, out: Act) -> None:
    with _Timed("attn_gate_fwd", 0.0, x.buf.element_size() * 2.0 * x.P * x.C):
        L.check(L.load().uz_attn_gate_fwd(L.dtype_code(x.dtype), x.ptr(), x.ld, q.data_ptr(), vec_q.data_ptr(),
                                          x.P, x.C, out.ptr(), out.ld, L.stream_ptr()), "uz_attn_gate_fwd")


def attn_bwd_psi(dout: Act, x: Act, q: torch.Tensor, vec_q: torch.Tensor, dxd: Act):
    dev = x.buf.device
    G = attn_grid(x.dtype, x.P, x.C)
    dz = torch.empty(x.P, dtype=torch.float32, device=dev)
    part = torch.empty((G, 2), dtype=torch.float32, device=dev)
    with _Timed("attn_bwd_psi", 0.0, x.buf.element_size() * 3.0 * x.P * x.C):
        L.check(L.load().uz_attn_bwd_psi(L.dtype_code(x.dtype), dout.ptr(), dout.ld, x.ptr(), x.ld, q.data_ptr(),
                                         vec_q.data_ptr(), x.P, x.C, dxd.ptr(), dxd.ld, dz.data_ptr(),
                                         part.data_ptr(), L.stream_ptr()), "uz_attn_bwd_psi")
    return dz, sum_rows(part, G, 2)


def attn_bwd_branches(g1: Act, x1: Act, q, dz, wpsi, vec_g, vec_x, vec_q, a01, dg1: Act, dx1: Act,
                      frozen: bool = False) -> torch.Tensor:
    lib = L.load()
    F_, P = g1.C, g1.P
    G = attn_grid(g1.dtype, P, F_)
    part = torch.empty((G, 4 * F_ + 1), dtype=torch.float32, device=g1.buf.device)
    code = L.dtype_code(g1.dtype)
    a01_k = torch.zeros_like(a01) if frozen else a01
    common = (code, g1.ptr(), g1.ld, x1.ptr(), x1.ld, q.data_ptr(), dz.data_ptr(), wpsi.data_ptr(),
              vec_g.data_ptr(), vec_x.data_ptr(), vec_q.data_ptr(), a01_k.data_ptr())
    es = g1.buf.element_size()
    with _Timed("attn_bwd_reduce", 0.0, es * 2.0 * P * F_):
        L.check(lib.uz_attn_bwd_reduce(*common, P, F_, part.data_ptr(), L.stream_ptr()), "uz_attn_bwd_reduce")
    tot = sum_rows(part, G, 4 * F_ + 1)
    tot_k = tot
    if frozen:
        tot_k = tot.clone()
        tot_k[:3 * F_].zero_()
    with _Timed("attn_bwd_apply", 0.0, es * 4.0 * P * F_):
        L.check(lib.uz_attn_bwd_apply(*common, tot_k.data_ptr(), P, F_, dg1.ptr(), dg1.ld, dx1.ptr(), dx1.ld,
                                      L.stream_ptr()), "uz_attn_bwd_apply")
    return tot


def sum2x2(du: Act, dx: Act) -> None:
    with _Timed("sum2x2", 0.0, du.buf.element_size() * 1.25 * du.P * du.C):
        L.check(L.load().uz_sum2x2(L.dtype_code(du.dtype), du.ptr(), du.ld, dx.N, dx.H, dx.W, dx.C, dx.ptr(),
                                   dx.ld, L.stream_ptr()), "uz_sum2x2")


def bilinear_fwd(x: Act, out: Act, align_corners: bool = False) -> None:
    assert x.N == out.N and x.C == out.C and x.dtype == out.dtype
    es = x.buf.element_size()
    with _Timed("bilinear_fwd", 0.0, es * (x.P + out.P) * x.C):
        L.check(L.load().uz_resize_bilinear_fwd(L.dtype_code(x.dtype), x.ptr(), x.ld, x.H * x.W * x.ld, x.N, x.H, x.W,
                                                x.C, out.ptr(), out.ld, out.H * out.W * out.ld, out.H, out.W,
                                                int(align_corners), L.stream_ptr()), "uz_resize_bilinear_fwd")


def bilinear_bwd(g: Act, dx: Act, align_corners: bool = False) -> None:
    assert g.N == dx.N and g.C == dx.C and g.dtype == dx.dtype
    es = g.buf.element_size()
    with _Timed("bilinear_bwd", 0.0, es * (g.P + dx.P) * g.C):
        L.check(L.load().uz_resize_bilinear_bwd(L.dtype_code(g.dtype), g.ptr(), g.ld, g.H * g.W * g.ld, g.N, dx.H, dx.W,
                                                g.C, dx.ptr(), dx.ld, dx.H * dx.W * dx.ld, g.H, g.W,
                                                int(align_corners), L.stream_ptr()), "uz_resize_bilinear_bwd")


RESAMPLE_COPY, RESAMPLE_SUBSAMPLE, RESAMPLE_ZERO_INSERT = 0, 1, 2

# ... 591 lines not shown
```

### unet_zoo_amd/step.py

```python
from __future__ import annotations

from typing import Callable, Dict, List, Optional, Sequence, Tuple, Union

import torch
import torch.distributed as dist
import torch.nn as nn

from .graph import HipModule, PhasedStep
from .loss import MulticlassLoss, RegionLoss, loss_and_dice, loss_and_dice_direct
from .optim import FlatClipAdamW

CAPTURE_MODE = "thread_local"


_HIP = None


def _memset_nodes(graph: "torch.cuda.CUDAGraph") -> Optional[int]:
    global _HIP
    import ctypes
    try:
        raw = graph.raw_cuda_graph()
        if _HIP is None:
            _HIP = ctypes.CDLL("libamdhip64.so")
# ... 7 lines not shown
            return None
        count = 0
        for i in range(n.value):
            t = ctypes.c_int(-1)
            if _HIP.hipGraphNodeGetType(ctypes.c_void_p(nodes[i]), ctypes.byref(t)) != 0:
                return None
            if t.value == 2:
                count += 1
        return count
    except Exception:
        return None


def _new_graph() -> "torch.cuda.CUDAGraph":
    try:
        return torch.cuda.CUDAGraph(keep_graph=True)
    except TypeError:
        return torch.cuda.CUDAGraph()


def _check_capture(graph: "torch.cuda.CUDAGraph", what: str) -> None:
    n = _memset_nodes(graph)
    if n:
        raise RuntimeError(f"GraphedStep: the captured {what} contains {n} memset node(s); on this stack a replayed "
                           f"memset node acts only once (DESIGN.md 5a) -- a library reduction / zero-fill by "
                           f"hipMemsetAsync was captured.  Keep it out of the graph (criterion as a callable runs "
                           f"eagerly) or replace it with a kernel.")


def _unwrap(model: nn.Module) -> HipModule:
    inner = model.module if hasattr(model, "module") and isinstance(model.module, HipModule) else model
    if not isinstance(inner, HipModule):
        raise TypeError(f"GraphedStep needs a unet_zoo_amd model (HipModule), got {type(model).__name__}")
    return inner


class _ShapeGraphs:
    __slots__ = ("x", "t", "fwd", "phases", "gouts", "loss", "dice", "outputs", "pool", "ps")


class GraphedStep:
    def __init__(self, model: nn.Module, criterion: Union[str, RegionLoss, MulticlassLoss, Callable] = "bce_dice", *, lr: float = 1e-4,
                 betas: Tuple[float, float] = (0.9, 0.999), eps: float = 1e-8, weight_decay: float = 1e-5,
                 max_norm: float = 1.0, phases: int = 5, process_group=None, data_parallel: Optional[bool] = None,
                 cu_reserve: Optional[int] = None, comm: str = "overlap", comm_dtype: Optional[torch.dtype] = None):
        self.model = _unwrap(model)
        if cu_reserve is not None:
            from . import _lib
            _lib.set_cu_reserve(cu_reserve)
        if isinstance(criterion, str):
            if criterion != "bce_dice":
                raise ValueError(f"unknown built-in criterion {criterion!r}; pass 'bce_dice' or a callable")
            self._fused_loss = True
            self._loss_fn = lambda out, t: loss_and_dice(out, t)[0]
            self._fused = (loss_and_dice, loss_and_dice_direct)
        elif isinstance(criterion, (RegionLoss, MulticlassLoss)):
            self._fused_loss = True
            self._loss_fn = lambda out, t: criterion.loss_and_dice(out, t)[0]
            self._fused = (criterion.loss_and_dice, criterion.direct)
        else:
            self._fused_loss = False
            self._loss_fn = criterion
        self._target_dtype = getattr(criterion, "target_dtype", torch.float32)
        self.lr, self.betas, self.eps, self.weight_decay, self.max_norm = lr, betas, eps, weight_decay, max_norm
        self.pg = process_group
        self.world = dist.get_world_size(process_group) if dist.is_initialized() else 1
        self.distributed = (self.world > 1) if data_parallel is None else bool(data_parallel)
        if self.distributed and not dist.is_initialized():
            raise RuntimeError("data_parallel=True needs an initialised torch.distributed process group")
        self._nccl = self.distributed and dist.get_backend(process_group) == "nccl"
        self.n_phases = max(1, int(phases)) if self.distributed else 1
        if comm not in ("overlap", "tail"):
            raise ValueError(f"comm must be 'overlap' or 'tail', got {comm!r}")
        self.comm = comm
        if comm_dtype not in (None, torch.float32, torch.bfloat16):
            raise ValueError(f"comm_dtype must be None, torch.float32 or torch.bfloat16, got {comm_dtype!r}")
        self.comm_dtype = torch.bfloat16 if comm_dtype == torch.bfloat16 else torch.float32
        self._comm_stream: Optional[torch.cuda.Stream] = None
        self._comm_bufs: Dict[tuple, tuple] = {}
        self.opt: Optional[FlatClipAdamW] = None
        self._g_opt: Optional[torch.cuda.CUDAGraph] = None
        self._cuts: Optional[List[int]] = None
        self._spans: List[Tuple[int, int]] = []
        self._graphs: Dict[tuple, _ShapeGraphs] = {}
        self._cur: Optional[_ShapeGraphs] = None
        self.loss: Optional[torch.Tensor] = None
        self.dice: Optional[torch.Tensor] = None
        self.outputs = None
        self.steps_done = 0

    def _dry_run(self, x: torch.Tensor, t: torch.Tensor):
        m = self.model
        saved = [b.detach().clone() for b in m.buffers()]
        rng = torch.cuda.get_rng_state(x.device)
        for p in m.parameters():
            p.grad = None
        ps = PhasedStep(m, self._loss_fn)
        side = torch.cuda.Stream(device=x.device)
        side.wait_stream(torch.cuda.current_stream())
        with torch.cuda.stream(side):
            ps.forward(x, t)
            ps.backward(ps.n_entries, 0, True)
            K = self.n_phases
            fr = [0.85 * (i + 1) / (K - 1) for i in range(K - 1)] if K > 1 else []
            cuts, groups = ps.plan(fr)
            ps.finish()
        torch.cuda.current_stream().wait_stream(side)
        torch.cuda.synchronize(x.device)
        for b, s in zip(m.buffers(), saved):
            b.copy_(s)
        torch.cuda.set_rng_state(rng, x.device)
        return cuts, groups

    def _setup(self, x: torch.Tensor, t: torch.Tensor) -> None:
        m = self.model
        if not m.training:
            raise RuntimeError("GraphedStep is the TRAINING step: call model.train() first "
                               "(evaluate with model.eval() and torch.no_grad() as the reference does)")
        cuts, groups = self._dry_run(x, t)
        ordered = [p for grp in groups for p in grp]
        if not ordered:
            raise RuntimeError("no parameter received a gradient")
        self.opt = FlatClipAdamW(ordered, lr=self.lr, betas=self.betas, eps=self.eps,
                                 weight_decay=self.weight_decay, max_norm=self.max_norm)
        m._pack_cache.repoint()
        m._pack_cache.refresh(m.run_dtype)
        A, off = FlatClipAdamW.ALIGN, 0
        self._spans = []
        for grp in groups:
            k = sum((p.numel() + A - 1) // A * A for p in grp)
            self._spans.append((off, off + k))
            off += k
        assert off == self.opt.n
        self._cuts = cuts
        if self.world > 1:
            self._broadcast(self.opt.flat_p)
            for b in m.buffers():
                self._broadcast(b)
        self._capture_opt()

    def _capture_opt(self) -> None:
        self._g_opt = _new_graph()
        with torch.cuda.graph(self._g_opt, capture_error_mode=CAPTURE_MODE):
            self.opt.step()
        _check_capture(self._g_opt, "optimizer graph")

    def set_lr(self, lr: float) -> None:
        self.lr = lr
        if self.opt is not None:
            self.opt.lr = lr
            torch.cuda.synchronize()
            self._capture_opt()

    def _capture(self, x: torch.Tensor, t: torch.Tensor) -> _ShapeGraphs:
        g = _ShapeGraphs()
        g.x, g.t = x, t
        ps = PhasedStep(self.model, self._loss_fn)
        cuts = self._cuts
        g.phases, g.fwd, g.gouts, g.dice, pool = [], None, None, None, None
        torch.cuda.synchronize()
        if self._fused_loss:
            dice_box = []
            with_autograd, direct = self._fused

            def fused(out, tt):
                l, d = with_autograd(out, tt)
                dice_box.append(d)
                return l

            def fused_direct(out, tt):
                l, d, gouts = direct(out, tt)
                dice_box.append(d)
                return l, gouts
            fused.direct = fused_direct
            ps.loss_fn = fused
        else:
            g.fwd = _new_graph()
            with torch.cuda.graph(g.fwd, capture_error_mode=CAPTURE_MODE):
                ps.emit(g.x)
            _check_capture(g.fwd, "forward graph")
            pool = g.fwd.pool()
            g.outputs = ps.outputs
            g.gouts = [torch.zeros_like(o) for o in ps._outs]
            ps.set_output_grads(g.gouts)
        for k in range(len(cuts) - 1):
            gk = _new_graph()
            with torch.cuda.graph(gk, pool=pool, capture_error_mode=CAPTURE_MODE):
                if k == 0 and self._fused_loss:
                    g.loss = ps.forward(g.x, g.t)
                    g.outputs = ps.outputs
                    g.dice = dice_box[-1].detach()
                ps.backward(cuts[k], cuts[k + 1], k == 0)
            _check_capture(gk, f"backward phase {k}")
            pool = gk.pool()
            g.phases.append(gk)
        g.ps = ps
        if self._fused_loss:
            ps.finish()
        else:
            ps.eng.tape.clear()
            ps.eng = None
        g.pool = pool
        return g

    def _broadcast(self, t: torch.Tensor) -> None:
        if self._nccl:
            dist.broadcast(t, src=0, group=self.pg)
        else:
            h = t.detach().cpu()
            dist.broadcast(h, src=0, group=self.pg)
            t.copy_(h)

    class _EventWait:

        def __init__(self, ev):
            self.ev = ev

        def wait(self):
            torch.cuda.current_stream().wait_event(self.ev)

    def _exchange_bf16(self, buf: torch.Tensor):
        n, W = buf.numel(), self.world
        shard = (n + W - 1) // W
        key = (buf.data_ptr(), n)
        if key not in self._comm_bufs:
            dev = buf.device
            self._comm_bufs[key] = (torch.zeros(W * shard, dtype=torch.bfloat16, device=dev),
                                    torch.empty(W * shard, dtype=torch.bfloat16, device=dev),
                                    torch.empty(shard, dtype=torch.bfloat16, device=dev))
        send, recv, mine = self._comm_bufs[key]
        if self._comm_stream is None:
            self._comm_stream = torch.cuda.Stream(device=buf.device)
        ready = torch.cuda.Event()
        ready.record()
        cs = self._comm_stream
        with torch.cuda.stream(cs):
            cs.wait_event(ready)
            send[:n].copy_(buf)
            dist.all_to_all_single(recv, send, group=self.pg)
            mine.copy_(recv.view(W, shard).float().sum(0).mul_(1.0 / W))
            dist.all_gather_into_tensor(send, mine, group=self.pg)
            buf.copy_(send[:n])
            done = torch.cuda.Event()
            done.record(cs)
        return GraphedStep._EventWait(done)

    def _all_reduce_avg(self, buf: torch.Tensor):
        if self.comm_dtype == torch.bfloat16:
            if self._nccl:
                return self._exchange_bf16(buf)
            h = buf.detach().to(torch.bfloat16).float().cpu()
            dist.all_reduce(h, op=dist.ReduceOp.SUM, group=self.pg)
            buf.copy_(h.mul_(1.0 / self.world).to(torch.bfloat16).float().to(buf.device))
            return None
        if self._nccl:
            return dist.all_reduce(buf, op=dist.ReduceOp.AVG, group=self.pg, async_op=True)
        h = buf.detach().cpu()
        dist.all_reduce(h, op=dist.ReduceOp.SUM, group=self.pg)
        buf.copy_(h.mul_(1.0 / self.world).to(buf.device))
        return None

    def forward_backward(self, x: torch.Tensor, target: torch.Tensor) -> torch.Tensor:
        key = (tuple(x.shape), tuple(target.shape))
        g = self._graphs.get(key)
        if g is None:
            dev = next(self.model.parameters()).device
            sx = x.detach().to(device=dev, dtype=torch.float32, copy=True)
            st = target.detach().to(device=dev, dtype=self._target_dtype, copy=True)
            if self.opt is None:
                self._setup(sx, st)
            g = self._graphs[key] = self._capture(sx, st)
        self._cur = g
        if x.data_ptr() != g.x.data_ptr():
            g.x.copy_(x)
        if target.data_ptr() != g.t.data_ptr():
            g.t.copy_(target)
        if g.fwd is not None:
            g.fwd.replay()
            loss = g.ps.loss(g.t)
            for dst, src in zip(g.gouts, g.ps._gouts):
                if src is None:
                    dst.zero_()
                else:
                    dst.copy_(src)
            self.loss = loss
        else:
            self.loss = g.loss
        self.dice, self.outputs = g.dice, g.outputs
        if self.distributed and self.comm == "tail":
            for gk in g.phases:
                gk.replay()
            w = self._all_reduce_avg(self.opt.flat_g[:self._spans[-1][1]])
            if w is not None:
                w.wait()
        elif self.distributed:
            works = []
            for gk, (a0, a1) in zip(g.phases, self._spans):
                gk.replay()
                works.append(self._all_reduce_avg(self.opt.flat_g[a0:a1]))
            for w in works:
                if w is not None:
                    w.wait()
        else:
            for gk in g.phases:
                gk.replay()
        return self.loss

    def autotune_comm(self, x: torch.Tensor, target: torch.Tensor, steps: int = 6) -> Dict[str, float]:
        if not self.distributed:
            return {}
        dev = next(self.model.parameters()).device
        out: Dict[str, float] = {}
        for mode in ("overlap", "tail"):
            self.comm = mode
            for _ in range(2):
                self(x, target)
            torch.cuda.synchronize(dev)
            if self.world > 1:
                dist.barrier(group=self.pg)
            e0, e1 = torch.cuda.Event(enable_timing=True), torch.cuda.Event(enable_timing=True)
            e0.record()
            for _ in range(steps):
                self(x, target)
            e1.record()
            torch.cuda.synchronize(dev)
            ms = torch.tensor([e0.elapsed_time(e1) / steps], dtype=torch.float64, device=dev if self._nccl else "cpu")
            if self.world > 1:
# ... 37 lines not shown
```

Measured before the change: 2554 images/sec.

## Fuse head 1x1 conv forward, BCE/dice loss, and head backward into one kernel

Adds a fused kernel that applies the last BN+ReLU, computes the 1x1 output conv logits, evaluates the BCE/dice loss terms and the logit gradient, then computes the head weight/bias gradients and BN backward partials in the same pass. This replaces separate outconv forward, bce_dice, and outconv backward launches, so the bf16 head activation is read once and the logits are not round-tripped through memory. In exchange the kernel carries heavy register and shared-memory state, including double-precision loss accumulators. The engine flag fuse_head_loss is enabled by default.

```diff
diff --git a/include/unetzoo_hip.h b/include/unetzoo_hip.h
--- a/include/unetzoo_hip.h
+++ b/include/unetzoo_hip.h
@@ -210,6 +210,11 @@
                          const float* g_nchw, void* dx, int lddx, float* dw, float* db, void* workspace,
                          const void* bn_y, int ld_bny, const float* scale, const float* shift, const float* mean,
                          const float* invstd, float* bn_partial, void* stream);
+long long uz_head_bce_fused_workspace_bytes(int dtype, int N, int HW, int C, int Kout);
+int uz_head_bce_fused(int dtype, const void* y, int ldy, int N, int HW, int C, const float* scale, const float* shift,
+                      const float* mean, const float* invstd, const float* w, const float* b, int Kout,
+                      const float* target, float* logits, float* dlogits, float* out2, float* dw, float* db,
+                      float* bn_partial, void* workspace, void* stream);
 
 int uz_attn_grid(int dtype, int P, int channels);
 int uz_attn_psi_fwd(int dtype, const void* g1raw, int ldg, const void* x1raw, int ldx, const float* vec_g,
diff --git a/unet_zoo_amd/_lib.py b/unet_zoo_amd/_lib.py
--- a/unet_zoo_amd/_lib.py
+++ b/unet_zoo_amd/_lib.py
@@ -19,7 +19,7 @@
     "uz_wgrad_split", "uz_wgrad_workspace_bytes", "uz_wgrad", "uz_wgrad_kernel_name", "uz_wgrad_phase", "uz_wgrad_xf_supported", "uz_wgrad_xf", "uz_conv3x3_first_supported", "uz_conv3x3_first_rows", "uz_conv3x3_first_fwd",
     "uz_conv3x3_first_wgrad_workspace_bytes", "uz_conv3x3_first_wgrad", "uz_conv3x3_first_wgrad_bn", "uz_pack_weights", "uz_pack_weights_batched", "uz_pack_conv3x3_batched", "uz_im2col3x3_nchw", "uz_bn_finalize",
     "uz_bn_eval_scale", "uz_bn_relu_apply", "uz_bn_relu_bwd_workspace_bytes", "uz_bn_relu_bwd_reduce", "uz_bn_relu_bwd_apply",
-    "uz_outconv_fwd", "uz_outconv_fwd_xf", "uz_outconv_bwd_workspace_bytes", "uz_outconv_bwd", "uz_outconv_bwd_rows", "uz_outconv_bwd_bnred", "uz_bn_relu_bwd_apply_head_supported", "uz_bn_relu_bwd_apply_head",
+    "uz_outconv_fwd", "uz_outconv_fwd_xf", "uz_outconv_bwd_workspace_bytes", "uz_outconv_bwd", "uz_outconv_bwd_rows", "uz_outconv_bwd_bnred", "uz_head_bce_fused_workspace_bytes", "uz_head_bce_fused", "uz_bn_relu_bwd_apply_head_supported", "uz_bn_relu_bwd_apply_head",
     "uz_colsum",
     "uz_attn_grid", "uz_attn_psi_fwd", "uz_attn_gate_fwd", "uz_attn_bwd_psi", "uz_attn_bwd_reduce",
     "uz_attn_bwd_apply", "uz_sum_rows", "uz_sum_rows_f32", "uz_sum2x2",
@@ -257,6 +257,8 @@
     lib.uz_bn_relu_bwd_apply_head_supported.argtypes = [ip, ip, ip]
     lib.uz_bn_relu_bwd_apply_head.argtypes = [POINTER(BnBwdDesc), vp, vp, vp, vp, vp, vp, vp, ip, vp, ctypes.c_double, vp, vp]
     lib.uz_outconv_bwd_bnred.argtypes = [ip, vp, ip, ip, ip, ip, vp, ip, vp, vp, ip, vp, vp, vp, vp, ip, vp, vp, vp, vp, vp, vp]
+    lib.uz_head_bce_fused_workspace_bytes.argtypes = [ip, ip, ip, ip, ip]
+    lib.uz_head_bce_fused.argtypes = [ip, vp, ip, ip, ip, ip, vp, vp, vp, vp, vp, vp, ip, vp, vp, vp, vp, vp, vp, vp, vp, vp]
     lib.uz_colsum.argtypes = [ip, vp, ip, ip, ip, vp, vp]
     lib.uz_colsum_workspace_bytes.argtypes = [ip, ip, ip]
     lib.uz_colsum_ws.argtypes = [ip, vp, ip, ip, ip, vp, vp, vp]
diff --git a/unet_zoo_amd/csrc/uz_common.h b/unet_zoo_amd/csrc/uz_common.h
--- a/unet_zoo_amd/csrc/uz_common.h
+++ b/unet_zoo_amd/csrc/uz_common.h
@@ -74,6 +74,19 @@
 }
 
 static inline int uz_cdiv(long long a, long long b) { return (int)((a + b - 1) / b); }
+
+__device__ __forceinline__ void uz_bce_dice_terms(float xv, float tv, double s[4]) {
+  const float m = fmaxf(-xv, 0.f);
+  s[0] += (double)((1.f - tv) * xv + m + logf(expf(-m) + expf(-xv - m)));
+  const float pred = xv > 0.f ? 1.f : 0.f;
+  s[1] += (double)(pred * tv);
+  s[2] += (double)pred;
+  s[3] += (double)tv;
+}
+__device__ __forceinline__ float uz_bce_grad(float xv, float tv, float inv_n) {
+  return (1.f / (1.f + expf(-xv)) - tv) * inv_n;
+}
+int uz_bce_dice_finalize_launch(const double* part, int rows, long long n, float* out2, hipStream_t s);
 
 template <int RG>
 __device__ __forceinline__ void uz_sum_rows_wide_body(const float* __restrict__ partial, int ld, int rows, int n,
diff --git a/unet_zoo_amd/csrc/uz_eltwise.hip b/unet_zoo_amd/csrc/uz_eltwise.hip
--- a/unet_zoo_amd/csrc/uz_eltwise.hip
+++ b/unet_zoo_amd/csrc/uz_eltwise.hip
@@ -831,6 +831,213 @@
 #pragma unroll
         for (int i = 0; i < VEC; ++i) bnpart[((size_t)blockIdx.x * 2 + which) * C + sub * VEC + i] = t[i];
       }
+    }
+  }
+#pragma unroll
+  for (int k = 0; k < KOUT; ++k) {
+    __syncthreads();
+#pragma unroll
+    for (int i = 0; i < VEC; ++i) red[threadIdx.x * 9 + i] = aw[k][i];
+    red[threadIdx.x * 9 + 8] = ab[k];
+    __syncthreads();
+    if (pl == 0) {
+      float t[9];
+#pragma unroll
+      for (int i = 0; i < 9; ++i) t[i] = 0.f;
+      for (int r = 0; r < ppb; ++r)
+#pragma unroll
+        for (int i = 0; i < 9; ++i)
+          if (i < VEC || i == 8) t[i] += red[(r * LPP + sub) * 9 + i];
+      float* row = partial + ((size_t)blockIdx.x * KOUT + k) * (C + 1);
+      if (live) {
+#pragma unroll
+        for (int i = 0; i < VEC; ++i) row[sub * VEC + i] = t[i];
+      }
+      if (sub == 0) row[C] = t[8];
+    }
+  }
+}
+
+template <typename T, int KOUT>
+__global__ __launch_bounds__(256, KOUT == 1 ? 4 : 1) void head_bce_fused_kernel(const T* __restrict__ bn_y, int ld_bny, int N, int HW, int C,
+                                                             const float* __restrict__ w, const float* __restrict__ b,
+                                                             const float* __restrict__ tgt, float inv_n,
+                                                             float* __restrict__ logits, float* __restrict__ dlogits,
+                                                             float* __restrict__ partial, double* __restrict__ lpart,
+                                                             const float* __restrict__ bn_scale, const float* __restrict__ bn_shift,
+                                                             const float* __restrict__ bn_mean, const float* __restrict__ bn_invstd,
+                                                             float* __restrict__ bnpart) {
+  constexpr int VEC = ElemTraits<T>::VEC;
+  constexpr int UNR = 4;
+  constexpr bool LATE = KOUT <= 4;
+  __shared__ float red[256 * 9];
+  __shared__ double lred[256 / 64][4];
+  __shared__ float bnc[4][64 * VEC];
+  __shared__ double lsum[256][4];
+  const int LPP = lanes_per_pixel(C / VEC);
+  const int ppb = blockDim.x / LPP;
+  const int sub = threadIdx.x % LPP, pl = threadIdx.x / LPP;
+  const bool live = sub < C / VEC;
+  const int P = N * HW;
+  float wr[KOUT][VEC], aw[KOUT][VEC], ab[KOUT], bb[KOUT];
+#pragma unroll
+  for (int k = 0; k < KOUT; ++k) {
+    ab[k] = 0.f;
+    bb[k] = b[k];
+#pragma unroll
+    for (int i = 0; i < VEC; ++i) {
+      wr[k][i] = live ? w[k * C + sub * VEC + i] : 0.f;
+      aw[k][i] = 0.f;
+    }
+  }
+  float S0[VEC], S1[VEC];
+#pragma unroll
+  for (int i = 0; i < VEC; ++i) S0[i] = S1[i] = 0.f;
+  for (int c = threadIdx.x; c < C; c += blockDim.x) {
+    bnc[0][c] = bn_mean[c];
+    bnc[1][c] = bn_invstd[c];
+    bnc[2][c] = bn_scale[c];
+    bnc[3][c] = bn_shift[c];
+  }
+#pragma unroll
+  for (int k = 0; k < 4; ++k) lsum[threadIdx.x][k] = 0.0;
+  __syncthreads();
+  for (int p0 = blockIdx.x * ppb * UNR; p0 < P; p0 += gridDim.x * ppb * UNR) {
+    Vec16<T> yr[UNR];
+    float tk[UNR][KOUT], zq[UNR][KOUT];
+#pragma unroll
+    for (int u = 0; u < UNR; ++u) {
+      const int p = p0 + u * ppb + pl;
+      const bool inp = p < P, ok = inp && live;
+      const size_t pc = ok ? (size_t)p : 0;
+      const int cs = ok ? sub * VEC : 0;
+      yr[u] = ld16(bn_y + pc * ld_bny + cs);
+      const int pg = inp ? p : 0;
+      const int img = (KOUT == 1) ? 0 : pg / HW;
+      const int hw = pg - img * HW;
+#pragma unroll
+      for (int k = 0; k < KOUT; ++k) tk[u][k] = tgt[((size_t)img * KOUT + k) * HW + hw];
+    }
+#pragma unroll
+    for (int u = 0; u < UNR; ++u) {
+      const int p = p0 + u * ppb + pl;
+      const bool inp = p < P, ok = inp && live;
+      float v[VEC], yv[VEC], gk[KOUT], bsc[VEC], bsh[VEC];
+      int co = live ? sub * VEC : 0;
+      asm volatile("" : "+v"(co));
+#pragma unroll
+      for (int i = 0; i < VEC; ++i) {
+        bsc[i] = bnc[2][co + i];
+        bsh[i] = bnc[3][co + i];
+      }
+      const int pg = inp ? p : 0;
+      const int img = (KOUT == 1) ? 0 : pg / HW;
+      const size_t li = (size_t)img * KOUT * HW + (pg - img * HW);
+#pragma unroll
+      for (int i = 0; i < VEC; ++i) {
+        yv[i] = (float)yr[u].v[i];
+        const float xv = (float)(T)fmaxf(fmaf(yv[i], bsc[i], bsh[i]), 0.f);
+        v[i] = ok ? xv : 0.f;
+      }
+#pragma unroll
+      for (int k = 0; k < KOUT; ++k) {
+        float s = 0.f;
+#pragma unroll
+        for (int i = 0; i < VEC; ++i) s = fmaf(v[i], wr[k][i], s);
+        for (int o = LPP >> 1; o > 0; o >>= 1) s += __shfl_xor(s, o);
+        const float z = s + bb[k];
+        const float gq = uz_bce_grad(z, tk[u][k], inv_n);
+        gk[k] = inp ? gq : 0.f;
+        if constexpr (LATE) zq[u][k] = z;
+        if (sub == 0 && inp) {
+          logits[li + (size_t)k * HW] = z;
+          dlogits[li + (size_t)k * HW] = gq;
+          if constexpr (!LATE) {
+            double ls[4];
+#pragma unroll
+            for (int q = 0; q < 4; ++q) ls[q] = lsum[threadIdx.x][q];
+            uz_bce_dice_terms(z, tk[u][k], ls);
+#pragma unroll
+            for (int q = 0; q < 4; ++q) lsum[threadIdx.x][q] = ls[q];
+          }
+        }
+      }
+      float d[VEC];
+#pragma unroll
+      for (int i = 0; i < VEC; ++i) d[i] = 0.f;
+#pragma unroll
+      for (int k = 0; k < KOUT; ++k) {
+        ab[k] += gk[k];
+#pragma unroll
+        for (int i = 0; i < VEC; ++i) {
+          d[i] = fmaf(gk[k], wr[k][i], d[i]);
+          aw[k][i] = fmaf(gk[k], v[i], aw[k][i]);
+        }
+      }
+      if (ok) {
+        float bmu[VEC], bis[VEC];
+#pragma unroll
+        for (int i = 0; i < VEC; ++i) {
+          bmu[i] = bnc[0][co + i];
+          bis[i] = bnc[1][co + i];
+        }
+#pragma unroll
+        for (int i = 0; i < VEC; ++i) {
+          const float dz = fmaf(yv[i], bsc[i], bsh[i]) > 0.f ? (float)(T)d[i] : 0.f;
+          S0[i] += dz;
+          S1[i] += dz * ((yv[i] - bmu[i]) * bis[i]);
+        }
+      }
+    }
+    const int EV = LPP < UNR ? LPP : UNR;
+    for (int j = 0; LATE && j < UNR; j += EV) {
+      const int us = j + sub;
+      if (sub < EV && p0 + us * ppb + pl < P) {
+        double ls[4];
+#pragma unroll
+        for (int q = 0; q < 4; ++q) ls[q] = lsum[threadIdx.x][q];
+#pragma unroll
+        for (int k = 0; k < KOUT; ++k) {
+          float zs = zq[0][k], ts = tk[0][k];
+#pragma unroll
+          for (int u = 1; u < UNR; ++u) {
+            zs = us == u ? zq[u][k] : zs;
+            ts = us == u ? tk[u][k] : ts;
+          }
+          uz_bce_dice_terms(zs, ts, ls);
+        }
+#pragma unroll
+        for (int q = 0; q < 4; ++q) lsum[threadIdx.x][q] = ls[q];
+      }
+    }
+  }
+#pragma unroll
+  for (int k = 0; k < 4; ++k) {
+    double t = lsum[threadIdx.x][k];
+    for (int o = 32; o > 0; o >>= 1) t += __shfl_down(t, o);
+    if ((threadIdx.x & 63) == 0) lred[threadIdx.x >> 6][k] = t;
+  }
+  __syncthreads();
+  if (threadIdx.x < 4) {
+    double t = 0.0;
+    for (int wv = 0; wv < 256 / 64; ++wv) t += lred[wv][threadIdx.x];
+    lpart[(size_t)blockIdx.x * 4 + threadIdx.x] = t;
+  }
+#pragma unroll
+  for (int which = 0; which < 2; ++which) {
+    __syncthreads();
+#pragma unroll
+    for (int i = 0; i < VEC; ++i) red[threadIdx.x * 9 + i] = which ? S1[i] : S0[i];
+    __syncthreads();
+    if (pl == 0 && live) {
+      float t[VEC];
+#pragma unroll
+      for (int i = 0; i < VEC; ++i) t[i] = 0.f;
+      for (int r = 0; r < ppb; ++r)
+#pragma unroll
+        for (int i = 0; i < VEC; ++i) t[i] += red[(r * LPP + sub) * 9 + i];
+#pragma unroll
+      for (int i = 0; i < VEC; ++i) bnpart[((size_t)blockIdx.x * 2 + which) * C + sub * VEC + i] = t[i];
     }
   }
 #pragma unroll
@@ -1713,6 +1920,46 @@
   return UZ_OK;
 }
 
+static long long head_bce_fused_part_bytes(int rows, int C, int Kout) {
+  return ((long long)rows * Kout * (C + 1) * (long long)sizeof(float) + 7) / 8 * 8;
+}
+
+extern "C" long long uz_head_bce_fused_workspace_bytes(int dtype, int N, int HW, int C, int Kout) {
+  UZ_REQUIRE(dtype == UZ_BF16, "uz_head_bce_fused_workspace_bytes: bf16 only");
+  UZ_REQUIRE(N > 0 && HW > 0 && Kout >= 1 && Kout <= OUTCONV_MAXK && C % 8 == 0 && C / 8 <= 64,
+             "uz_head_bce_fused_workspace_bytes: bad shape");
+  const int g = outconv_bwd_grid(dtype, N, HW, C);
+  return head_bce_fused_part_bytes(g, C, Kout) + (long long)g * 4 * (long long)sizeof(double);
+}
+
+extern "C" int uz_head_bce_fused(int dtype, const void* y, int ldy, int N, int HW, int C, const float* scale,
+                                 const float* shift, const float* mean, const float* invstd, const float* w,
+                                 const float* b, int Kout, const float* target, float* logits, float* dlogits,
+                                 float* out2, float* dw, float* db, float* bn_partial, void* workspace, void* stream) {
+  UZ_REQUIRE(dtype == UZ_BF16, "uz_head_bce_fused: bf16 only");
+  UZ_REQUIRE(y && scale && shift && mean && invstd && w && b && target && logits && dlogits && out2 && dw && db &&
+                 bn_partial && workspace, "uz_head_bce_fused: null pointer");
+  UZ_REQUIRE(Kout >= 1 && Kout <= OUTCONV_MAXK, "uz_head_bce_fused: Kout=%d (max %d)", Kout, OUTCONV_MAXK);
+  UZ_REQUIRE(C % 8 == 0 && C / 8 <= 64, "uz_head_bce_fused: C=%d unsupported", C);
+  UZ_REQUIRE(ldy % 8 == 0 && ldy >= C && N > 0 && HW > 0 && (long long)N * HW < (1LL << 31), "uz_head_bce_fused: bad shape");
+  UZ_REQUIRE(((uintptr_t)workspace & 7) == 0, "uz_head_bce_fused: workspace not 8-byte aligned");
+  const int g = outconv_bwd_grid(dtype, N, HW, C);
+  float* part = static_cast<float*>(workspace);
+  double* lpart = reinterpret_cast<double*>(static_cast<char*>(workspace) + head_bce_fused_part_bytes(g, C, Kout));
+  const long long n = (long long)N * Kout * HW;
+  hipStream_t s = (hipStream_t)stream;
+  UZ_KOUT_SWITCH(Kout, hipLaunchKernelGGL((head_bce_fused_kernel<bf16_t, KOUT>), dim3((unsigned)g), dim3(256), 0, s,
+                                          (const bf16_t*)y, ldy, N, HW, C, w, b, target, 1.f / (float)n, logits, dlogits, part,
+                                          lpart, scale, shift, mean, invstd, bn_partial))
+  UZ_LAUNCH_CHECK("uz_head_bce_fused");
+  const int rc = uz_bce_dice_finalize_launch(lpart, g, n, out2, s);
+  if (rc != UZ_OK) return rc;
+  const int ne = Kout * (C + 1);
+  hipLaunchKernelGGL(outconv_bwd_finalize_kernel, dim3(uz_cdiv(ne, 32)), dim3(1024), 0, s, part, g, Kout, C, dw, db);
+  UZ_LAUNCH_CHECK("uz_head_bce_fused(finalize)");
+  return UZ_OK;
+}
+
 extern "C" int uz_outconv_bwd(int dtype, const void* x, int ldx, int N, int HW, int C, const float* w,
                               int Kout, const float* g_nchw, void* dx, int lddx, float* dw, float* db,
                               void* workspace, void* stream) {
diff --git a/unet_zoo_amd/csrc/uz_loss.hip b/unet_zoo_amd/csrc/uz_loss.hip
--- a/unet_zoo_amd/csrc/uz_loss.hip
+++ b/unet_zoo_amd/csrc/uz_loss.hip
@@ -11,13 +11,8 @@
   double s[4] = {0.0, 0.0, 0.0, 0.0};
   for (long long i = (long long)blockIdx.x * BD_THREADS + threadIdx.x; i < n; i += (long long)gridDim.x * BD_THREADS) {
     const float xv = x[i], tv = t[i];
-    const float m = fmaxf(-xv, 0.f);
-    s[0] += (double)((1.f - tv) * xv + m + logf(expf(-m) + expf(-xv - m)));
-    const float pred = xv > 0.f ? 1.f : 0.f;
-    s[1] += (double)(pred * tv);
-    s[2] += (double)pred;
-    s[3] += (double)tv;
-    if (dlogits != nullptr) dlogits[i] = (1.f / (1.f + expf(-xv)) - tv) * inv_n;
+    uz_bce_dice_terms(xv, tv, s);
+    if (dlogits != nullptr) dlogits[i] = uz_bce_grad(xv, tv, inv_n);
   }
   __shared__ double red[BD_THREADS / 64][4];
 #pragma unroll
@@ -76,7 +71,11 @@
   hipLaunchKernelGGL(bce_dice_kernel, dim3(rows), dim3(BD_THREADS), 0, s, logits, target, n, 1.f / (float)n, dlogits,
                      (double*)workspace);
   UZ_LAUNCH_CHECK("uz_bce_dice");
-  hipLaunchKernelGGL(bce_dice_finalize_kernel, dim3(1), dim3(BD_THREADS), 0, s, (const double*)workspace, rows, n, out2);
+  return uz_bce_dice_finalize_launch((const double*)workspace, rows, n, out2, s);
+}
+
+int uz_bce_dice_finalize_launch(const double* part, int rows, long long n, float* out2, hipStream_t s) {
+  hipLaunchKernelGGL(bce_dice_finalize_kernel, dim3(1), dim3(BD_THREADS), 0, s, part, rows, n, out2);
   UZ_LAUNCH_CHECK("uz_bce_dice(finalize)");
   return UZ_OK;
 }
diff --git a/unet_zoo_amd/engine.py b/unet_zoo_amd/engine.py
--- a/unet_zoo_amd/engine.py
+++ b/unet_zoo_amd/engine.py
@@ -125,6 +125,7 @@
     fold_bn_apply = True
     fold_bn_apply_head = True
     fold_head_grad = True
+    fuse_head_loss = True
     fold_first_bn_bwd = True
     fuse_bn_finalize = False
     FIN_FLAGS = 4096
@@ -163,6 +164,8 @@
         self._cur_entry = -1
         self._fin_flags: Optional[torch.Tensor] = None
         self._fin_used = 0
+        self.head_target: Optional[torch.Tensor] = None
+        self.head_loss: Optional[tuple] = None
 
     def _fin_flag(self) -> Optional[torch.Tensor]:
         if not self.fuse_bn_finalize:
@@ -1729,6 +1732,8 @@
         b = conv.bias.detach() if conv.bias is not None else torch.zeros(K, device=self.device)
         assert x.lazy is None or sole_reader, "a lazy activation goes to the head it was deferred for"
         xf = x.take_lazy()
+        if self._fuse_head_loss(x, K, xf, sole_reader):
+            return self._out_conv_fused(x, conv, w, b)
         logits = ops.outconv_fwd(x, w, b, xform=xf)
         if self.record:
             def bwd(g_logits: torch.Tensor):
@@ -1756,6 +1761,31 @@
             self._heads.append((bwd, 1))
         return logits
 
+    def _fuse_head_loss(self, x: Act, K: int, xf, sole_reader: bool) -> bool:
+        t = self.head_target
+        return (self.fuse_head_loss and t is not None and self.head_loss is None and self.record and xf is not None
+                and sole_reader and self.fold_head_grad and x.bn_src is not None and self.training
+                and not self.fuse_bn_finalize and self.dtype == torch.bfloat16 and ops.bn_bwd_head_supported(x.bn_src[0], K)
+                and t.dtype == torch.float32 and t.is_contiguous() and tuple(t.shape) == (x.N, K, x.H, x.W))
+
+    def _out_conv_fused(self, x: Act, conv: nn.Conv2d, w: torch.Tensor, b: torch.Tensor) -> torch.Tensor:
+        K = conv.out_channels
+        dwt = self._dst(conv.weight)
+        dbt = self._dst(conv.bias) if conv.bias is not None else None
+        logits, out2, dlogits, dw, db, part = ops.head_bce_fused(x, w, b, x.bn_src, self.head_target,
+                                                                 dwt.view(K, x.C) if dwt is not None else None, dbt)
+        self.head_loss = (logits, out2[0], out2[1], dlogits)
+
+        def bwd(g_logits: torch.Tensor):
+            assert g_logits is dlogits, "the fused head's logit gradients are the ones its own pass wrote"
+            self._give_grad(conv.weight, dwt if dwt is not None else dw.reshape(conv.weight.shape))
+            if conv.bias is not None:
+                self._give_grad(conv.bias, db)
+            x.add_grad(ops.HeadGrad(dlogits, w, part))
+
+        self._heads.append((bwd, 1))
+        return logits
+
     def out_conv_resized(self, x: Act, conv: nn.Conv2d, H: int, W: int, align_corners: bool = True) -> torch.Tensor:
         low = self.out_conv(x, conv)
         N, K, h, w = low.shape
diff --git a/unet_zoo_amd/graph.py b/unet_zoo_amd/graph.py
--- a/unet_zoo_amd/graph.py
+++ b/unet_zoo_amd/graph.py
@@ -93,16 +93,20 @@
         self.eng: Optional[Engine] = None
         self._gouts: Optional[Tuple[Optional[torch.Tensor], ...]] = None
 
+    def _takes_head_loss(self) -> bool:
+        return bool(getattr(getattr(self.loss_fn, "direct", None), "takes_head_loss", False))
+
     def forward(self, x: torch.Tensor, target: torch.Tensor) -> torch.Tensor:
-        self.emit(x)
+        self.emit(x, target if self._takes_head_loss() else None)
         return self.loss(target)
 
-    def emit(self, x: torch.Tensor):
+    def emit(self, x: torch.Tensor, head_target: Optional[torch.Tensor] = None):
         m = self.model
         L.load()
         L.require_cuda(x)
         m._pack_cache.refresh(m.run_dtype)
         self.eng = Engine(m.run_dtype, x.device, m.training, True, None, m._pack_cache, True)
+        self.eng.head_target = head_target
         with torch.no_grad():
             self._outs = tuple(m.emit(self.eng, x))
             self.eng.finish_forward()
@@ -112,7 +116,9 @@
     def loss(self, target: torch.Tensor) -> torch.Tensor:
         direct = getattr(self.loss_fn, "direct", None)
         if direct is not None:
-            res = direct(self.model.wrap_outputs(tuple(o.detach() for o in self._outs)), target)
+            kw = {"head_loss": (self.eng.head_target,) + self.eng.head_loss} \
+                if (self.eng.head_loss is not None and self._takes_head_loss()) else {}
+            res = direct(self.model.wrap_outputs(tuple(o.detach() for o in self._outs)), target, **kw)
             loss, gouts = res[0], res[-1]
             assert len(gouts) == len(self._outs)
             self._gouts = tuple(gouts)
diff --git a/unet_zoo_amd/loss.py b/unet_zoo_amd/loss.py
--- a/unet_zoo_amd/loss.py
+++ b/unet_zoo_amd/loss.py
@@ -34,9 +34,11 @@
         return (ctx.dlogits * g_loss).to(ctx.in_dtype), None
 
 
-def bce_dice_direct(logits: torch.Tensor, target: torch.Tensor):
+def bce_dice_direct(logits: torch.Tensor, target: torch.Tensor, head_loss: Optional[tuple] = None):
     L.require_cuda(logits, target)
     assert logits.shape == target.shape, (logits.shape, target.shape)
+    if head_loss is not None and _same_tensor(head_loss[0], target) and _same_tensor(head_loss[1], logits):
+        return head_loss[2], head_loss[3], head_loss[4]
     x = logits.detach().contiguous().float()
     t = target.detach().contiguous().float()
     n = x.numel()
@@ -50,15 +52,22 @@
     return out[0], out[1], dlogits
 
 
-def loss_and_dice_direct(outputs, target: torch.Tensor):
+def _same_tensor(a: torch.Tensor, b: torch.Tensor) -> bool:
+    return (a.data_ptr() == b.data_ptr() and a.shape == b.shape and a.dtype == b.dtype and a.stride() == b.stride())
+
+
+def loss_and_dice_direct(outputs, target: torch.Tensor, head_loss: Optional[tuple] = None):
     if isinstance(outputs, dict):
-        trip = [bce_dice_direct(v, target) for v in outputs.values()]
+        trip = [bce_dice_direct(v, target, head_loss) for v in outputs.values()]
         return sum(p[0] for p in trip), trip[0][1], tuple(p[2] for p in trip)
     if isinstance(outputs, (list, tuple)):
-        trip = [bce_dice_direct(v, target) for v in outputs]
+        trip = [bce_dice_direct(v, target, head_loss) for v in outputs]
         return sum(p[0] for p in trip), trip[-1][1], tuple(p[2] for p in trip)
-    l, d, g = bce_dice_direct(outputs, target)
+    l, d, g = bce_dice_direct(outputs, target, head_loss)
     return l, d, (g,)
+
+
+loss_and_dice_direct.takes_head_loss = True
 
 
 def bce_dice_with_logits(logits: torch.Tensor, target: torch.Tensor) -> Tuple[torch.Tensor, torch.Tensor]:
diff --git a/unet_zoo_amd/ops.py b/unet_zoo_amd/ops.py
--- a/unet_zoo_amd/ops.py
+++ b/unet_zoo_amd/ops.py
@@ -659,13 +659,15 @@
     out = torch.empty((x.N, K, x.H, x.W), dtype=torch.float32, device=x.buf.device)
     if xform is not None:
         assert outconv_xform_supported(x, K)
-        L.check(lib.uz_outconv_fwd_xf(L.dtype_code(x.dtype), x.raw_ptr(), x.ld, x.N, x.H * x.W, x.C, xform[0].data_ptr(),
-                                      xform[1].data_ptr(), w.data_ptr(), b.data_ptr(), K, out.data_ptr(), L.stream_ptr()),
-                "uz_outconv_fwd_xf")
+        with _Timed("outconv_fwd", 2.0 * K * x.P * x.C, x.buf.element_size() * x.P * x.C + 4.0 * K * x.P):
+            L.check(lib.uz_outconv_fwd_xf(L.dtype_code(x.dtype), x.raw_ptr(), x.ld, x.N, x.H * x.W, x.C, xform[0].data_ptr(),
+                                          xform[1].data_ptr(), w.data_ptr(), b.data_ptr(), K, out.data_ptr(), L.stream_ptr()),
+                    "uz_outconv_fwd_xf")
         return out
-    L.check(lib.uz_outconv_fwd(L.dtype_code(x.dtype), x.ptr(), x.ld, x.N, x.H * x.W, x.C,
-                               w.data_ptr(), b.data_ptr(), K, out.data_ptr(), L.stream_ptr()),
-            "uz_outconv_fwd")
+    with _Timed("outconv_fwd", 2.0 * K * x.P * x.C, x.buf.element_size() * x.P * x.C + 4.0 * K * x.P):
+        L.check(lib.uz_outconv_fwd(L.dtype_code(x.dtype), x.ptr(), x.ld, x.N, x.H * x.W, x.C,
+                                   w.data_ptr(), b.data_ptr(), K, out.data_ptr(), L.stream_ptr()),
+                "uz_outconv_fwd")
     return out
 
 
@@ -692,20 +694,52 @@
         bn_y, vec4 = bnred
         rows = L.check_count(lib.uz_outconv_bwd_rows(code, x.N, x.H * x.W, x.C), "uz_outconv_bwd_rows")
         part = torch.empty((rows, 2, x.C), dtype=torch.float32, device=dev)
-        L.check(lib.uz_outconv_bwd_bnred(code, None if lazy else x.ptr(), x.ld, x.N, x.H * x.W, x.C, w.data_ptr(), K, g.data_ptr(),
-                                         dx.ptr() if store_dx else None, dx.ld if store_dx else 0, dw.data_ptr(), db.data_ptr(),
-                                         ws.data_ptr(), bn_y.ptr(), bn_y.ld,
-                                         vec4[0].data_ptr(), vec4[1].data_ptr(), vec4[2].data_ptr(), vec4[3].data_ptr(),
-                                         part.data_ptr(), L.stream_ptr()), "uz_outconv_bwd_bnred")
+        with _Timed("outconv_bwd", 4.0 * K * x.P * x.C, x.buf.element_size() * x.P * x.C * (1 + store_dx) + 4.0 * K * x.P):
+            L.check(lib.uz_outconv_bwd_bnred(code, None if lazy else x.ptr(), x.ld, x.N, x.H * x.W, x.C, w.data_ptr(), K, g.data_ptr(),
+                                             dx.ptr() if store_dx else None, dx.ld if store_dx else 0, dw.data_ptr(), db.data_ptr(),
+                                             ws.data_ptr(), bn_y.ptr(), bn_y.ld,
+                                             vec4[0].data_ptr(), vec4[1].data_ptr(), vec4[2].data_ptr(), vec4[3].data_ptr(),
+                                             part.data_ptr(), L.stream_ptr()), "uz_outconv_bwd_bnred")
         if not store_dx:
             return dw.view(K, x.C), db, part
         dx.bn_partials = part
         return dw.view(K, x.C), db
-    L.check(lib.uz_outconv_bwd(code, x.ptr(), x.ld, x.N, x.H * x.W, x.C, w.data_ptr(), K, g.data_ptr(),
-                               dx.ptr() if dx is not None else None,
-                               dx.ld if dx is not None else 0, dw.data_ptr(), db.data_ptr(),
-                               ws.data_ptr(), L.stream_ptr()), "uz_outconv_bwd")
+    with _Timed("outconv_bwd", 4.0 * K * x.P * x.C, x.buf.element_size() * x.P * x.C * (1 + (dx is not None)) + 4.0 * K * x.P):
+        L.check(lib.uz_outconv_bwd(code, x.ptr(), x.ld, x.N, x.H * x.W, x.C, w.data_ptr(), K, g.data_ptr(),
+                                   dx.ptr() if dx is not None else None,
+                                   dx.ld if dx is not None else 0, dw.data_ptr(), db.data_ptr(),
+                                   ws.data_ptr(), L.stream_ptr()), "uz_outconv_bwd")
     return dw.view(K, x.C), db
+
+
+def head_bce_fused(x: Act, w: torch.Tensor, b: torch.Tensor, bnred: tuple, target: torch.Tensor,
+                   dw: Optional[torch.Tensor] = None, db: Optional[torch.Tensor] = None):
+    lib = L.load()
+    K = w.shape[0]
+    bn_y, vec4 = bnred
+    assert outconv_xform_supported(bn_y, K) and (bn_y.P, bn_y.C) == (x.P, x.C) and bn_bwd_head_supported(bn_y, K)
+    assert target.dtype == torch.float32 and target.is_contiguous() and target.shape == (x.N, K, x.H, x.W)
+    dev = x.buf.device
+    logits = torch.empty((x.N, K, x.H, x.W), dtype=torch.float32, device=dev)
+    dlogits = torch.empty_like(logits)
+    out2 = torch.empty(2, dtype=torch.float32, device=dev)
+    if dw is None:
+        dw = torch.empty((K, x.C), dtype=torch.float32, device=dev)
+    if db is None:
+        db = torch.empty(K, dtype=torch.float32, device=dev)
+    code = L.dtype_code(x.dtype)
+    HW = x.H * x.W
+    wsb = L.check_count(lib.uz_head_bce_fused_workspace_bytes(code, x.N, HW, x.C, K), "uz_head_bce_fused_workspace_bytes")
+    ws = torch.empty(wsb // 8, dtype=torch.float64, device=dev)
+    rows = L.check_count(lib.uz_outconv_bwd_rows(code, x.N, HW, x.C), "uz_outconv_bwd_rows")
+    part = torch.empty((rows, 2, x.C), dtype=torch.float32, device=dev)
+    es = bn_y.buf.element_size()
+    with _Timed("head_bce_fused", 4.0 * K * x.P * x.C, es * x.P * x.C + 12.0 * K * x.P):
+        L.check(lib.uz_head_bce_fused(code, bn_y.ptr(), bn_y.ld, x.N, HW, x.C, vec4[0].data_ptr(), vec4[1].data_ptr(),
+                                      vec4[2].data_ptr(), vec4[3].data_ptr(), w.data_ptr(), b.data_ptr(), K, target.data_ptr(),
+                                      logits.data_ptr(), dlogits.data_ptr(), out2.data_ptr(), dw.data_ptr(), db.data_ptr(),
+                                      part.data_ptr(), ws.data_ptr(), L.stream_ptr()), "uz_head_bce_fused")
+    return logits, out2, dlogits, dw.view(K, x.C), db, part
 
 
 def colsum(x: Act, out: Optional[torch.Tensor] = None) -> torch.Tensor:
diff --git a/unet_zoo_amd/step.py b/unet_zoo_amd/step.py
--- a/unet_zoo_amd/step.py
+++ b/unet_zoo_amd/step.py
@@ -183,6 +183,22 @@
             torch.cuda.synchronize()
             self._capture_opt()
 
+    def _fused_loss_fn(self, dice_box: list):
+        with_autograd, direct = self._fused
+
+        def fused(out, tt):
+            l, d = with_autograd(out, tt)
+            dice_box.append(d)
+            return l
+
+        def fused_direct(out, tt, **head):
+            l, d, gouts = direct(out, tt, **head)
+            dice_box.append(d)
+            return l, gouts
+        fused_direct.takes_head_loss = getattr(direct, "takes_head_loss", False)
+        fused.direct = fused_direct
+        return fused
+
     def _capture(self, x: torch.Tensor, t: torch.Tensor) -> _ShapeGraphs:
         g = _ShapeGraphs()
         g.x, g.t = x, t
@@ -192,18 +208,7 @@
         torch.cuda.synchronize()
         if self._fused_loss:
             dice_box = []
-            with_autograd, direct = self._fused
-
-            def fused(out, tt):
-                l, d = with_autograd(out, tt)
-                dice_box.append(d)
-                return l
-
-            def fused_direct(out, tt):
-                l, d, gouts = direct(out, tt)
-                dice_box.append(d)
-                return l, gouts
-            fused.direct = fused_direct
+            fused = self._fused_loss_fn(dice_box)
             ps.loss_fn = fused
         else:
             g.fwd = _new_graph()
```

New measurement: 2559 images/sec (median of 2 runs). Within noise of the previous version (+0.2%).
